# ziwang1121/IEEE

Hardware: AMD Instinct MI355X
Metric: 3-modal images/s (train fwd+bwd) (higher is better)
Workload: dtype bf16

## Files before the change

ieee_amd/_lib.py:

```python
import ctypes
import os

_HERE = os.path.dirname(os.path.abspath(__file__))
LIB_PATH = os.environ.get("IEEE_AMD_LIB", os.path.join(_HERE, "libieee_amd.so"))
_lib = None

c_void_p, c_int, c_int64, c_float, c_double = (ctypes.c_void_p, ctypes.c_int, ctypes.c_int64,
                                               ctypes.c_float, ctypes.c_double)

IEEE_F32, IEEE_BF16 = 0, 1

HEADER_PATH = os.path.join(os.path.dirname(_HERE), "include", "ieee_amd.h")

_CTYPE = {"int": c_int, "int64_t": c_int64, "float": c_float, "double": c_double}


def _parse_header(path=HEADER_PATH):
    import re
    txt = open(path).read()
    txt = re.sub(r"/\*.*?\*/", "", txt, flags=re.S)
    txt = re.sub(r"^\s*#.*$", "", txt, flags=re.M)
    sigs, res = {}, {}
    for m in re.finditer(r"([A-Za-z_][\w\s\*]*?)\b(ieee_[a-z0-9_]+)\s*\(([^)]*)\)\s*;", txt):
        ret, name, args = m.group(1).strip(), m.group(2), m.group(3).strip()
        argt = []
        if args and args != "void":
            for a in args.split(","):
                a = a.strip()
                if "*" in a:
                    argt.append(c_void_p)
                else:
                    base = a.replace("const", "").split()[0]
                    argt.append(_CTYPE[base])
        sigs[name] = argt
        if "char" in ret and "*" in ret:
            res[name] = ctypes.c_char_p
        elif "*" in ret:
            res[name] = c_void_p
        else:
            res[name] = _CTYPE[ret.replace("const", "").split()[0]]
    return sigs, res


_SIGNATURES, _RESTYPE = _parse_header()


class WgradReduceDesc(ctypes.Structure):
    _fields_ = [("slab", c_void_p), ("dw", c_void_p), ("slab_gs", c_int64), ("dw_gs", c_int64),
                ("nsplit", ctypes.c_int32), ("Co", ctypes.c_int32), ("Ci", ctypes.c_int32), ("RS", ctypes.c_int32),
                ("kind", ctypes.c_int32), ("sl_log2", ctypes.c_int32), ("blocks", ctypes.c_int32),
                ("accumulate", ctypes.c_int32), ("block_begin", ctypes.c_int32), ("reserved_", ctypes.c_int32)]


class ConvExtras(ctypes.Structure):
    _fields_ = [("totals", c_void_p), ("group_stride", c_int64), ("replicas", ctypes.c_int32), ("reserved_", ctypes.c_int32),
                ("overflow", c_void_p), ("start", c_void_p), ("stop", c_void_p)]


class SgemmSet(ctypes.Structure):
    _fields_ = [("groups", c_int64), ("A", c_void_p), ("B", c_void_p), ("C", c_void_p), ("bias", c_void_p),
                ("M", c_int64), ("N", c_int64), ("K", c_int64), ("sam", c_int64), ("sak", c_int64), ("sbn", c_int64),
                ("sbk", c_int64), ("ldc", c_int64), ("alpha", c_float), ("relu", ctypes.c_int32), ("accumulate", ctypes.c_int32)]


class IeeeAmdError(RuntimeError):
    pass


def exported_symbols():
    return sorted(_SIGNATURES)


def load():
    global _lib
    if _lib is not None:
        return _lib
    if not os.path.exists(LIB_PATH):
        raise IeeeAmdError(
            "ieee_amd HIP library not built: %s is missing. Run `python -c 'import __graft_entry__ as g; "
            "g.build()'` or `make -C ieee_amd/csrc`. There is no CPU fallback." % LIB_PATH)
    import torch
    lib = ctypes.CDLL(LIB_PATH)
    for name, argtypes in _SIGNATURES.items():
        fn = getattr(lib, name)
        fn.argtypes = argtypes
        fn.restype = _RESTYPE.get(name, c_int)
    _lib = lib
    return lib


def check(status):
    if status != 0:
        msg = load().ieee_last_error()
        raise IeeeAmdError((msg or b"").decode("utf-8", "replace") or "ieee_amd error %d" % status)


def require_gpu():
    import torch
    if not torch.cuda.is_available():
        raise IeeeAmdError("ieee_amd needs an MI355X (gfx950) GPU: torch.cuda.is_available() is False and there "
                           "is no CPU fallback.")
    lib = load()
    if not lib.ieee_device_is_gfx950():
        raise IeeeAmdError("ieee_amd kernels are built for gfx950 only; current device is not gfx950.")
    return lib


def ptr(t):
    return c_void_p(t.data_ptr()) if t is not None else c_void_p(0)


def stream():
    import torch
    return c_void_p(torch.cuda.current_stream().cuda_stream)
```

ieee_amd/csrc/head.hip:

```cpp
#include "gemm_core.h"

namespace ieee {

constexpr int MAXG = IEEE_MAX_GROUPS;

struct PtrTab { void* p[MAXG]; };

struct SgemmArgs {
  PtrTab A, B, C, bias;
  int M, N, K;
  int64_t sam, sak, sbn, sbk, ldc;
  float alpha;
  int relu, accumulate;
  int splitk, kchunk, vec_a, vec_b;
  float* slab;
};

typedef float SgemmStage[64][33];
__device__ __forceinline__ void sgemm_tile(const SgemmArgs& a, int bx, int by, int bz, SgemmStage* As, SgemmStage* Bs) {
  const int g = bz / a.splitk, ks = bz - g * a.splitk;
  const float* A = (const float*)a.A.p[g];
  const float* B = (const float*)a.B.p[g];
  const int m0 = by * 64, n0 = bx * 64;
  const int t = threadIdx.x, lane = t & 63, wave = t >> 6, wm = wave >> 1, wn = wave & 1;
  const int kbeg = ks * a.kchunk, kend = min(a.K, kbeg + a.kchunk);
  const int ktiles = (kend - kbeg + 31) / 32;
  f32x4 acc[2][2];
#pragma unroll
  for (int i = 0; i < 2; ++i)
#pragma unroll
    for (int j = 0; j < 2; ++j) acc[i][j] = f32x4{0.f, 0.f, 0.f, 0.f};
  float ra[8], rb[8];
  auto fetch = [&](const float* P, int vec, int64_t srow, int64_t sk, int row0, int nrows, int kt, float* r) {
    const int k0 = kbeg + kt * 32;
    if (vec == 1) {
#pragma unroll
      for (int h = 0; h < 2; ++h) {
        const int row = row0 + (t >> 3) + 32 * h, k = k0 + (t & 7) * 4;
        float4 v = make_float4(0.f, 0.f, 0.f, 0.f);
        if (row < nrows && k + 3 < kend) v = *(const float4*)(P + row * srow + k);
        else if (row < nrows) {
          if (k < kend) v.x = P[row * srow + k];
          if (k + 1 < kend) v.y = P[row * srow + k + 1];
          if (k + 2 < kend) v.z = P[row * srow + k + 2];
        }
        r[4 * h] = v.x; r[4 * h + 1] = v.y; r[4 * h + 2] = v.z; r[4 * h + 3] = v.w;
      }
    } else if (vec == 2) {
#pragma unroll
      for (int h = 0; h < 2; ++h) {
        const int k = k0 + (t >> 4) + 16 * h, row = row0 + (t & 15) * 4;
        float4 v = make_float4(0.f, 0.f, 0.f, 0.f);
        if (k < kend && row + 3 < nrows) v = *(const float4*)(P + k * sk + row);
        else if (k < kend) {
          if (row < nrows) v.x = P[k * sk + row];
          if (row + 1 < nrows) v.y = P[k * sk + row + 1];
          if (row + 2 < nrows) v.z = P[k * sk + row + 2];
        }
        r[4 * h] = v.x; r[4 * h + 1] = v.y; r[4 * h + 2] = v.z; r[4 * h + 3] = v.w;
      }
    } else {
#pragma unroll
      for (int e = 0; e < 8; ++e) {
        const int row = row0 + (t & 63), k = k0 + (t >> 6) + 4 * e;
        r[e] = (row < nrows && k < kend) ? P[row * srow + k * sk] : 0.f;
      }
    }
  };
  auto stash = [&](float (*S)[33], int vec, const float* r) {
    if (vec == 1) {
#pragma unroll
      for (int e = 0; e < 8; ++e) S[(t >> 3) + 32 * (e >> 2)][(t & 7) * 4 + (e & 3)] = r[e];
    } else if (vec == 2) {
#pragma unroll
      for (int e = 0; e < 8; ++e) S[(t & 15) * 4 + (e & 3)][(t >> 4) + 16 * (e >> 2)] = r[e];
    } else {
#pragma unroll
      for (int e = 0; e < 8; ++e) S[t & 63][(t >> 6) + 4 * e] = r[e];
    }
  };
  if (ktiles > 0) {
    fetch(A, a.vec_a, a.sam, a.sak, m0, a.M, 0, ra);
    fetch(B, a.vec_b, a.sbn, a.sbk, n0, a.N, 0, rb);
    stash(As[0], a.vec_a, ra);
    stash(Bs[0], a.vec_b, rb);
  }
  __syncthreads();
  for (int kt = 0; kt < ktiles; ++kt) {
    const int cur = kt & 1;
    const bool has_next = kt + 1 < ktiles;
    if (has_next) {
      fetch(A, a.vec_a, a.sam, a.sak, m0, a.M, kt + 1, ra);
      fetch(B, a.vec_b, a.sbn, a.sbk, n0, a.N, kt + 1, rb);
    }
#pragma unroll
    for (int kk = 0; kk < 8; ++kk) {
      float fa[2], fb[2];
#pragma unroll
      for (int i = 0; i < 2; ++i) fa[i] = As[cur][wm * 32 + i * 16 + (lane & 15)][kk * 4 + (lane >> 4)];
#pragma unroll
      for (int j = 0; j < 2; ++j) fb[j] = Bs[cur][wn * 32 + j * 16 + (lane & 15)][kk * 4 + (lane >> 4)];
#pragma unroll
      for (int i = 0; i < 2; ++i)
#pragma unroll
        for (int j = 0; j < 2; ++j) acc[i][j] = mfma16(fb[j], fa[i], acc[i][j]);
    }
    if (has_next) {
      stash(As[cur ^ 1], a.vec_a, ra);
      stash(Bs[cur ^ 1], a.vec_b, rb);
    }
    __syncthreads();
  }
  if (a.splitk > 1) {
    float* S = a.slab + (int64_t)bz * a.M * a.N;
#pragma unroll
    for (int i = 0; i < 2; ++i)
#pragma unroll
      for (int j = 0; j < 2; ++j) {
        const int m = m0 + wm * 32 + i * 16 + (lane & 15);
        const int n = n0 + wn * 32 + j * 16 + (lane >> 4) * 4;
        if (m >= a.M) continue;
#pragma unroll
        for (int r = 0; r < 4; ++r)
          if (n + r < a.N) S[(int64_t)m * a.N + n + r] = acc[i][j][r];
      }
    return;
  }
  float* C = (float*)a.C.p[g];
  const float* bias = (const float*)a.bias.p[g];
#pragma unroll
  for (int i = 0; i < 2; ++i)
#pragma unroll
    for (int j = 0; j < 2; ++j) {
      const int m = m0 + wm * 32 + i * 16 + (lane & 15);
      const int n = n0 + wn * 32 + j * 16 + (lane >> 4) * 4;
      if (m >= a.M) continue;
#pragma unroll
      for (int r = 0; r < 4; ++r) {
        if (n + r >= a.N) continue;
        float v = a.alpha * acc[i][j][r];
        if (bias) v += bias[n + r];
        float* c = C + (int64_t)m * a.ldc + n + r;
        if (a.accumulate) v += *c;
        if (a.relu) v = fmaxf(v, 0.f);
        *c = v;
      }
    }
}

__global__ __launch_bounds__(256) void sgemm_grouped_kernel(SgemmArgs a) {
  __shared__ float As[2][64][33];
  __shared__ float Bs[2][64][33];
  sgemm_tile(a, blockIdx.x, blockIdx.y, blockIdx.z, As, Bs);
}

struct PairDims { int gx0, gy0, blocks0, gx1, gy1; };
__global__ __launch_bounds__(256) void sgemm_grouped2_kernel(SgemmArgs a0, SgemmArgs a1, PairDims d) {
  __shared__ float As[2][64][33];
  __shared__ float Bs[2][64][33];
  int b = blockIdx.x;
  if (b < d.blocks0) {
    sgemm_tile(a0, b % d.gx0, (b / d.gx0) % d.gy0, b / (d.gx0 * d.gy0), As, Bs);
  } else {
    b -= d.blocks0;
    sgemm_tile(a1, b % d.gx1, (b / d.gx1) % d.gy1, b / (d.gx1 * d.gy1), As, Bs);
  }
}

__device__ __forceinline__ void sgemm_splitk_reduce_one(const SgemmArgs& a, int g, int64_t i) {
  const int64_t mn = (int64_t)a.M * a.N;
  if (i >= mn) return;
  const float* S = a.slab + (int64_t)g * a.splitk * mn + i;
  float s = 0.f;
  for (int k = 0; k < a.splitk; ++k) s += S[k * mn];
  const int m = (int)(i / a.N), n = (int)(i - (int64_t)m * a.N);
  float v = a.alpha * s;
  const float* bias = (const float*)a.bias.p[g];
  if (bias) v += bias[n];
  float* c = (float*)a.C.p[g] + (int64_t)m * a.ldc + n;
  if (a.accumulate) v += *c;
  if (a.relu) v = fmaxf(v, 0.f);
  *c = v;
}
__global__ __launch_bounds__(256) void sgemm_splitk_reduce_kernel(SgemmArgs a) {
  sgemm_splitk_reduce_one(a, blockIdx.y, (int64_t)blockIdx.x * blockDim.x + threadIdx.x);
}
struct PairReduceDims { int rb0, blocks0, rb1; };
__global__ __launch_bounds__(256) void sgemm_splitk_reduce2_kernel(SgemmArgs a0, SgemmArgs a1, PairReduceDims d) {
  int b = blockIdx.x;
  if (b < d.blocks0) {
    sgemm_splitk_reduce_one(a0, b / d.rb0, (int64_t)(b % d.rb0) * blockDim.x + threadIdx.x);
  } else {
    b -= d.blocks0;
    sgemm_splitk_reduce_one(a1, b / d.rb1, (int64_t)(b % d.rb1) * blockDim.x + threadIdx.x);
  }
}

struct ZeroArgs { PtrTab p; int64_t n[MAXG]; };
__global__ void zero_spans_kernel(ZeroArgs a) {
  float* p = (float*)a.p.p[blockIdx.y];
  const int64_t n = a.n[blockIdx.y];
  for (int64_t i = (int64_t)blockIdx.x * blockDim.x + threadIdx.x; i < n; i += (int64_t)gridDim.x * blockDim.x) p[i] = 0.f;
}

struct ColsumArgs {
  PtrTab X, out;
  int M, N;
  int64_t ldx;
  int accumulate;
};
__global__ void colsum_grouped_kernel(ColsumArgs a) {
  const int g = blockIdx.y;
  const int n = blockIdx.x * blockDim.x + threadIdx.x;
  if (n >= a.N) return;
  const float* X = (const float*)a.X.p[g];
  float s = 0.f;
  for (int m = 0; m < a.M; ++m) s += X[(int64_t)m * a.ldx + n];
  float* o = (float*)a.out.p[g] + n;
  *o = a.accumulate ? *o + s : s;
}

struct RowBnArgs {
  PtrTab x, out, gamma, beta, rmean, rvar, save;
  int R, C;
  int64_t ldx, ldo;
  float momentum, eps;
  int training, relu;
};
constexpr int RB_TX = 16, RB_TY = 16;
__device__ __forceinline__ float rb_sum(float (*red)[RB_TX], int tx) {
  float s = 0.f;
#pragma unroll
  for (int y = 0; y < RB_TY; ++y) s += red[y][tx];
  return s;
}
__global__ __launch_bounds__(256) void rowbn_fwd_kernel(RowBnArgs a) {
  __shared__ float red[RB_TY][RB_TX];
  const int g = blockIdx.y;
  const int tx = threadIdx.x % RB_TX, ty = threadIdx.x / RB_TX;
  const int c = blockIdx.x * RB_TX + tx;
  const bool ok = c < a.C;
  const float* x = (const float*)a.x.p[g];
  float* out = (float*)a.out.p[g];
  float mean, invstd;
  if (a.training) {
    float s = 0.f;
    if (ok) {
#pragma unroll 4
      for (int r = ty; r < a.R; r += RB_TY) s += x[(int64_t)r * a.ldx + c];
    }
    red[ty][tx] = s;
    __syncthreads();
    mean = rb_sum(red, tx) / a.R;
    __syncthreads();
    float v = 0.f;
    if (ok) {
#pragma unroll 4
      for (int r = ty; r < a.R; r += RB_TY) { const float d = x[(int64_t)r * a.ldx + c] - mean; v += d * d; }
    }
    red[ty][tx] = v;
    __syncthreads();
    const float var = rb_sum(red, tx) / a.R;
    invstd = 1.0f / sqrtf(var + a.eps);
    if (ok && ty == 0) {
      float* rm = (float*)a.rmean.p[g];
      float* rv = (float*)a.rvar.p[g];
      if (rm) {
        const float unb = a.R > 1 ? var * ((float)a.R / (float)(a.R - 1)) : var;
        rm[c] = (1.f - a.momentum) * rm[c] + a.momentum * mean;
        rv[c] = (1.f - a.momentum) * rv[c] + a.momentum * unb;
      }
    }
  } else {
    mean = ok ? ((const float*)a.rmean.p[g])[c] : 0.f;
    invstd = ok ? 1.0f / sqrtf(((const float*)a.rvar.p[g])[c] + a.eps) : 0.f;
  }
  if (!ok) return;
  if (ty == 0 && a.save.p[g]) { float* sv = (float*)a.save.p[g]; sv[c] = mean; sv[a.C + c] = invstd; }
  const float ga = ((const float*)a.gamma.p[g])[c], be = ((const float*)a.beta.p[g])[c];
#pragma unroll 4
  for (int r = ty; r < a.R; r += RB_TY) {
    float v = (x[(int64_t)r * a.ldx + c] - mean) * invstd * ga + be;
    if (a.relu) v = fmaxf(v, 0.f);
    out[(int64_t)r * a.ldo + c] = v;
  }
}

struct RowBnBwdArgs {
  PtrTab dout, out, x, gamma, save, dx, dgamma, dbeta;
  int R, C;
  int64_t lddo, ldo, ldx, lddx;
  int relu, accumulate;
};
__global__ __launch_bounds__(256) void rowbn_bwd_kernel(RowBnBwdArgs a) {
  __shared__ float red[2][RB_TY][RB_TX];
  const int g = blockIdx.y;
  const int tx = threadIdx.x % RB_TX, ty = threadIdx.x / RB_TX;
  const int c = blockIdx.x * RB_TX + tx;
  const bool ok = c < a.C;
  const float* dout = (const float*)a.dout.p[g];
  const float* out = (const float*)a.out.p[g];
  const float* x = (const float*)a.x.p[g];
  const float* sv = (const float*)a.save.p[g];
  const float mean = ok ? sv[c] : 0.f, invstd = ok ? sv[a.C + c] : 0.f;
  float s1 = 0.f, s2 = 0.f;
  if (ok) {
#pragma unroll 4
    for (int r = ty; r < a.R; r += RB_TY) {
      float gq = dout[(int64_t)r * a.lddo + c];
      if ((a.relu & 1) && !(out[(int64_t)r * a.ldo + c] > 0.f)) gq = 0.f;
      s1 += gq;
      s2 += gq * (x[(int64_t)r * a.ldx + c] - mean) * invstd;
    }
  }
  red[0][ty][tx] = s1;
  red[1][ty][tx] = s2;
  __syncthreads();
  s1 = rb_sum(red[0], tx);
  s2 = rb_sum(red[1], tx);
  if (!ok) return;
  const float ga = ((const float*)a.gamma.p[g])[c];
  const bool frozen = (a.relu & 2) != 0;
  if (ty == 0 && !frozen) {
    float* dg = (float*)a.dgamma.p[g] + c;
    float* db = (float*)a.dbeta.p[g] + c;
    *dg = a.accumulate ? *dg + s2 : s2;
    *db = a.accumulate ? *db + s1 : s1;
  }
  float* dx = (float*)a.dx.p[g];
  const float c1 = frozen ? 0.f : s1 / a.R, c2 = frozen ? 0.f : s2 / a.R;
#pragma unroll 4
  for (int r = ty; r < a.R; r += RB_TY) {
    float gq = dout[(int64_t)r * a.lddo + c];
    if ((a.relu & 1) && !(out[(int64_t)r * a.ldo + c] > 0.f)) gq = 0.f;
    const float xh = (x[(int64_t)r * a.ldx + c] - mean) * invstd;
    dx[(int64_t)r * a.lddx + c] = ga * invstd * (gq - c1 - xh * c2);
  }
}

__global__ void add_halves_kernel(const float* h, float* hs, int64_t half, int64_t gs_in, int64_t gs_out) {
  const int z = blockIdx.y;
  for (int64_t i = (int64_t)blockIdx.x * blockDim.x + threadIdx.x; i < half; i += (int64_t)gridDim.x * blockDim.x)
    hs[z * gs_out + i] = h[z * gs_in + i] + h[z * gs_in + half + i];
}
__global__ void sigmoid_kernel(float* x, int64_t n) {
  for (int64_t i = (int64_t)blockIdx.x * blockDim.x + threadIdx.x; i < n; i += (int64_t)gridDim.x * blockDim.x)
    x[i] = 1.0f / (1.0f + expf(-x[i]));
}
__global__ void sigmoid_bwd_kernel(const float* datt, const float* att, float* dz, int64_t n) {
  for (int64_t i = (int64_t)blockIdx.x * blockDim.x + threadIdx.x; i < n; i += (int64_t)gridDim.x * blockDim.x)
    dz[i] = datt[i] * att[i] * (1.f - att[i]);
}
__global__ void add_halves_bwd_kernel(const float* dhs, const float* h, float* dh, int64_t half, int64_t gs_half,
                                      int64_t gs_full) {
  const int z = blockIdx.y;
  for (int64_t i = (int64_t)blockIdx.x * blockDim.x + threadIdx.x; i < half; i += (int64_t)gridDim.x * blockDim.x) {
    const float d = dhs[z * gs_half + i];
    dh[z * gs_full + i] = h[z * gs_full + i] > 0.f ? d : 0.f;
    dh[z * gs_full + half + i] = h[z * gs_full + half + i] > 0.f ? d : 0.f;
  }
}

__global__ void rem_fwd_kernel(const float* part, const float* r, const float* param, int64_t param_gs, float* out,
                               int B, int parts, int D) {
  const int z = blockIdx.y;
  const float s = 2.0f * param[z * param_gs];
  const int64_t n = (int64_t)B * parts * D;
  for (int64_t i = (int64_t)blockIdx.x * blockDim.x + threadIdx.x; i < n; i += (int64_t)gridDim.x * blockDim.x) {
    const int k = (int)(i % D);
    const int b = (int)(i / ((int64_t)parts * D));
    out[z * n + i] = part[z * n + i] + s * r[((int64_t)z * B + b) * D + k];
  }
}
__global__ __launch_bounds__(256) void rem_bwd_kernel(const float* dout, const float* r, const float* param,
                                                      int64_t param_gs, float* dr, float* dparam_partial, int B,
                                                      int parts, int D) {
  __shared__ float red[256];
  const int z = blockIdx.y, b = blockIdx.x;
  const float s = 2.0f * param[z * param_gs];
  float accp = 0.f;
  for (int k = threadIdx.x; k < D; k += blockDim.x) {
    float sum = 0.f;
    for (int i = 0; i < parts; ++i) sum += dout[(((int64_t)z * B + b) * parts + i) * D + k];
    dr[((int64_t)z * B + b) * D + k] = s * sum;
    accp += sum * r[((int64_t)z * B + b) * D + k];
  }
  red[threadIdx.x] = accp;
  __syncthreads();
  for (int o = 128; o > 0; o >>= 1) { if (threadIdx.x < o) red[threadIdx.x] += red[threadIdx.x + o]; __syncthreads(); }
  if (threadIdx.x == 0) dparam_partial[(int64_t)z * B + b] = 2.0f * red[0];
}
__global__ void rem_dparam_kernel(const float* partial, float* dparam, int64_t grad_gs, int B, int accumulate) {
  const int z = threadIdx.x;
  if (z >= 3) return;
  float s = 0.f;
  for (int b = 0; b < B; ++b) s += partial[(int64_t)z * B + b];
  float* o = dparam + z * grad_gs;
  *o = accumulate ? *o + s : s;
}

__global__ void l2norm_fwd_kernel(const float* x, float* y, float* norms, int64_t rows, int D) {
  const int64_t row = (int64_t)blockIdx.x * 4 + (threadIdx.x >> 6);
  if (row >= rows) return;
  const int lane = threadIdx.x & 63;
  float s = 0.f;
  for (int k = lane; k < D; k += 64) { const float v = x[row * D + k]; s += v * v; }
  s = wave_sum(s);
  const float nrm = fmaxf(sqrtf(s), 1e-12f);
  for (int k = lane; k < D; k += 64) y[row * D + k] = x[row * D + k] / nrm;
  if (lane == 0) norms[row] = nrm;
}
__global__ void l2norm_bwd_kernel(const float* dy, const float* y, const float* norms, float* dx, int64_t rows, int D,
                                  int accumulate) {
  const int64_t row = (int64_t)blockIdx.x * 4 + (threadIdx.x >> 6);
  if (row >= rows) return;
  const int lane = threadIdx.x & 63;
  float s = 0.f;
  for (int k = lane; k < D; k += 64) s += dy[row * D + k] * y[row * D + k];
  s = wave_sum(s);
  const float nrm = norms[row];
  const float dot = nrm > 1e-12f ? s : 0.f;
  for (int k = lane; k < D; k += 64) {
    const float v = (dy[row * D + k] - y[row * D + k] * dot) / nrm;
    dx[row * D + k] = accumulate ? dx[row * D + k] + v : v;
  }
}

__global__ void ce_rows_kernel(const float* logits, const int64_t* target, float* rowloss, int* correct,
                               float* dlogits, int heads, int B, int C, float eps, float gscale) {
  const int64_t row = (int64_t)blockIdx.x * 4 + (threadIdx.x >> 6);
  if (row >= (int64_t)heads * B) return;
  const int lane = threadIdx.x & 63;
  const int b = (int)(row % B);
  const float* x = logits + row * C;
  const int y = (int)target[b];
  float mx = -INFINITY;
  int am = 0;
  for (int c = lane; c < C; c += 64) { const float v = x[c]; if (v > mx) { mx = v; am = c; } }
  for (int o = 32; o > 0; o >>= 1) {
    const float ov = __shfl_xor(mx, o);
    const int oi = __shfl_xor(am, o);
    if (ov > mx || (ov == mx && oi < am)) { mx = ov; am = oi; }
  }
  float se = 0.f, sx = 0.f;
  for (int c = lane; c < C; c += 64) { se += expf(x[c] - mx); sx += x[c]; }
  se = wave_sum(se);
  sx = wave_sum(sx);
  const float lse = mx + logf(se);
  const float logpy = x[y] - lse;
  if (lane == 0) {
    rowloss[row] = -(1.f - eps) * logpy - (eps / C) * (sx - C * lse);
    correct[row] = am == y ? 1 : 0;
  }
  if (dlogits) {
    const float sc = gscale / B;
    for (int c = lane; c < C; c += 64) {
      const float p = expf(x[c] - lse);
      const float tt = (c == y ? (1.f - eps) : 0.f) + eps / C;
      dlogits[row * C + c] = (p - tt) * sc;
    }
  }
}
__global__ void ce_heads_kernel(const float* rowloss, const int* correct, float* head_loss, float* head_acc,
                                int heads, int B) {
  const int h = blockIdx.x * blockDim.x + threadIdx.x;
  if (h >= heads) return;
  float s = 0.f;
  int k = 0;
  for (int b = 0; b < B; ++b) { s += rowloss[(int64_t)h * B + b]; k += correct[(int64_t)h * B + b]; }
  head_loss[h] = s / B;
  head_acc[h] = 100.0f * k / B;
}

__global__ __launch_bounds__(256) void margin3m_kernel(const float* feats, const int64_t* pids, float* dfeats,
                                                       float* terms, int B, int D, float margin, float gscale) {
  __shared__ float red[3][256];
  __shared__ int s_cnt[256];
  __shared__ int s_sel;
  __shared__ float s_sign;
  const int t = threadIdx.x;
  int cnt = 0;
  for (int i = t; i < B; i += 256) {
    bool seen = false;
    for (int j = 0; j < i; ++j) if (pids[j] == pids[i]) { seen = true; break; }
    cnt += seen ? 0 : 1;
  }
  s_cnt[t] = cnt;
  __syncthreads();
  for (int o = 128; o > 0; o >>= 1) { if (t < o) s_cnt[t] += s_cnt[t + o]; __syncthreads(); }
  const int n = s_cnt[0];
  const int csize = (B + n - 1) / n;
  const int nchunks = (B + csize - 1) / csize;
  const int nuse = nchunks < n ? nchunks : n;
  const int ch = blockIdx.x;
  const int64_t BD = (int64_t)B * D;
  if (ch == 0 && t == 0) { terms[B] = (float)n; terms[B + 1] = (float)nchunks; terms[B + 2] = (float)nuse; }
  const int r0 = ch * csize, r1 = min(B, r0 + csize), rows = r1 - r0;
  if (rows <= 0) { if (t == 0) terms[ch] = 0.f; return; }
  if (ch >= nuse) {
    if (t == 0) terms[ch] = 0.f;
    if (dfeats)
      for (int m = 0; m < 3; ++m)
        for (int64_t i = t; i < (int64_t)rows * D; i += 256) dfeats[m * BD + (int64_t)r0 * D + i] = 0.f;
    return;
  }
  float d12 = 0.f, d23 = 0.f, d13 = 0.f;
  for (int k = t; k < D; k += 256) {
    float c1 = 0.f, c2 = 0.f, c3 = 0.f;
    for (int r = r0; r < r1; ++r) { c1 += feats[r * D + k]; c2 += feats[BD + r * D + k]; c3 += feats[2 * BD + r * D + k]; }
    c1 /= rows; c2 /= rows; c3 /= rows;
    d12 += (c1 - c2) * (c1 - c2);
    d23 += (c2 - c3) * (c2 - c3);
    d13 += (c1 - c3) * (c1 - c3);
  }
  red[0][t] = d12; red[1][t] = d23; red[2][t] = d13;
  __syncthreads();
  for (int o = 128; o > 0; o >>= 1) {
    if (t < o) { red[0][t] += red[0][t + o]; red[1][t] += red[1][t + o]; red[2][t] += red[2][t + o]; }
    __syncthreads();
  }
  if (t == 0) {
    const float a1 = fabsf(margin - red[0][0]), a2 = fabsf(margin - red[1][0]), a3 = fabsf(margin - red[2][0]);
    int sel = 0; float best = a1;
    if (a2 > best) { best = a2; sel = 1; }
    if (a3 > best) { best = a3; sel = 2; }
    const float dsel = sel == 0 ? red[0][0] : (sel == 1 ? red[1][0] : red[2][0]);
    const float x = margin - dsel;
    s_sel = sel;
    s_sign = x > 0.f ? -1.f : (x < 0.f ? 1.f : 0.f);
    terms[ch] = best;
  }
  __syncthreads();
  if (dfeats) {
    const int sel = s_sel;
    const int ia = sel == 1 ? 1 : 0;
    const int ib = sel == 0 ? 1 : 2;
    const int ic = 3 - ia - ib;
    const float coef = s_sign * 2.0f / rows * gscale;
    for (int k = t; k < D; k += 256) {
      float ca = 0.f, cb = 0.f;
      for (int r = r0; r < r1; ++r) { ca += feats[ia * BD + r * D + k]; cb += feats[ib * BD + r * D + k]; }
      const float diff = (ca - cb) / rows;
      for (int r = r0; r < r1; ++r) {
        dfeats[ia * BD + r * D + k] = coef * diff;
        dfeats[ib * BD + r * D + k] = -coef * diff;
        dfeats[ic * BD + r * D + k] = 0.f;
      }
    }
  }
}
__global__ void margin3m_sum_kernel(const float* terms, float* out, int B) {
  if (threadIdx.x != 0) return;
  const int nuse = (int)terms[B + 2];
  float loss = 0.f;
  for (int c = 0; c < nuse; ++c) loss += terms[c];
  out[0] = loss; out[1] = terms[B]; out[2] = terms[B + 1];
}

__device__ __forceinline__ void sgd_one(float& w, float g, float& buf, float lr, float momentum, float wd, int nesterov) {
  float d = g + wd * w;
  if (momentum != 0.f) {
    const float b = momentum * buf + d;
    buf = b;
    d = nesterov ? d + momentum * b : b;
  }
  w = w - lr * d;
}
__global__ void sgd_nesterov_kernel(float* __restrict__ p, const float* __restrict__ g, float* __restrict__ buf,
                                    int64_t n, float lr, float momentum, float wd, int nesterov, int vec, bf16* __restrict__ shadow,
                                    const int* __restrict__ skip) {
  if (skip != nullptr && (skip[0] | skip[1]) != 0) return;
  const int64_t tid = (int64_t)blockIdx.x * blockDim.x + threadIdx.x, nth = (int64_t)gridDim.x * blockDim.x;
  int64_t done = 0;
  if (vec) {
    const int64_t n4 = n >> 2;
    for (int64_t i = tid; i < n4; i += nth) {
      float4 w = ((float4*)p)[i];
      const float4 gg = ((const float4*)g)[i];
      float4 b = momentum != 0.f ? ((float4*)buf)[i] : make_float4(0.f, 0.f, 0.f, 0.f);
      sgd_one(w.x, gg.x, b.x, lr, momentum, wd, nesterov);
      sgd_one(w.y, gg.y, b.y, lr, momentum, wd, nesterov);
      sgd_one(w.z, gg.z, b.z, lr, momentum, wd, nesterov);
      sgd_one(w.w, gg.w, b.w, lr, momentum, wd, nesterov);
      if (momentum != 0.f) ((float4*)buf)[i] = b;
      ((float4*)p)[i] = w;
      if (shadow != nullptr) ((uint2*)shadow)[i] = make_uint2(Vec16<bf16>::pk(w.x, w.y), Vec16<bf16>::pk(w.z, w.w));
    }
    done = n4 << 2;
  }
  for (int64_t i = done + tid; i < n; i += nth) {
    float w = p[i], b = momentum != 0.f ? buf[i] : 0.f;
    sgd_one(w, g[i], b, lr, momentum, wd, nesterov);
    if (momentum != 0.f) buf[i] = b;
    p[i] = w;
    if (shadow != nullptr) shadow[i] = (bf16)w;
  }
}

static int ewb(int64_t n) {
  static const int64_t cap = getenv("IEEE_HEAD_EW_BLOCKS") ? atoll(getenv("IEEE_HEAD_EW_BLOCKS")) : 2048;
  int64_t b = (n + 255) / 256;
  return (int)(b > cap ? cap : (b < 1 ? 1 : b));
}

}

using namespace ieee;

static int fill_tab(PtrTab* t, const void* const* src, int groups) {
  for (int i = 0; i < MAXG; ++i) t->p[i] = i < groups && src ? (void*)src[i] : nullptr;
  return 0;
}

static bool aligned16(const void* const* tab, int groups) {
  for (int i = 0; i < groups; ++i)
    if (((uintptr_t)tab[i] & 15) != 0) return false;
  return true;
}

static int sgemm_fill(SgemmArgs& a, int64_t groups, const void* const* A, const void* const* B, void* const* C,
                      const void* const* bias, int64_t M, int64_t N, int64_t K, int64_t sam, int64_t sak, int64_t sbn,
                      int64_t sbk, int64_t ldc, float alpha, int relu, int accumulate, void* work, int64_t work_bytes);

extern "C" int ieee_sgemm_grouped_ws(int64_t groups, const void* const* A, const void* const* B, void* const* C,
                                     const void* const* bias, int64_t M, int64_t N, int64_t K, int64_t sam, int64_t sak,
                                     int64_t sbn, int64_t sbk, int64_t ldc, float alpha, int relu, int accumulate,
                                     void* work, int64_t work_bytes, void* stream) {
  SgemmArgs a;
  IEEE_TRY(sgemm_fill(a, groups, A, B, C, bias, M, N, K, sam, sak, sbn, sbk, ldc, alpha, relu, accumulate, work, work_bytes));
  dim3 grid(cdiv(N, 64), cdiv(M, 64), (unsigned)(groups * a.splitk));
  sgemm_grouped_kernel<<<grid, 256, 0, (hipStream_t)stream>>>(a);
  IEEE_TRY(launch_status("sgemm_grouped_kernel"));
  if (a.splitk > 1) {
    sgemm_splitk_reduce_kernel<<<dim3(cdiv(M * N, 256), (unsigned)groups), 256, 0, (hipStream_t)stream>>>(a);
    return launch_status("sgemm_splitk_reduce_kernel");
  }
  return IEEE_OK;
}

extern "C" int ieee_sgemm_grouped_pair_ws(const ieee_sgemm_set* s0, const ieee_sgemm_set* s1, void* work, int64_t work_bytes,
                                          void* stream) {
  IEEE_REQUIRE(s0 && s1, "sgemm_grouped_pair: null problem set");
  const int64_t half = work ? (work_bytes / 2) & ~(int64_t)255 : 0;
  SgemmArgs a0, a1;
  IEEE_TRY(sgemm_fill(a0, s0->groups, s0->A, s0->B, s0->C, s0->bias, s0->M, s0->N, s0->K, s0->sam, s0->sak, s0->sbn, s0->sbk, s0->ldc,
                      s0->alpha, s0->relu, s0->accumulate, work, half));
  IEEE_TRY(sgemm_fill(a1, s1->groups, s1->A, s1->B, s1->C, s1->bias, s1->M, s1->N, s1->K, s1->sam, s1->sak, s1->sbn, s1->sbk, s1->ldc,
                      s1->alpha, s1->relu, s1->accumulate, work ? (char*)work + half : nullptr, half));
  PairDims d;
  d.gx0 = cdiv(s0->N, 64); d.gy0 = cdiv(s0->M, 64); d.blocks0 = d.gx0 * d.gy0 * (int)(s0->groups * a0.splitk);
  d.gx1 = cdiv(s1->N, 64); d.gy1 = cdiv(s1->M, 64);
  const int blocks1 = d.gx1 * d.gy1 * (int)(s1->groups * a1.splitk);
  sgemm_grouped2_kernel<<<dim3((unsigned)(d.blocks0 + blocks1)), 256, 0, (hipStream_t)stream>>>(a0, a1, d);
  IEEE_TRY(launch_status("sgemm_grouped2_kernel"));
  if (a0.splitk > 1 || a1.splitk > 1) {
    PairReduceDims r;
    r.rb0 = a0.splitk > 1 ? cdiv(s0->M * s0->N, 256) : 1;
    r.blocks0 = a0.splitk > 1 ? r.rb0 * (int)s0->groups : 0;
    r.rb1 = a1.splitk > 1 ? cdiv(s1->M * s1->N, 256) : 1;
    const int rblocks1 = a1.splitk > 1 ? r.rb1 * (int)s1->groups : 0;
    sgemm_splitk_reduce2_kernel<<<dim3((unsigned)(r.blocks0 + rblocks1)), 256, 0, (hipStream_t)stream>>>(a0, a1, r);
    return launch_status("sgemm_splitk_reduce2_kernel");
  }
  return IEEE_OK;
}

static int sgemm_fill(SgemmArgs& a, int64_t groups, const void* const* A, const void* const* B, void* const* C,
                      const void* const* bias, int64_t M, int64_t N, int64_t K, int64_t sam, int64_t sak, int64_t sbn,
                      int64_t sbk, int64_t ldc, float alpha, int relu, int accumulate, void* work, int64_t work_bytes) {
  IEEE_REQUIRE(groups >= 1 && groups <= MAXG, "sgemm_grouped: groups %ld out of range [1,%d]", (long)groups, MAXG);
  IEEE_REQUIRE(A && B && C, "sgemm_grouped: null pointer table");
  IEEE_REQUIRE(M > 0 && N > 0 && K > 0, "sgemm_grouped: empty problem");
  fill_tab(&a.A, A, (int)groups);
  fill_tab(&a.B, B, (int)groups);
  fill_tab(&a.C, (const void* const*)C, (int)groups);
  fill_tab(&a.bias, bias, (int)groups);
  a.M = (int)M; a.N = (int)N; a.K = (int)K;
  a.sam = sam; a.sak = sak; a.sbn = sbn; a.sbk = sbk; a.ldc = ldc;
  a.alpha = alpha; a.relu = relu; a.accumulate = accumulate;
  a.vec_a = (sak == 1 && sam % 4 == 0 && aligned16(A, (int)groups)) ? 1
            : (sam == 1 && sak % 4 == 0 && aligned16(A, (int)groups)) ? 2 : 0;
  a.vec_b = (sbk == 1 && sbn % 4 == 0 && aligned16(B, (int)groups)) ? 1
            : (sbn == 1 && sbk % 4 == 0 && aligned16(B, (int)groups)) ? 2 : 0;
  const int64_t tiles = cdiv(N, 64) * cdiv(M, 64) * groups;
  int64_t splitk = 1;
  if (work && tiles < 1024 && K >= 256) {
    splitk = cdiv(1024, tiles);
    if (splitk > K / 128) splitk = K / 128;
    if (splitk > 32) splitk = 32;
    while (splitk > 1 && splitk * groups * M * N * 4 > work_bytes) --splitk;
    if (splitk < 1) splitk = 1;
  }
  a.kchunk = (int)(cdiv(cdiv(K, splitk), 32) * 32);
  a.splitk = (int)cdiv(K, a.kchunk);
  a.slab = (float*)work;
  return IEEE_OK;
}

extern "C" int ieee_sgemm_grouped(int64_t groups, const void* const* A, const void* const* B, void* const* C,
                                  const void* const* bias, int64_t M, int64_t N, int64_t K, int64_t sam, int64_t sak,
                                  int64_t sbn, int64_t sbk, int64_t ldc, float alpha, int relu, int accumulate,
                                  void* stream) {
  return ieee_sgemm_grouped_ws(groups, A, B, C, bias, M, N, K, sam, sak, sbn, sbk, ldc, alpha, relu, accumulate, nullptr,
                               0, stream);
}

extern "C" int ieee_zero_spans(int64_t count, void* const* ptrs, const int64_t* floats, void* stream) {
  IEEE_REQUIRE(count >= 1 && count <= MAXG && ptrs && floats, "zero_spans: bad arguments");
  ZeroArgs a;
  fill_tab(&a.p, (const void* const*)ptrs, (int)count);
  int64_t most = 1;
  for (int i = 0; i < MAXG; ++i) { a.n[i] = i < count ? floats[i] : 0; most = a.n[i] > most ? a.n[i] : most; }
  zero_spans_kernel<<<dim3(ewb(most), (unsigned)count), 256, 0, (hipStream_t)stream>>>(a);
  return launch_status("zero_spans_kernel");
}

extern "C" int ieee_colsum_grouped(int64_t groups, const void* const* X, void* const* out, int64_t M, int64_t N,
                                   int64_t ldx, int accumulate, void* stream) {
  IEEE_REQUIRE(groups >= 1 && groups <= MAXG && X && out, "colsum_grouped: bad arguments");
  ColsumArgs a;
  fill_tab(&a.X, X, (int)groups);
  fill_tab(&a.out, (const void* const*)out, (int)groups);
  a.M = (int)M; a.N = (int)N; a.ldx = ldx; a.accumulate = accumulate;
  colsum_grouped_kernel<<<dim3(cdiv(N, 128), (unsigned)groups), 128, 0, (hipStream_t)stream>>>(a);
  return launch_status("colsum_grouped_kernel");
}

extern "C" int ieee_rowbn_fwd(int64_t groups, const void* const* x, void* const* out, const void* const* gamma,
                              const void* const* beta, void* const* running_mean, void* const* running_var,
                              void* const* save, int64_t R, int64_t C, int64_t ldx, int64_t ldo, float momentum,
                              float eps, int training, int relu, void* stream) {
  IEEE_REQUIRE(groups >= 1 && groups <= MAXG && x && out && gamma && beta, "rowbn_fwd: bad arguments");
  IEEE_REQUIRE(training || (running_mean && running_var), "rowbn_fwd: eval mode needs running stats");
  RowBnArgs a;
  fill_tab(&a.x, x, (int)groups);
  fill_tab(&a.out, (const void* const*)out, (int)groups);
  fill_tab(&a.gamma, gamma, (int)groups);
  fill_tab(&a.beta, beta, (int)groups);
  fill_tab(&a.rmean, (const void* const*)running_mean, (int)groups);
  fill_tab(&a.rvar, (const void* const*)running_var, (int)groups);
  fill_tab(&a.save, (const void* const*)save, (int)groups);
  a.R = (int)R; a.C = (int)C; a.ldx = ldx; a.ldo = ldo; a.momentum = momentum; a.eps = eps;
  a.training = training; a.relu = relu;
  rowbn_fwd_kernel<<<dim3(cdiv(C, RB_TX), (unsigned)groups), 256, 0, (hipStream_t)stream>>>(a);
  return launch_status("rowbn_fwd_kernel");
}

extern "C" int ieee_rowbn_bwd(int64_t groups, const void* const* dout, const void* const* out, const void* const* x,
                              const void* const* gamma, const void* const* save, void* const* dx,
                              void* const* dgamma, void* const* dbeta, int64_t R, int64_t C, int64_t lddo,
                              int64_t ldo, int64_t ldx, int64_t lddx, int relu, int accumulate, void* stream) {
  IEEE_REQUIRE(groups >= 1 && groups <= MAXG && dout && out && x && gamma && save && dx && dgamma && dbeta,
               "rowbn_bwd: bad arguments");
  RowBnBwdArgs a;
  fill_tab(&a.dout, dout, (int)groups);
  fill_tab(&a.out, out, (int)groups);
  fill_tab(&a.x, x, (int)groups);
  fill_tab(&a.gamma, gamma, (int)groups);
  fill_tab(&a.save, save, (int)groups);
  fill_tab(&a.dx, (const void* const*)dx, (int)groups);
  fill_tab(&a.dgamma, (const void* const*)dgamma, (int)groups);
  fill_tab(&a.dbeta, (const void* const*)dbeta, (int)groups);
  a.R = (int)R; a.C = (int)C; a.lddo = lddo; a.ldo = ldo; a.ldx = ldx; a.lddx = lddx;
  a.relu = relu; a.accumulate = accumulate;
  rowbn_bwd_kernel<<<dim3(cdiv(C, RB_TX), (unsigned)groups), 256, 0, (hipStream_t)stream>>>(a);
  return launch_status("rowbn_bwd_kernel");
}

extern "C" int ieee_ca_mix_fwd(const float* h, float* hs, int64_t B, int64_t hidden, void* stream) {
  IEEE_REQUIRE(h && hs, "ca_mix_fwd: null pointer");
  add_halves_kernel<<<dim3(ewb(B * hidden), 3), 256, 0, (hipStream_t)stream>>>(h, hs, B * hidden, 2 * B * hidden,
                                                                                B * hidden);
  return launch_status("add_halves_kernel");
}
extern "C" int ieee_ca_mix_bwd(const float* dhs, const float* h, float* dh, int64_t B, int64_t hidden, void* stream) {
  IEEE_REQUIRE(dhs && h && dh, "ca_mix_bwd: null pointer");
  add_halves_bwd_kernel<<<dim3(ewb(B * hidden), 3), 256, 0, (hipStream_t)stream>>>(dhs, h, dh, B * hidden, B * hidden,
                                                                                    2 * B * hidden);
  return launch_status("add_halves_bwd_kernel");
}
extern "C" int ieee_sigmoid_fwd(float* x, int64_t n, void* stream) {
  IEEE_REQUIRE(x, "sigmoid_fwd: null pointer");
  sigmoid_kernel<<<ewb(n), 256, 0, (hipStream_t)stream>>>(x, n);
  return launch_status("sigmoid_kernel");
}
extern "C" int ieee_sigmoid_bwd(const float* datt, const float* att, float* dz, int64_t n, void* stream) {
  IEEE_REQUIRE(datt && att && dz, "sigmoid_bwd: null pointer");
  sigmoid_bwd_kernel<<<ewb(n), 256, 0, (hipStream_t)stream>>>(datt, att, dz, n);
  return launch_status("sigmoid_bwd_kernel");
}

extern "C" int ieee_rem_fwd(const float* part, const float* r, const float* param, int64_t param_gs, float* out,
                            int64_t B, int64_t parts, int64_t D, void* stream) {
  IEEE_REQUIRE(part && r && param && out, "rem_fwd: null pointer");
  rem_fwd_kernel<<<dim3(ewb(B * parts * D), 3), 256, 0, (hipStream_t)stream>>>(part, r, param, param_gs, out, (int)B,
                                                                                (int)parts, (int)D);
  return launch_status("rem_fwd_kernel");
}
extern "C" int ieee_rem_bwd(const float* dout, const float* r, const float* param, int64_t param_gs, float* dr,
                            float* dparam, int64_t grad_gs, float* work, int64_t B, int64_t parts, int64_t D,
                            int accumulate, void* stream) {
  IEEE_REQUIRE(dout && r && param && dr && dparam && work, "rem_bwd: null pointer");
  hipStream_t st = (hipStream_t)stream;
  rem_bwd_kernel<<<dim3((unsigned)B, 3), 256, 0, st>>>(dout, r, param, param_gs, dr, work, (int)B, (int)parts, (int)D);
  IEEE_TRY(launch_status("rem_bwd_kernel"));
  rem_dparam_kernel<<<1, 64, 0, st>>>(work, dparam, grad_gs, (int)B, accumulate);
  return launch_status("rem_dparam_kernel");
}

extern "C" int ieee_l2norm_fwd(const float* x, float* y, float* norms, int64_t rows, int64_t D, void* stream) {
  IEEE_REQUIRE(x && y && norms, "l2norm_fwd: null pointer");
  l2norm_fwd_kernel<<<cdiv(rows, 4), 256, 0, (hipStream_t)stream>>>(x, y, norms, rows, (int)D);
  return launch_status("l2norm_fwd_kernel");
}
extern "C" int ieee_l2norm_bwd(const float* dy, const float* y, const float* norms, float* dx, int64_t rows,
                               int64_t D, int accumulate, void* stream) {
  IEEE_REQUIRE(dy && y && norms && dx, "l2norm_bwd: null pointer");
  l2norm_bwd_kernel<<<cdiv(rows, 4), 256, 0, (hipStream_t)stream>>>(dy, y, norms, dx, rows, (int)D, accumulate);
  return launch_status("l2norm_bwd_kernel");
}

extern "C" int ieee_ce_ls_fwd_bwd(const float* logits, const int64_t* targets, float* dlogits, float* head_loss,
                                  float* head_acc, float* work, int64_t heads, int64_t B, int64_t C, float eps,
                                  float grad_scale, void* stream) {
  IEEE_REQUIRE(logits && targets && head_loss && head_acc && work, "ce_ls_fwd_bwd: null pointer");
  IEEE_REQUIRE(heads >= 1 && B >= 1 && C >= 1, "ce_ls_fwd_bwd: empty input");
  hipStream_t st = (hipStream_t)stream;
  float* rowloss = work;
  int* correct = (int*)(work + heads * B);
  ce_rows_kernel<<<cdiv(heads * B, 4), 256, 0, st>>>(logits, targets, rowloss, correct, dlogits, (int)heads, (int)B,
                                                     (int)C, eps, grad_scale);
  IEEE_TRY(launch_status("ce_rows_kernel"));
  ce_heads_kernel<<<cdiv(heads, 64), 64, 0, st>>>(rowloss, correct, head_loss, head_acc, (int)heads, (int)B);
  return launch_status("ce_heads_kernel");
}

extern "C" int ieee_margin3m_fwd_bwd(const float* feats, const int64_t* pids, float* dfeats, float* out3, float* work,
                                     int64_t B, int64_t D, float margin, float grad_scale, void* stream) {
  IEEE_REQUIRE(feats && pids && out3 && work, "margin3m_fwd_bwd: null pointer");
  IEEE_REQUIRE(B >= 1 && D >= 1 && B <= 65535, "margin3m_fwd_bwd: batch out of range");
  hipStream_t st = (hipStream_t)stream;
  margin3m_kernel<<<(unsigned)B, 256, 0, st>>>(feats, pids, dfeats, work, (int)B, (int)D, margin, grad_scale);
  IEEE_TRY(launch_status("margin3m_kernel"));
  margin3m_sum_kernel<<<1, 64, 0, st>>>(work, out3, (int)B);
  return launch_status("margin3m_sum_kernel");
}

__global__ void adam_kernel(float* __restrict__ p, const float* __restrict__ g, float* __restrict__ m,
                            float* __restrict__ v, float* __restrict__ vmax, int64_t n, float lr, float b1, float b2,
                            float eps, float wd, float bc1, float bc2_sqrt) {
  const float step_size = lr / bc1;
  for (int64_t i = (int64_t)blockIdx.x * blockDim.x + threadIdx.x; i < n; i += (int64_t)gridDim.x * blockDim.x) {
    const float w = p[i];
    const float d = g[i] + wd * w;
    const float mi = m[i] + (d - m[i]) * (1.f - b1);
    const float vi = b2 * v[i] + (1.f - b2) * d * d;
    m[i] = mi;
    v[i] = vi;
    float vv = vi;
    if (vmax != nullptr) {
      vv = fmaxf(vmax[i], vi);
      vmax[i] = vv;
    }
    const float denom = sqrtf(vv) / bc2_sqrt + eps;
    p[i] = w - step_size * (mi / denom);
  }
}

extern "C" int ieee_adam_step(float* params, const float* grads, float* exp_avg, float* exp_avg_sq,
                              float* max_exp_avg_sq, int64_t n, float lr, float beta1, float beta2, float eps,
                              float weight_decay, int64_t step, void* stream) {
  IEEE_REQUIRE(params && grads && exp_avg && exp_avg_sq, "adam_step: null pointer");
  IEEE_REQUIRE(step >= 1, "adam_step: step counts from 1");
  if (n <= 0) return IEEE_OK;
  const double bc1 = 1.0 - pow((double)beta1, (double)step), bc2 = 1.0 - pow((double)beta2, (double)step);
  adam_kernel<<<ewb(n), 256, 0, (hipStream_t)stream>>>(params, grads, exp_avg, exp_avg_sq, max_exp_avg_sq, n, lr, beta1,
                                                       beta2, eps, weight_decay, (float)bc1, (float)sqrt(bc2));
  return launch_status("adam_kernel");
}

__global__ void guard_buffers_kernel(const int* __restrict__ flags, float* __restrict__ buffers, float* __restrict__ backup, int64_t n) {
  const bool restore = flags[0] != 0;
  for (int64_t i = (int64_t)blockIdx.x * blockDim.x + threadIdx.x; i < n; i += (int64_t)gridDim.x * blockDim.x) {
    if (restore) buffers[i] = backup[i]; else backup[i] = buffers[i];
  }
}
extern "C" int ieee_guard_buffers(const int* flags, float* buffers, float* backup, int64_t n, void* stream) {
  IEEE_REQUIRE(flags && buffers && backup && n >= 0, "guard_buffers: bad arguments");
  if (n == 0) return IEEE_OK;
  guard_buffers_kernel<<<ewb(n), 256, 0, (hipStream_t)stream>>>(flags, buffers, backup, n);
  return launch_status("guard_buffers_kernel");
}

extern "C" int ieee_sgd_nesterov_step_ex(float* params, const float* grads, float* momentum_buf, int64_t n, float lr,
                                         float momentum, float weight_decay, int nesterov, void* shadow_bf16,
                                         const int* skip_flags, void* stream) {
  IEEE_REQUIRE(params && grads && (momentum == 0.f || momentum_buf), "sgd_nesterov_step: null pointer");
  if (n <= 0) return IEEE_OK;
  const int vec = ((((uintptr_t)params | (uintptr_t)grads | (uintptr_t)momentum_buf) & 15) == 0 && ((uintptr_t)shadow_bf16 & 7) == 0) ? 1 : 0;
  sgd_nesterov_kernel<<<ewb(vec ? (n + 3) / 4 : n), 256, 0, (hipStream_t)stream>>>(params, grads, momentum_buf, n, lr,
                                                                                   momentum, weight_decay, nesterov, vec,
                                                                                   (bf16*)shadow_bf16, skip_flags);
  return launch_status("sgd_nesterov_kernel");
}

extern "C" int ieee_sgd_nesterov_step(float* params, const float* grads, float* momentum_buf, int64_t n, float lr,
                                      float momentum, float weight_decay, int nesterov, void* stream) {
  return ieee_sgd_nesterov_step_ex(params, grads, momentum_buf, n, lr, momentum, weight_decay, nesterov, nullptr, nullptr, stream);
}

__global__ void grad_pack_bf16_kernel(const float* __restrict__ g, bf16* __restrict__ out, int64_t n, int64_t peel) {
  const int64_t tid = (int64_t)blockIdx.x * blockDim.x + threadIdx.x, nth = (int64_t)gridDim.x * blockDim.x;
  const int64_t n8 = (n - peel) >> 3;
  const float4* g4 = (const float4*)(g + peel);
  uint4* o4 = (uint4*)(out + peel);
  for (int64_t i = tid; i < n8; i += nth) {
    const float4 a = g4[2 * i], b = g4[2 * i + 1];
    const float f[8] = {a.x, a.y, a.z, a.w, b.x, b.y, b.z, b.w};
    o4[i] = Vec16<bf16>::pack(f);
  }
  for (int64_t i = tid; i < peel; i += nth) out[i] = (bf16)g[i];
  for (int64_t i = peel + (n8 << 3) + tid; i < n; i += nth) out[i] = (bf16)g[i];
}
__global__ void grad_unpack_bf16_kernel(const bf16* __restrict__ in, float* __restrict__ g, int64_t n, int64_t peel) {
  const int64_t tid = (int64_t)blockIdx.x * blockDim.x + threadIdx.x, nth = (int64_t)gridDim.x * blockDim.x;
  const int64_t n8 = (n - peel) >> 3;
  const uint4* i4 = (const uint4*)(in + peel);
  float4* g4 = (float4*)(g + peel);
  for (int64_t i = tid; i < n8; i += nth) {
    float f[8];
    Vec16<bf16>::unpack(i4[i], f);
    g4[2 * i] = make_float4(f[0], f[1], f[2], f[3]);
    g4[2 * i + 1] = make_float4(f[4], f[5], f[6], f[7]);
  }
  for (int64_t i = tid; i < peel; i += nth) g[i] = (float)in[i];
  for (int64_t i = peel + (n8 << 3) + tid; i < n; i += nth) g[i] = (float)in[i];
}

static int64_t grad_peel(const void* f32p, const void* bf16p, int64_t n) {
  const int64_t peel = (int64_t)(((32 - ((uintptr_t)f32p & 31)) & 31) >> 2);
  if ((((uintptr_t)f32p & 3) != 0) || ((((uintptr_t)bf16p + 2 * peel) & 15) != 0) || peel > n) return n;
  return peel;
}

extern "C" int ieee_grad_pack_bf16(const float* grads, void* out_bf16, int64_t n, void* stream) {
  if (n <= 0) return IEEE_OK;
  IEEE_REQUIRE(grads && out_bf16, "grad_pack_bf16: null pointer");
  const int64_t peel = grad_peel(grads, out_bf16, n);
  grad_pack_bf16_kernel<<<ewb((n + 7) / 8 + 8), 256, 0, (hipStream_t)stream>>>(grads, (bf16*)out_bf16, n, peel);
  return launch_status("grad_pack_bf16_kernel");
}
extern "C" int ieee_grad_unpack_bf16(const void* in_bf16, float* grads, int64_t n, void* stream) {
  if (n <= 0) return IEEE_OK;
  IEEE_REQUIRE(grads && in_bf16, "grad_unpack_bf16: null pointer");
  const int64_t peel = grad_peel(grads, in_bf16, n);
  grad_unpack_bf16_kernel<<<ewb((n + 7) / 8 + 8), 256, 0, (hipStream_t)stream>>>((const bf16*)in_bf16, grads, n, peel);
  return launch_status("grad_unpack_bf16_kernel");
}
```

ieee_amd/csrc/net.hip:

```cpp
#include <stdio.h>
#include <stdlib.h>
#include <string.h>

#include <map>
#include <string>
#include <vector>

#include "common.h"

namespace {

using namespace ieee;

struct Tensor {
  size_t off = 0;
  int64_t numel = 0;
  int dtype = IEEE_F32;
};

static constexpr int TOT_REP_MAX = 8;
static int totals_tiles() {
  static const int t = getenv("IEEE_BN_TOTALS_TILES") ? atoi(getenv("IEEE_BN_TOTALS_TILES")) : 1024;
  return t;
}
// ... 649 lines not shown
    return wgrad_on(u, dy, x);
  }
  int wgrad_on(const ConvUnit& u, const void* dy, const void* x) {
    prof_begin(1, u);
    struct G { Run* r; ~G() { r->prof_end(); } } guard{this};
    if (u.Ci != u.Ci_src || u.S != u.S_src || u.R != u.R_src) {
      const int64_t npad = (int64_t)u.Co * u.Ci * u.R * u.S;
      IEEE_TRY(wgrad_pending_now());
      IEEE_TRY(ieee_conv2d_wgrad(dy, x, F(u.dwpad), P(n.slab), n.dtype, 3, B, u.Hi, u.Wi, u.Ci, u.Co, u.R, u.S, u.stride,
                                 u.pad, u.M(B) * u.Co, (int64_t)B * u.Hi * u.Wi * u.Ci, npad, 0, st));
      return ieee_unpad_weight_grad(F(u.dwpad), grd(u.s_w), 3, u.Co, u.Ci, u.R, u.S, u.Ci_src, u.R_src, u.S_src, npad, gs(u.s_w), 0,
                                    st);
    }
    if (wgrad_batch_mode() == 0 && wgrad_chain()) {
      ieee_wgrad_reduce_desc d;
      const int rc = ieee_conv2d_wgrad_chained(dy, x, grd(u.s_w), P(n.wflip ? n.slab2 : n.slab), n.dtype, 3, B, u.Hi, u.Wi, u.Ci, u.Co,
                                               u.R, u.S, u.stride, u.pad, u.M(B) * u.Co, (int64_t)B * u.Hi * u.Wi * u.Ci, gs(u.s_w), 0,
                                               n.wpend.kind != 0 ? &n.wpend : nullptr, &d, st);
      if (rc != IEEE_OK) return rc;
      n.wpend = d;
      if (d.kind != 0) n.wflip ^= 1;
      return IEEE_OK;
    }
    if (wgrad_batch_mode() == 0 && wgrad_fold() && n.dtype == IEEE_BF16)
      return ieee_conv2d_wgrad_fold(dy, x, grd(u.s_w), P(n.slab), (int32_t*)P(n.wtickets), n.dtype, 3, B, u.Hi, u.Wi, u.Ci, u.Co,
                                    u.R, u.S, u.stride, u.pad, u.M(B) * u.Co, (int64_t)B * u.Hi * u.Wi * u.Ci, gs(u.s_w), 0, st);
    if (wgrad_batch_mode() == 0)
      return ieee_conv2d_wgrad(dy, x, grd(u.s_w), P(n.slab), n.dtype, 3, B, u.Hi, u.Wi, u.Ci, u.Co, u.R, u.S, u.stride,
                               u.pad, u.M(B) * u.Co, (int64_t)B * u.Hi * u.Wi * u.Ci, gs(u.s_w), 0, st);
    ieee_wgrad_reduce_desc d;
    IEEE_TRY(ieee_conv2d_wgrad_deferred(dy, x, grd(u.s_w), P(u.slab), n.dtype, 3, B, u.Hi, u.Wi, u.Ci, u.Co, u.R, u.S, u.stride,
                                        u.pad, u.M(B) * u.Co, (int64_t)B * u.Hi * u.Wi * u.Ci, gs(u.s_w), 0, &d, st));
    if (d.kind != 0) n.rpend.push_back(d);
    return IEEE_OK;
  }
  int wgrad_pending_now() {
    if (n.wpend.kind == 0) return IEEE_OK;
    const ieee_wgrad_reduce_desc d = n.wpend;
    n.wpend.kind = 0;
    return ieee_wgrad_reduce_pending(&d, 3, st);
  }
  int wgrad_flush(int slot) {
    if (n.wpend.kind != 0) {
      void* main_st = st;
      const bool on_side = side_enabled();
      if (on_side) st = (void*)n.side;
      prof_begin(1, n.reduce_unit, "wgrad_reduce");
      const int rc = wgrad_pending_now();
      prof_end();
      st = main_st;
      if (on_side) n.side_dirty = true;
      IEEE_TRY(rc);
    }
    if (n.rpend.empty()) return IEEE_OK;
    std::vector<ieee_wgrad_reduce_desc> tab;
    tab.swap(n.rpend);
    IEEE_REQUIRE(slot >= 0 && slot < Net::RT_SLOTS && (int)tab.size() <= Net::RT_MAX, "net: reduce table overflow (%d entries, slot %d)",
                 (int)tab.size(), slot);
    int blocks = 0;
    for (auto& d : tab) { d.block_begin = blocks; blocks += d.blocks; }
    void* main_st = st;
    const bool on_side = side_enabled();
    if (on_side) st = (void*)n.side;
    struct G { Run* r; void* m; ~G() { r->st = m; } } restore{this, main_st};
    ieee_wgrad_reduce_desc* dev = (ieee_wgrad_reduce_desc*)(ws + n.rtab.off) + (size_t)slot * Net::RT_MAX;
    std::vector<ieee_wgrad_reduce_desc>& host = n.rtab_host[slot];
    const size_t bytes = tab.size() * sizeof(ieee_wgrad_reduce_desc);
    if (n.rtab_ws[slot] != (const void*)ws || host.size() != tab.size() || memcmp(host.data(), tab.data(), bytes) != 0) {
      host = tab;
      IEEE_HIP(hipStreamSynchronize((hipStream_t)st));
      IEEE_HIP(hipMemcpy(dev, host.data(), bytes, hipMemcpyHostToDevice));
      n.rtab_ws[slot] = (const void*)ws;
    }
    prof_begin(1, n.reduce_unit, "wgrad_reduce");
    struct H { Run* r; ~H() { r->prof_end(); } } guard{this};
    const int rc = ieee_wgrad_reduce_batch(dev, (int64_t)tab.size(), blocks, 3, st);
    if (on_side) n.side_dirty = true;
    return rc;
  }
  const ConvUnit* ds_sums_of = nullptr;
  int dgrad(const ConvUnit& u, const void* dy, void* dx, const void* addend, const ConvUnit* prev = nullptr,
            bool prev_mask_tensor = false, int addend_stride = 1, const ConvUnit* prev_ds = nullptr) {
    const int64_t ldd = ieee_conv_packed_ld(n.dtype, u.Co, u.R, u.S);
    const bool fuse = prev != nullptr && n.dtype == IEEE_BF16;
    static const bool ds_sums = getenv("IEEE_DS_SUMS") && atoi(getenv("IEEE_DS_SUMS")) != 0;
    const bool fuse2 = fuse && prev_ds != nullptr && ds_sums && !branch_enabled(2);
    fused_bwd = fuse;
    n.bwd_totals_state = fuse && !fuse2 && use_totals(*prev) && !frz(*prev);
    if (fuse2) ds_sums_of = prev_ds;
    will_write(dx);
    prof_begin(0, u, "dgrad", true);
    struct G { Run* r; ~G() { r->prof_end(); } } guard{this};
    const ieee_conv_extras* ex = n.bwd_totals_state ? take_extras(P(prev->tot_b), (int64_t)2 * prev->Co, totals_rep(*prev))
                                                    : take_extras(nullptr, 0, 1);
    return ieee_conv2d_dgrad_ex(dy, P(u.wd), dx, addend, n.dtype, 3, B, u.Hi, u.Wi, u.Ci, u.Co, u.R, u.S, u.stride, u.pad,
                              u.M(B) * u.Co, u.Ci * ldd, (int64_t)B * u.Hi * u.Wi * u.Ci, fuse ? bnpart_cur : nullptr,
                              fuse ? P(prev->y) : nullptr,
                              (fuse && prev_mask_tensor) ? (prev->abits.numel ? P(prev->abits) : P(prev->a)) : nullptr,
                              (fuse && !prev_mask_tensor) ? F(prev->stats) : nullptr,
                              (fuse && prev_mask_tensor && prev->abits.numel) ? 1 : 0, addend_stride,
                              fuse2 ? P(prev_ds->y) : nullptr, fuse2 ? (float*)(ws + n.bnpart2.off) : nullptr, ex, st);
  }
  bool compact_ds(const ConvUnit& d, const ConvUnit* prev) const {
    static const bool on = !(getenv("IEEE_DS_COMPACT") && atoi(getenv("IEEE_DS_COMPACT")) == 0);
    return on && n.dtype == IEEE_BF16 && prev != nullptr && d.R == 1 && d.S == 1 && d.stride == 2 && d.pad == 0 && d.Hi == 2 * d.Ho &&
           d.Wi == 2 * d.Wo && !(d.Hi & (d.Hi - 1)) && !(d.Wi & (d.Wi - 1));
  }
  int dgrad_compact(const ConvUnit& d, const void* dy, void* dx) {
    const int64_t ldd = ieee_conv_packed_ld(n.dtype, d.Co, 1, 1);
    fused_bwd = false;
    n.bwd_totals_state = false;
    will_write(dx);
    prof_begin(0, d, "dgrad", true);
    struct G { Run* r; ~G() { r->prof_end(); } } guard{this};
    return ieee_conv2d_dgrad_ex(dy, P(d.wd), dx, nullptr, n.dtype, 3, B, d.Ho, d.Wo, d.Ci, d.Co, 1, 1, 1, 0, d.M(B) * d.Co,
                                d.Ci * ldd, d.M(B) * d.Ci, nullptr, nullptr, nullptr, nullptr, 0, 1, nullptr, nullptr,
                                take_extras(nullptr, 0, 1), st);
  }
  int gemm3(const float* A, int64_t a_gs, const float* Bm, int64_t b_gs, float* C, int64_t c_gs, const float* bias,
            int64_t bias_gs, int64_t M, int64_t N, int64_t K, int64_t sam, int64_t sak, int64_t sbn, int64_t sbk,
            int64_t ldc, int relu, int acc) {
    const void* a[3]; const void* b[3]; void* c[3]; const void* bi[3];
    for (int m = 0; m < 3; ++m) { a[m] = A + m * a_gs; b[m] = Bm + m * b_gs; c[m] = C + m * c_gs; bi[m] = bias ? bias + m * bias_gs : nullptr; }
    return ieee_sgemm_grouped_ws(3, a, b, c, bias ? bi : nullptr, M, N, K, sam, sak, sbn, sbk, ldc, 1.0f, relu, acc,
                                 P(n.gemm_work), (int64_t)n.gemm_work.numel * 2, st);
  }
  static bool head_pairs() {
    static const bool on = !(getenv("IEEE_HEAD_PAIRS") && atoi(getenv("IEEE_HEAD_PAIRS")) == 0);
    return on;
  }
  struct Set3 {
    const void* a[3]; const void* b[3]; void* c[3]; const void* bi[3];
    ieee_sgemm_set s;
  };
  static void set3(Set3& o, const float* A, int64_t a_gs, const float* Bm, int64_t b_gs, float* C, int64_t c_gs, const float* bias,
                   int64_t bias_gs, int64_t M, int64_t N, int64_t K, int64_t sam, int64_t sak, int64_t sbn, int64_t sbk,
                   int64_t ldc, int relu, int acc) {
    for (int m = 0; m < 3; ++m) { o.a[m] = A + m * a_gs; o.b[m] = Bm + m * b_gs; o.c[m] = C + m * c_gs; o.bi[m] = bias ? bias + m * bias_gs : nullptr; }
    o.s = ieee_sgemm_set{3, o.a, o.b, o.c, bias ? o.bi : nullptr, M, N, K, sam, sak, sbn, sbk, ldc, 1.0f, relu, acc};
  }
  static ieee_sgemm_set setg(int64_t groups, const void* const* A, const void* const* B, void* const* C, int64_t M, int64_t N,
                             int64_t K, int64_t sam, int64_t sak, int64_t sbn, int64_t sbk, int64_t ldc, int acc) {
    return ieee_sgemm_set{groups, A, B, C, nullptr, M, N, K, sam, sak, sbn, sbk, ldc, 1.0f, 0, acc};
  }
  int gemm_pair(const ieee_sgemm_set& s0, const ieee_sgemm_set& s1) {
    const int64_t bytes = (int64_t)n.gemm_work.numel * 4;
    if (head_pairs()) return ieee_sgemm_grouped_pair_ws(&s0, &s1, P(n.gemm_work), bytes, st);
    const int64_t half = (bytes / 2) & ~(int64_t)255;
    for (const ieee_sgemm_set* s : {&s0, &s1})
      IEEE_TRY(ieee_sgemm_grouped_ws(s->groups, s->A, s->B, s->C, s->bias, s->M, s->N, s->K, s->sam, s->sak, s->sbn, s->sbk, s->ldc,
                                     s->alpha, s->relu, s->accumulate, P(n.gemm_work), half, st));
    return IEEE_OK;
  }
  bool late_pack_pending = false;
  bool use_shadow = false;
  int forward(const float* xr, const float* xn, const float* xt, int training, float* logits_out, float* feats_out) {
    const int rc = forward_impl(xr, xn, xt, training, logits_out, feats_out);
    if (rc != IEEE_OK && training)
      (void)hipMemsetAsync(P(n.tickets), 0, 512 * 4, (hipStream_t)st);
    if (late_pack_pending) {
      (void)hipStreamWaitEvent((hipStream_t)st, n.pack_ev[1], 0);
      late_pack_pending = false;
    }
    return rc;
  }
  int forward_impl(const float* xr, const float* xn, const float* xt, int training, float* logits_out, float* feats_out);
  int backward(const float* dlogits, const float* dfeats, int part = -1, bool join = true) {
    const int rc = backward_impl(dlogits, dfeats, part);
    if (join || rc != IEEE_OK) side_join();
    return rc;
  }
  void side_wait_on(void* other) {
    if (!n.side_dirty || n.side == nullptr) return;
    (void)hipEventRecord(n.side_done, n.side);
    (void)hipStreamWaitEvent((hipStream_t)other, n.side_done, 0);
  }
  int backward_impl(const float* dlogits, const float* dfeats, int part);
  int backward_head(const float* dlogits, const float* dfeats);
};

int Run::forward_impl(const float* xr, const float* xn, const float* xt, int training, float* logits_out, float* feats_out) {
  Net& N = n;
  const int dt = N.dtype;
  {
    char* tab_dev = ws + N.packtab.off;
    const size_t bytes_eval = N.pack_eval.size() * sizeof(PackDescHost);
    const size_t bytes_train = N.pack_train.size() * sizeof(PackDescHost);
    const size_t bytes_late = N.pack_late.size() * sizeof(PackDescHost);
    const size_t bytes_train_s = N.pack_train_s.size() * sizeof(PackDescHost);
    if (N.pack_uploaded_ws != (const void*)ws) {
      IEEE_HIP(hipMemcpyAsync(tab_dev, N.pack_eval.data(), bytes_eval, hipMemcpyHostToDevice, (hipStream_t)st));
      IEEE_HIP(hipMemcpyAsync(tab_dev + bytes_eval, N.pack_train.data(), bytes_train, hipMemcpyHostToDevice, (hipStream_t)st));
      IEEE_HIP(hipMemcpyAsync(tab_dev + bytes_eval + bytes_train, N.pack_late.data(), bytes_late, hipMemcpyHostToDevice, (hipStream_t)st));
      if (bytes_train_s)
        IEEE_HIP(hipMemcpyAsync(tab_dev + bytes_eval + bytes_train + bytes_late, N.pack_train_s.data(), bytes_train_s,
                                hipMemcpyHostToDevice, (hipStream_t)st));
      if (!N.pack_late_s.empty())
        IEEE_HIP(hipMemcpyAsync(tab_dev + bytes_eval + bytes_train + bytes_late + bytes_train_s, N.pack_late_s.data(),
                                N.pack_late_s.size() * sizeof(PackDescHost), hipMemcpyHostToDevice, (hipStream_t)st));
      N.pack_uploaded_ws = ws;
    }
    use_shadow = training && dt == IEEE_BF16 && N.shadow != nullptr;
    const char* t_train = use_shadow ? tab_dev + bytes_eval + bytes_train + bytes_late : tab_dev + bytes_eval;
    const char* t_late = use_shadow ? tab_dev + bytes_eval + bytes_train + bytes_late + bytes_train_s : tab_dev + bytes_eval + bytes_train;
    const int64_t n_train = use_shadow ? (int64_t)N.pack_train_s.size() : (int64_t)N.pack_train.size();
    const int64_t n_late = use_shadow ? (int64_t)N.pack_late_s.size() : (int64_t)N.pack_late.size();
    const int64_t n_early = use_shadow ? N.pack_late_first_s : N.pack_late_first;
    const int b_train = use_shadow ? N.pack_blocks_train_s : N.pack_blocks_train, b_late = use_shadow ? N.pack_blocks_late_s : N.pack_blocks_late,
              b_early = use_shadow ? N.pack_blocks_early_s : N.pack_blocks_early;
    static const bool pack_async = !(getenv("IEEE_PACK_ASYNC") && atoi(getenv("IEEE_PACK_ASYNC")) == 0);
    if (training && pack_async && side_enabled() && n_late > 0) {
      IEEE_HIP(hipEventRecord(N.pack_ev[0], (hipStream_t)st));
      IEEE_HIP(hipStreamWaitEvent(N.side, N.pack_ev[0], 0));
      IEEE_TRY(ieee_pack_all_weights(N.params, ws, t_late, n_late, b_late, dt, (void*)N.side));
      IEEE_HIP(hipEventRecord(N.pack_ev[1], N.side));
      late_pack_pending = true;
      if (n_early > 0) IEEE_TRY(ieee_pack_all_weights(N.params, ws, t_train, n_early, b_early, dt, st));
    } else if (training)
      IEEE_TRY(ieee_pack_all_weights(N.params, ws, t_train, n_train, b_train, dt, st));
    else if (!(eval_cached = (N.eval_cache_valid && N.eval_cache_ws == (const void*)ws && !N.profiling)))
      IEEE_TRY(ieee_pack_all_weights(N.params, ws, tab_dev, (int64_t)N.pack_eval.size(), N.pack_blocks_eval, dt, st));
    if (training) N.eval_cache_valid = false;
  }
  {
    static const bool f_fin = getenv("IEEE_BN_FIN_FUSE") && atoi(getenv("IEEE_BN_FIN_FUSE")) != 0;
    if (training && f_fin) IEEE_HIP(hipMemsetAsync(P(N.tickets), 0, 512 * 4, (hipStream_t)st));
  }
  if (training && dt == IEEE_BF16 && (totals_tiles() > 0 || wgrad_fold())) {
    IEEE_HIP(hipMemsetAsync(ws + N.tot_begin, 0, N.tot_end - N.tot_begin, (hipStream_t)st));
    N.bwd_totals_fresh = true;
  }
  IEEE_TRY(ieee_nchw_to_nhwc3(xr, xn, xt, P(N.x0), dt, B, 3, N.H, N.W, 4, 3, st));
  const ConvUnit& s = N.units[N.u_stem];
  static const bool fuse_eval = !(getenv("IEEE_EVAL_FUSE") && atoi(getenv("IEEE_EVAL_FUSE")) == 0);
  const bool fe = !training && fuse_eval;
  bool stem_pool_fused = false;
  if (fe) {
    IEEE_TRY(conv_bn_eval(s, P(N.x0), nullptr, P(s.a), 1));
  } else {
    IEEE_TRY(conv(s, P(N.x0), training != 0));
    static const bool fuse_pool = !(getenv("IEEE_STEM_POOL_FUSE") && atoi(getenv("IEEE_STEM_POOL_FUSE")) == 0);
    stem_pool_fused = training && fuse_pool;
    IEEE_TRY(bn(s, nullptr, stem_pool_fused ? nullptr : P(s.a), 1, training));
  }
  N.stem_a_valid = !stem_pool_fused;
  if (stem_pool_fused)
    IEEE_TRY(ieee_bn_relu_maxpool3x3s2_fwd(P(s.y), F(s.stats), P(N.pool), (uint8_t*)P(N.pool_arg), dt, 3, B, s.Ho, s.Wo, s.Co, st));
  else
    IEEE_TRY(ieee_maxpool3x3s2_fwd(P(s.a), P(N.pool), (uint8_t*)P(N.pool_arg), dt, 3, B, s.Ho, s.Wo, s.Co, st));
  const void* x = P(N.pool);
  int ds_slot = 0;
  for (const Block& b : N.blocks) {
    const ConvUnit &c1 = N.units[b.c1], &c2 = N.units[b.c2], &c3 = N.units[b.c3];
    if (late_pack_pending && b.c1 >= N.pack_late_unit) {
      IEEE_HIP(hipStreamWaitEvent((hipStream_t)st, N.pack_ev[1], 0));
      late_pack_pending = false;
    }
    const bool ws_ = training != 0;
    const bool par_ds = b.ds >= 0 && training && branch_enabled(1);
    if (par_ds) {
      const ConvUnit& d = N.units[b.ds];
      BranchScope scope(*this, ds_slot);
      IEEE_TRY(conv(d, x, ws_));
      IEEE_TRY(bn(d, nullptr, P(d.a), 0, training));
    }
    if (fe) {
      IEEE_TRY(conv_bn_eval(c1, x, nullptr, P(c1.a), 1));
      IEEE_TRY(conv_bn_eval(c2, P(c1.a), nullptr, P(c2.a), 1));
      const void* idn = x;
      if (b.ds >= 0) {
        const ConvUnit& d = N.units[b.ds];
        IEEE_TRY(conv_bn_eval(d, x, nullptr, P(d.a), 0));
        idn = P(d.a);
      }
      IEEE_TRY(conv_bn_eval(c3, P(c2.a), idn, P(c3.a), 1));
      x = P(c3.a);
      continue;
    }
    IEEE_TRY(conv(c1, x, ws_));
    IEEE_TRY(bn(c1, nullptr, P(c1.a), 1, training));
    IEEE_TRY(conv(c2, P(c1.a), ws_));
    IEEE_TRY(bn(c2, nullptr, P(c2.a), 1, training));
    const void* identity = x;
    if (b.ds >= 0) {
      const ConvUnit& d = N.units[b.ds];
      if (par_ds) {
        branch_join(ds_slot);
      } else {
        IEEE_TRY(conv(d, x, ws_));
        IEEE_TRY(bn(d, nullptr, P(d.a), 0, training));
      }
      identity = P(d.a);
      ++ds_slot;
    }
    IEEE_TRY(conv(c3, P(c2.a), ws_));
    IEEE_TRY(bn(c3, identity, P(c3.a), 1, training, (training && c3.abits.numel) ? P(c3.abits) : nullptr));
    x = P(c3.a);
  }
  const void* Fm = x;
  const ConvUnit &uo = N.units[N.u_one], &ur = N.units[N.u_rest];
  const int Hh_ = uo.Hi, Ww = uo.Wi, C = N.fdim;
  const int64_t BC = (int64_t)B * C;
  IEEE_TRY(ieee_gpool_sum_others(Fm, N.interaction ? P(N.S) : nullptr, F(N.Gp), dt, B, Hh_, Ww, C, st));
  const int mode = !N.interaction ? 2 : (N.attention ? 0 : 1);
  if (N.interaction) {
    IEEE_TRY(conv(uo, Fm, training != 0));
    if (!eval_cached) IEEE_TRY(bn(uo, nullptr, nullptr, 1, training));
    IEEE_TRY(conv(ur, P(N.S), training != 0));
    if (!eval_cached) IEEE_TRY(bn(ur, nullptr, nullptr, 1, training));
    if (N.attention) {
      IEEE_TRY(ieee_ca_pool(P(ur.y), F(ur.stats), F(N.avgmax), F(N.avgmax) + BC, 2 * BC, (int32_t*)P(N.amax), dt, B, Hh_,
                            Ww, C, st));
      IEEE_TRY(gemm3(F(N.avgmax), 2 * BC, par(N.s_ca1), gs(N.s_ca1), F(N.Hh), 2 * B * N.hid, nullptr, 0, 2 * B, N.hid, C,
                     C, 1, C, 1, N.hid, 1, 0));
      IEEE_TRY(ieee_ca_mix_fwd(F(N.Hh), F(N.Hs), B, N.hid, st));
      IEEE_TRY(gemm3(F(N.Hs), (int64_t)B * N.hid, par(N.s_ca2), gs(N.s_ca2), F(N.att), BC, nullptr, 0, B, C, N.hid,
                     N.hid, 1, N.hid, 1, C, 0, 0));
      IEEE_TRY(ieee_sigmoid_fwd(F(N.att), 3 * BC, st));
    }
    IEEE_TRY(ieee_cim_tail_fwd(P(uo.y), P(ur.y), F(uo.stats), F(ur.stats), F(N.att), F(N.Pp), dt, B, Hh_, Ww, C, N.parts,
                               mode, st));
  } else {
    IEEE_TRY(ieee_cim_tail_fwd(Fm, nullptr, nullptr, nullptr, nullptr, F(N.Pp), dt, B, Hh_, Ww, C, N.parts, 2, st));
  }
  const int R = N.rdim, PB = N.parts * B;
  {
    Set3 g, p;
    set3(g, F(N.Gp), BC, par(N.s_rw), gs(N.s_rw), F(N.Zg), (int64_t)B * R, nullptr, 0, B, R, C, C, 1, C, 1, R, 0, 0);
    set3(p, F(N.Pp), (int64_t)PB * C, par(N.s_rw), gs(N.s_rw), F(N.Zp), (int64_t)PB * R, nullptr, 0, PB, R, C, C, 1, C, 1, R, 0, 0);
    IEEE_TRY(gemm_pair(g.s, p.s));
  }
  {
    const void *x1[3], *x2[3], *ga[3], *be[3];
    void *o1[3], *o2[3], *rm[3], *rv[3], *s1[3], *s2[3];
    for (int m = 0; m < 3; ++m) {
      x1[m] = F(N.Zg) + (int64_t)m * B * R; o1[m] = F(N.glob) + (int64_t)m * B * R;
      x2[m] = F(N.Zp) + (int64_t)m * PB * R; o2[m] = F(N.part) + (int64_t)m * PB * R;
      ga[m] = par(N.s_rg + m); be[m] = par(N.s_rb + m); rm[m] = buf(N.s_rrm + m); rv[m] = buf(N.s_rrv + m);
      s1[m] = F(N.sv_g) + m * 2 * R; s2[m] = F(N.sv_p) + m * 2 * R;
    }
    const int tr_red = (training && !(N.frozen & IEEE_FROZEN_REDUCE)) ? 1 : 0;
    IEEE_TRY(ieee_rowbn_fwd(3, x1, o1, ga, be, rm, rv, s1, B, R, R, R, N.bn_mom, N.bn_eps, tr_red, 1, st));
    IEEE_TRY(ieee_rowbn_fwd(3, x2, o2, ga, be, rm, rv, s2, PB, R, R, R, N.bn_mom, N.bn_eps, tr_red, 1, st));
  }
  const float* p2 = F(N.part);
  if (N.using_rem) {
    IEEE_TRY(gemm3(F(N.glob), (int64_t)B * R, par(N.s_rem_pw), gs(N.s_rem_pw), F(N.rr), (int64_t)B * R, par(N.s_rem_pb),
                   gs(N.s_rem_pb), B, R, R, R, 1, R, 1, R, 0, 0));
    IEEE_TRY(ieee_rem_fwd(F(N.part), F(N.rr), par(N.s_rem_param), gs(N.s_rem_param), F(N.part2), B, N.parts, R, st));
    p2 = F(N.part2);
  }
  const int D = N.cdim;
  {
    const void *a[18], *w[18], *bi[18], *ga[18], *be[18], *xs[18];
    void *c[18], *o[18], *rm[18], *rv[18], *sv[18];
    const int eval_off[3] = {R, 2 * R, 0};
    for (int m = 0; m < 3; ++m)
      for (int i = 0; i < 6; ++i) {
        const int g = m * 6 + i;
        a[g] = p2 + (int64_t)m * PB * R + i * R;
        w[g] = par(N.s_fcw[g]); bi[g] = par(N.s_fcb[g]);
        c[g] = F(N.fcraw) + (int64_t)g * B * D; xs[g] = c[g];
        ga[g] = par(N.s_fcg[g]); be[g] = par(N.s_fcbe[g]); rm[g] = buf(N.s_fcrm[g]); rv[g] = buf(N.s_fcrv[g]);
        sv[g] = F(N.sv_fc) + g * 2 * D;
        o[g] = training ? (void*)(F(N.featcat) + (int64_t)m * B * R + i * D) : (void*)(F(N.fcall) + eval_off[m] + i * D);
      }
    IEEE_TRY(ieee_sgemm_grouped_ws(18, a, w, c, bi, B, D, R, (int64_t)N.parts * R, 1, R, 1, D, 1.0f, 0, 0, P(N.gemm_work),
                                   (int64_t)N.gemm_work.numel * 2, st));
    const int fz = (N.frozen / IEEE_FROZEN_FC_R) & 7;
    if (!training || fz == 0 || fz == 7) {
      IEEE_TRY(ieee_rowbn_fwd(18, xs, o, ga, be, rm, rv, sv, B, D, D, training ? R : 3 * R, N.bn_mom, N.bn_eps,
                              (training && fz == 0) ? 1 : 0, 1, st));
    } else {
      for (int m = 0; m < 3; ++m)
        IEEE_TRY(ieee_rowbn_fwd(6, xs + 6 * m, o + 6 * m, ga + 6 * m, be + 6 * m, rm + 6 * m, rv + 6 * m, sv + 6 * m, B, D, D, R,
                                N.bn_mom, N.bn_eps, (fz >> m) & 1 ? 0 : 1, 1, st));
    }
  }
  if (!training) {
    IEEE_HIP(hipMemcpyAsync(feats_out, F(N.fcall), sizeof(float) * (size_t)B * 3 * R, hipMemcpyDeviceToDevice, (hipStream_t)st));
    if (fe) { N.eval_cache_valid = true; N.eval_cache_ws = ws; }
    return IEEE_OK;
  }
  {
    const void *a[18], *w[18], *bi[18];
    void* c[18];
    const int NC = N.num_classes;
    for (int m = 0; m < 3; ++m)
      for (int i = 0; i < 6; ++i) {
        const int g = m * 6 + i;
        a[g] = F(N.featcat) + (int64_t)m * B * R + i * D;
        w[g] = par(N.s_clw[g]); bi[g] = par(N.s_clb[g]);
        c[g] = logits_out + (int64_t)g * B * NC;
      }
    IEEE_TRY(ieee_sgemm_grouped_ws(18, a, w, c, bi, B, NC, D, R, 1, D, 1, NC, 1.0f, 0, 0, P(N.gemm_work),
                                   (int64_t)N.gemm_work.numel * 2, st));
  }
  IEEE_TRY(ieee_l2norm_fwd(F(N.featcat), F(N.featn), F(N.norms), 3 * (int64_t)B, R, st));
  IEEE_HIP(hipMemcpyAsync(feats_out, F(N.featn), sizeof(float) * (size_t)3 * B * R, hipMemcpyDeviceToDevice, (hipStream_t)st));
  return IEEE_OK;
}

int Run::backward_impl(const float* dlogits, const float* dfeats, int part) {
  Net& N = n;
  const int dt = N.dtype;
  if (!N.rpend.empty()) {
    N.rpend.clear();
    for (int i = 0; i < Net::RT_SLOTS; ++i) N.rtab_ws[i] = nullptr;
    IEEE_REQUIRE(false, "net_backward: the previous backward ended with unflushed weight-gradient reductions (a failed call?); "
                        "its gradients are incomplete -- run the step again");
  }
  if (part <= 0) {
    N.wpend.kind = 0;
    if (dt == IEEE_BF16 && (totals_tiles() > 0 || wgrad_fold())) {
      if (!N.bwd_totals_fresh) {
        const size_t skip = (size_t)N.oflags.numel * 4;
        IEEE_HIP(hipMemsetAsync(ws + N.tot_begin + skip, 0, N.tot_end - N.tot_begin - skip, (hipStream_t)st));
      }
      N.bwd_totals_fresh = false;
    }
    IEEE_TRY(backward_head(dlogits, dfeats));
  }
  if (part == 0) return IEEE_OK;
  static const int first_block[5] = {0, 3, 7, 13, 16};
  int hi = (int)N.blocks.size() - 1, lo = 0;
  if (part > 0) { hi = first_block[5 - part] - 1; lo = first_block[4 - part]; }
  static const int nsets = gbuf_sets();
  auto set_of = [](int bi) { return nsets == 2 ? ((bi & 1) ? 0 : 5) : ((bi + 3) % 3) * 5; };
  void *X = nullptr, *Q = nullptr, *Rb = nullptr, *U = nullptr, *V = nullptr, *Xout = nullptr;
  for (int bi = hi; bi >= lo; --bi) {
    const Block& b = N.blocks[bi];
    const int sb = set_of(bi);
    X = P(N.gbuf[sb]); Q = P(N.gbuf[sb + 1]); Rb = P(N.gbuf[sb + 2]); U = P(N.gbuf[sb + 3]); V = P(N.gbuf[sb + 4]);
    Xout = P(N.gbuf[set_of(bi - 1)]);
    const ConvUnit &c1 = N.units[b.c1], &c2 = N.units[b.c2], &c3 = N.units[b.c3];
    const void* xin = bi == 0 ? P(N.pool) : P(N.units[N.blocks[bi - 1].c3].a);
    if (N.tap_base && bi + 1 == (int)N.blocks.size()) IEEE_TRY(tap(c3.name + ".dout", X, out_numel(c3)));
    if (dt == IEEE_BF16 && bi + 1 < (int)N.blocks.size()) {
      static const bool ds_totals = !(getenv("IEEE_DS_TOTALS") && atoi(getenv("IEEE_DS_TOTALS")) == 0);
      if (ds_totals && b.ds >= 0 && !branch_enabled(2)) ds_pending = &N.units[b.ds];
      IEEE_TRY(bn_bwd(c3, X, nullptr, Q, nullptr));
      std::swap(X, Q);
    } else {
      IEEE_TRY(bn_bwd(c3, X, P(c3.a), X, Q));
    }
    if (N.tap_base) {
      IEEE_TRY(tap(c3.name + ".g", Q, out_numel(c3)));
      IEEE_TRY(tap(c3.name + ".dy", X, out_numel(c3)));
    }
    const int bslot = 4 + (bi == 0 ? 0 : (bi == 3 ? 1 : (bi == 7 ? 2 : 3)));
    const bool par_ds = b.ds >= 0 && branch_enabled(2);
    if (par_ds) {
      const ConvUnit& d = N.units[b.ds];
      BranchScope scope(*this, bslot);
      IEEE_TRY(bn_bwd(d, Q, nullptr, Q, nullptr));
      IEEE_TRY(tap(d.name + ".dy", Q, out_numel(d)));
      IEEE_TRY(wgrad(d, Q, xin));
      IEEE_TRY(dgrad(d, Q, V, nullptr));
      IEEE_TRY(tap(d.name + ".dx", V, in_numel(d)));
    }
    IEEE_TRY(wgrad(c3, X, P(c2.a)));
    IEEE_TRY(dgrad(c3, X, Rb, nullptr, &c2));
    IEEE_TRY(tap(c3.name + ".dx", Rb, in_numel(c3)));
    IEEE_TRY(bn_bwd(c2, Rb, nullptr, Rb, nullptr, 1));
    IEEE_TRY(tap(c2.name + ".dy", Rb, out_numel(c2)));
    IEEE_TRY(wgrad(c2, Rb, P(c1.a)));
    IEEE_TRY(dgrad(c2, Rb, U, nullptr, &c1));
    IEEE_TRY(tap(c2.name + ".dx", U, in_numel(c2)));
    IEEE_TRY(bn_bwd(c1, U, nullptr, U, nullptr, 1));
    IEEE_TRY(tap(c1.name + ".dy", U, out_numel(c1)));
    IEEE_TRY(wgrad(c1, U, xin));
    const void* addend = Q;
    const ConvUnit* pc3 = bi > 0 ? &N.units[N.blocks[bi - 1].c3] : nullptr;
    int addend_stride = 1;
    if (b.ds >= 0) {
      const ConvUnit& d = N.units[b.ds];
      const bool compact = !par_ds && compact_ds(d, pc3);
      if (par_ds) {
        branch_join(bslot);
      } else {
        if (ds_sums_of == &d)
          IEEE_TRY(bn_bwd(d, Q, nullptr, Q, nullptr, 0, (float*)(ws + N.bnpart2.off), (d.M(B) + 127) / 128));
        else
          IEEE_TRY(bn_bwd(d, Q, nullptr, Q, nullptr));
        ds_sums_of = nullptr;
        IEEE_TRY(tap(d.name + ".dy", Q, out_numel(d)));
        IEEE_TRY(wgrad(d, Q, xin));
        if (compact) IEEE_TRY(dgrad_compact(d, Q, V));
        else IEEE_TRY(dgrad(d, Q, V, nullptr));
        IEEE_TRY(tap(d.name + (compact ? ".dx_compact" : ".dx"), V, compact ? (int64_t)3 * d.M(B) * d.Ci : in_numel(d)));
      }
      addend = V;
      if (compact) addend_stride = 2;
    }
    const ConvUnit* pds = (bi > 0 && N.blocks[bi - 1].ds >= 0) ? &N.units[N.blocks[bi - 1].ds] : nullptr;
    IEEE_TRY(dgrad(c1, U, Xout, addend, pc3, true, addend_stride, pds));
    IEEE_TRY(tap(c1.name + ".dx", Xout, in_numel(c1)));
    if (wgrad_batch_mode() == 2 && bi > 0) IEEE_TRY(wgrad_flush(5 + bi));
    if (bi > 0)
      for (int l = 1; l < 4; ++l) if (bi == first_block[l]) IEEE_TRY(wgrad_flush(4 - l));
  }
  if (lo > 0) return IEEE_OK;
  X = P(N.gbuf[set_of(-1)]);
  Q = P(N.gbuf[set_of(-1) + 1]);
  const ConvUnit& s = N.units[N.u_stem];
  will_write(Q);
  static const bool fuse_stem = !(getenv("IEEE_STEM_BWD_FUSE") && atoi(getenv("IEEE_STEM_BWD_FUSE")) == 0);
  if (fuse_stem && !frz(s)) {
    fused_bwd = false;
    IEEE_TRY(ieee_bn2d_bwd_pooled(X, (const uint8_t*)P(N.pool_arg), P(s.y), Q, dt, 3, B, s.Ho, s.Wo, s.Co, par(s.s_g),
                                  gs(s.s_g), F(s.stats), grd(s.s_g), grd(s.s_b), gs(s.s_g), bnpart_cur, bncoef_cur, 0, st));
  } else {
    IEEE_TRY(ieee_maxpool3x3s2_bwd(X, (const uint8_t*)P(N.pool_arg), Q, dt, 3, B, s.Ho, s.Wo, s.Co, st));
    IEEE_TRY(bn_bwd(s, Q, nullptr, Q, nullptr, 1));
  }
  IEEE_TRY(tap(s.name + ".dy", Q, out_numel(s)));
  IEEE_TRY(wgrad(s, Q, P(N.x0)));
  IEEE_TRY(wgrad_flush(4));
  return IEEE_OK;
}

int Run::backward_head(const float* dlogits, const float* dfeats) {
  Net& N = n;
  fused_bwd = false;
  const int dt = N.dtype;
  const int R = N.rdim, D = N.cdim, C = N.fdim, PB = N.parts * B, NC = N.num_classes;
  const int64_t BC = (int64_t)B * C;
  const ConvUnit &uo = N.units[N.u_one], &ur = N.units[N.u_rest];
  const int Hh_ = uo.Hi, Ww = uo.Wi;
  const float* p2 = N.using_rem ? F(N.part2) : F(N.part);
  IEEE_TRY(ieee_l2norm_bwd(dfeats, F(N.featn), F(N.norms), F(N.dfeatcat), 3 * (int64_t)B, R, 0, st));
  {
    const void *dl[18], *fe[18], *w[18], *xs[18], *ga[18], *sv[18], *dfr[18], *pp[18];
    void *dw[18], *db[18], *dfc[18], *dx[18], *dg[18], *dbe[18], *dwf[18], *dbf[18], *dp2[18];
    for (int m = 0; m < 3; ++m)
      for (int i = 0; i < 6; ++i) {
        const int g = m * 6 + i;
        dl[g] = dlogits + (int64_t)g * B * NC;
        fe[g] = F(N.featcat) + (int64_t)m * B * R + i * D;
        w[g] = par(N.s_clw[g]);
        dw[g] = grd(N.s_clw[g]); db[g] = grd(N.s_clb[g]);
        dfc[g] = F(N.dfeatcat) + (int64_t)m * B * R + i * D;
        xs[g] = F(N.fcraw) + (int64_t)g * B * D;
        ga[g] = par(N.s_fcg[g]); sv[g] = F(N.sv_fc) + g * 2 * D;
        dx[g] = F(N.dfcraw) + (int64_t)g * B * D; dfr[g] = dx[g];
        dg[g] = grd(N.s_fcg[g]); dbe[g] = grd(N.s_fcbe[g]);
        dwf[g] = grd(N.s_fcw[g]); dbf[g] = grd(N.s_fcb[g]);
        pp[g] = p2 + (int64_t)m * PB * R + i * R;
        dp2[g] = F(N.dpart2) + (int64_t)m * PB * R + i * R;
      }
    IEEE_TRY(gemm_pair(setg(18, dl, fe, dw, NC, D, B, 1, NC, 1, R, D, 0), setg(18, dl, w, dfc, B, D, NC, NC, 1, 1, D, R, 1)));
    IEEE_TRY(ieee_colsum_grouped(18, dl, db, B, NC, NC, 0, st));
    const int fz = (N.frozen / IEEE_FROZEN_FC_R) & 7;
    if (fz == 0 || fz == 7) {
      IEEE_TRY(ieee_rowbn_bwd(18, (const void* const*)dfc, fe, xs, ga, sv, dx, dg, dbe, B, D, R, R, D, D, fz ? 3 : 1, 0, st));
    } else {
      for (int m = 0; m < 3; ++m)
        IEEE_TRY(ieee_rowbn_bwd(6, (const void* const*)dfc + 6 * m, fe + 6 * m, xs + 6 * m, ga + 6 * m, sv + 6 * m, dx + 6 * m,
                                dg + 6 * m, dbe + 6 * m, B, D, R, R, D, D, (fz >> m) & 1 ? 3 : 1, 0, st));
    }
    const void* wf[18];
    for (int g = 0; g < 18; ++g) wf[g] = par(N.s_fcw[g]);
    IEEE_TRY(gemm_pair(setg(18, dfr, pp, dwf, D, R, B, 1, D, 1, (int64_t)N.parts * R, R, 0),
                       setg(18, dfr, wf, dp2, B, R, D, D, 1, 1, R, (int64_t)N.parts * R, 0)));
    IEEE_TRY(ieee_colsum_grouped(18, dfr, dbf, B, D, D, 0, st));
  }
  bool have_dglob = false;
  if (N.using_rem) {
    IEEE_TRY(ieee_rem_bwd(F(N.dpart2), F(N.rr), par(N.s_rem_param), gs(N.s_rem_param), F(N.dr), grd(N.s_rem_param),
                          gs(N.s_rem_param), F(N.remwork), B, N.parts, R, 0, st));
    {
      Set3 dw_, dx_;
      set3(dw_, F(N.dr), (int64_t)B * R, F(N.glob), (int64_t)B * R, grd(N.s_rem_pw), gs(N.s_rem_pw), nullptr, 0, R, R, B, 1, R, 1, R, R, 0, 0);
      set3(dx_, F(N.dr), (int64_t)B * R, par(N.s_rem_pw), gs(N.s_rem_pw), F(N.dglob), (int64_t)B * R, nullptr, 0, B, R, R, R, 1, 1, R, R, 0, 0);
      IEEE_TRY(gemm_pair(dw_.s, dx_.s));
    }
    {
      const void* x[3]; void* o[3];
      for (int m = 0; m < 3; ++m) { x[m] = F(N.dr) + (int64_t)m * B * R; o[m] = grd(N.s_rem_pb + m); }
      IEEE_TRY(ieee_colsum_grouped(3, x, o, B, R, R, 0, st));
    }
    have_dglob = true;
    void* zp[6];
    int64_t zn[6];
    for (int m = 0; m < 3; ++m) {
      zp[2 * m] = grd(N.s_rem_qw + m); zn[2 * m] = (int64_t)R * R;
      zp[2 * m + 1] = grd(N.s_rem_qb + m); zn[2 * m + 1] = R;
    }
    IEEE_TRY(ieee_zero_spans(6, zp, zn, st));
  }
  {
    const void *d1[3], *o1[3], *x1[3], *ga[3], *s1[3], *d2[3], *o2[3], *x2[3], *s2[3];
    void *dx1[3], *dx2[3], *dg[3], *db[3];
    for (int m = 0; m < 3; ++m) {
      d1[m] = F(N.dpart2) + (int64_t)m * PB * R; o1[m] = F(N.part) + (int64_t)m * PB * R; x1[m] = F(N.Zp) + (int64_t)m * PB * R;
      dx1[m] = F(N.dZp) + (int64_t)m * PB * R; s1[m] = F(N.sv_p) + m * 2 * R;
      d2[m] = F(N.dglob) + (int64_t)m * B * R; o2[m] = F(N.glob) + (int64_t)m * B * R; x2[m] = F(N.Zg) + (int64_t)m * B * R;
      dx2[m] = F(N.dZg) + (int64_t)m * B * R; s2[m] = F(N.sv_g) + m * 2 * R;
      ga[m] = par(N.s_rg + m); dg[m] = grd(N.s_rg + m); db[m] = grd(N.s_rb + m);
    }
    const int rl = (N.frozen & IEEE_FROZEN_REDUCE) ? 3 : 1;
    IEEE_TRY(ieee_rowbn_bwd(3, d1, o1, x1, ga, s1, dx1, dg, db, PB, R, R, R, R, R, rl, 0, st));
    if (have_dglob) IEEE_TRY(ieee_rowbn_bwd(3, d2, o2, x2, ga, s2, dx2, dg, db, B, R, R, R, R, R, rl, 1, st));
  }
  {
    Set3 dw_, dx_;
    set3(dw_, F(N.dZp), (int64_t)PB * R, F(N.Pp), (int64_t)PB * C, grd(N.s_rw), gs(N.s_rw), nullptr, 0, R, C, PB, 1, R, 1, C, C, 0, 0);
    set3(dx_, F(N.dZp), (int64_t)PB * R, par(N.s_rw), gs(N.s_rw), F(N.dPp), (int64_t)PB * C, nullptr, 0, PB, C, R, R, 1, 1, C, C, 0, 0);
    IEEE_TRY(gemm_pair(dw_.s, dx_.s));
  }
  if (have_dglob) {
    Set3 dw_, dx_;
    set3(dw_, F(N.dZg), (int64_t)B * R, F(N.Gp), BC, grd(N.s_rw), gs(N.s_rw), nullptr, 0, R, C, B, 1, R, 1, C, C, 0, 1);
    set3(dx_, F(N.dZg), (int64_t)B * R, par(N.s_rw), gs(N.s_rw), F(N.dGp), BC, nullptr, 0, B, C, R, R, 1, 1, C, C, 0, 0);
    IEEE_TRY(gemm_pair(dw_.s, dx_.s));
  } else {
    IEEE_HIP(hipMemsetAsync(P(N.dGp), 0, sizeof(float) * (size_t)3 * BC, (hipStream_t)st));
  }
  void* dF = P(N.gbuf[0]);
  const void* Fm = P(N.units[N.blocks.back().c3].a);
  const int mode = !N.interaction ? 2 : (N.attention ? 0 : 1);
  if (N.interaction) {
    if (N.attention) {
      IEEE_TRY(ieee_cim_tail_bwd_datt(F(N.dPp), P(ur.y), F(ur.stats), F(N.datt), dt, B, Hh_, Ww, C, N.parts, st));
      IEEE_TRY(ieee_sigmoid_bwd(F(N.datt), F(N.att), F(N.datt), 3 * BC, st));
      {
        Set3 dw_, dx_;
        set3(dw_, F(N.datt), BC, F(N.Hs), (int64_t)B * N.hid, grd(N.s_ca2), gs(N.s_ca2), nullptr, 0, C, N.hid, B, 1, C, 1, N.hid, N.hid, 0, 0);
        set3(dx_, F(N.datt), BC, par(N.s_ca2), gs(N.s_ca2), F(N.dHs), (int64_t)B * N.hid, nullptr, 0, B, N.hid, C, C, 1, 1, N.hid, N.hid, 0, 0);
        IEEE_TRY(gemm_pair(dw_.s, dx_.s));
      }
      IEEE_TRY(ieee_ca_mix_bwd(F(N.dHs), F(N.Hh), F(N.dH), B, N.hid, st));
      {
        Set3 dw_, dx_;
        set3(dw_, F(N.dH), 2 * (int64_t)B * N.hid, F(N.avgmax), 2 * BC, grd(N.s_ca1), gs(N.s_ca1), nullptr, 0, N.hid, C, 2 * B, 1, N.hid, 1, C, C, 0, 0);
        set3(dx_, F(N.dH), 2 * (int64_t)B * N.hid, par(N.s_ca1), gs(N.s_ca1), F(N.davgmax), 2 * BC, nullptr, 0, 2 * B, C, N.hid, N.hid, 1, 1, C, C, 0, 0);
        IEEE_TRY(gemm_pair(dw_.s, dx_.s));
      }
    }
    const int hb = gbuf_sets() == 3 ? 5 : 0;
    void *g1 = P(N.gbuf[hb + 1]), *g2 = P(N.gbuf[hb + 2]);
    IEEE_TRY(ieee_cim_tail_bwd_g(F(N.dPp), P(uo.y), P(ur.y), F(uo.stats), F(ur.stats), F(N.att), F(N.davgmax),
                                 F(N.davgmax) + BC, 2 * BC, (const int32_t*)P(N.amax), g1, g2, dt, B, Hh_, Ww, C, N.parts,
                                 mode, F(N.bnpart), F(N.bnpart) + 6 * BC, st));
    if (N.tap_base) { IEEE_TRY(tap(uo.name + ".g", g1, out_numel(uo))); IEEE_TRY(tap(ur.name + ".g", g2, out_numel(ur))); }
    IEEE_TRY(bn_bwd(uo, g1, nullptr, g1, nullptr, 0, F(N.bnpart), B));
    IEEE_TRY(bn_bwd(ur, g2, nullptr, g2, nullptr, 0, F(N.bnpart) + 6 * BC, B));
    if (N.tap_base) { IEEE_TRY(tap(uo.name + ".dy", g1, out_numel(uo))); IEEE_TRY(tap(ur.name + ".dy", g2, out_numel(ur))); }
    IEEE_TRY(wgrad(uo, g1, Fm));
    IEEE_TRY(wgrad(ur, g2, P(N.S)));
    IEEE_TRY(wgrad_flush(0));
    IEEE_TRY(dgrad(uo, g1, P(N.gbuf[hb + 3]), nullptr));
    IEEE_TRY(dgrad(ur, g2, P(N.gbuf[hb + 4]), nullptr));
    if (N.tap_base) { IEEE_TRY(tap(uo.name + ".dx", P(N.gbuf[hb + 3]), in_numel(uo))); IEEE_TRY(tap(ur.name + ".dx", P(N.gbuf[hb + 4]), in_numel(ur))); }
    IEEE_TRY(ieee_cim_bwd_combine(P(N.gbuf[hb + 3]), P(N.gbuf[hb + 4]), F(N.dGp), dF, dt, B, Hh_, Ww, C, mode, st));
  } else {
    IEEE_TRY(ieee_cim_tail_bwd_g(F(N.dPp), nullptr, nullptr, nullptr, nullptr, nullptr, nullptr, nullptr, 0, nullptr,
                                 P(N.gbuf[1]), nullptr, dt, B, Hh_, Ww, C, N.parts, 2, nullptr, nullptr, st));
    IEEE_TRY(ieee_cim_bwd_combine(P(N.gbuf[1]), nullptr, F(N.dGp), dF, dt, B, Hh_, Ww, C, 2, st));
  }
  return IEEE_OK;
}

Net* as_net(void* h) { return (Net*)h; }

}

extern "C" int ieee_net_create(int64_t batch, int64_t height, int64_t width, int64_t num_classes, int dtype,
                               int interaction, int attention, int using_rem, void** handle) {
  IEEE_REQUIRE(handle, "net_create: null handle");
  IEEE_REQUIRE(batch >= 1 && batch <= 4096, "net_create: batch %ld out of range", (long)batch);
  IEEE_REQUIRE(height >= 32 && width >= 32 && height % 16 == 0 && width % 16 == 0,
               "net_create: image size %ldx%ld must be a multiple of 16", (long)height, (long)width);
  IEEE_REQUIRE(num_classes >= 1, "net_create: num_classes");
  IEEE_REQUIRE(dtype == IEEE_F32 || dtype == IEEE_BF16, "net_create: dtype");
  Net* n = new Net();
  n->B = (int)batch; n->H = (int)height; n->W = (int)width; n->num_classes = (int)num_classes; n->dtype = dtype;
  n->interaction = interaction; n->attention = attention; n->using_rem = using_rem;
  n->build();
  n->plan();
  *handle = n;
  return IEEE_OK;
}

extern "C" int ieee_net_destroy(void* handle) {
  delete as_net(handle);
  return IEEE_OK;
}

extern "C" int64_t ieee_net_num_slots(void* handle) { return handle ? (int64_t)as_net(handle)->slot_names.size() : -1; }

extern "C" const char* ieee_net_slot_name(void* handle, int64_t i) {
  Net* n = as_net(handle);
  if (!n || i < 0 || i >= (int64_t)n->slot_names.size()) return nullptr;
  return n->slot_names[i].c_str();
}

extern "C" int64_t ieee_net_workspace_bytes(void* handle) { return handle ? (int64_t)as_net(handle)->ws_bytes : -1; }

extern "C" int ieee_net_bind(void* handle, float* params, float* grads, float* buffers, const int64_t* offsets,
                             int64_t num_offsets) {
  Net* n = as_net(handle);
  IEEE_REQUIRE(n && params && buffers && offsets, "net_bind: null pointer");
  IEEE_REQUIRE(num_offsets == (int64_t)n->slot_names.size(), "net_bind: expected %zu offsets, got %ld",
               n->slot_names.size(), (long)num_offsets);
  for (int64_t i = 0; i < num_offsets; ++i) {
    IEEE_REQUIRE(offsets[i] >= 0, "net_bind: slot %s is unbound", n->slot_names[i].c_str());
    n->slot_off[i] = offsets[i];
  }
  for (int t : n->triples)
    IEEE_REQUIRE(offsets[t + 2] - offsets[t + 1] == offsets[t + 1] - offsets[t],
                 "net_bind: modality stride of %s is not uniform", n->slot_names[t].c_str());
  n->params = params;
  n->grads = grads;
  n->buffers = buffers;
  n->bound = true;
  const int es = n->esz();
  for (int training = 0; training < 2; ++training) {
    std::vector<PackDescHost>& tab = training ? n->pack_train : n->pack_eval;
    tab.clear();
    int blocks = 0;
    for (size_t ui = 0; ui < n->units.size(); ++ui) {
      const ConvUnit& u = n->units[ui];
      const bool used = n->interaction || ((int)ui != n->u_one && (int)ui != n->u_rest);
      if (!used) continue;
      for (int mode = 0; mode < 2; ++mode) {
        if (mode == 1 && (!training || !u.need_dgrad)) continue;
        PackDescHost d;
        const int64_t ld = ieee_conv_packed_ld(n->dtype, mode == 0 ? u.Ci : u.Co, u.R, u.S);
        const int rows = mode == 0 ? u.Co : u.Ci;
        d.src_off = n->slot_off[u.s_w];
        d.src_gs = n->slot_off[u.s_w + 1] - n->slot_off[u.s_w];
        d.dst_off = (int64_t)((mode == 0 ? u.wf.off : u.wd.off) / es);
        d.dst_gs = rows * ld;
        d.Co = u.Co; d.Ci = u.Ci; d.R = u.R; d.S = u.S; d.ld = (int)ld; d.mode = mode;
        d.Ci_src = u.Ci_src; d.S_src = u.S_src; d.R_src = u.R_src; d.reserved_ = 0;
        d.block_begin = blocks;
        const bool tiled = mode == 1 && u.R == 1 && u.S == 1 && u.Co % 64 == 0 && u.Ci % 64 == 0 && ld == u.Co &&
                           u.Ci == u.Ci_src;
        const bool k3 = u.R == 3 && u.S == 3 && u.Ci == u.Ci_src && u.S == u.S_src && u.Co % 32 == 0 && u.Ci % 64 == 0 &&
                        ld == 9 * (mode == 0 ? u.Ci : u.Co);
        const int vec = 16 / es;
        const bool conv1 = mode == 0 && u.R == 1 && u.S == 1 && ld == u.Ci && u.Ci == u.Ci_src && (u.Co * ld) % vec == 0 &&
                           d.src_off % 4 == 0 && d.src_gs % 4 == 0;
        d.pad_ = tiled ? 1 : (k3 ? (mode == 0 ? 2 : 3) : (conv1 ? 4 : 0));
        if (training && mode == 0)
          n->units[ui].shadow_ok = conv1 && es == 2 && d.src_off % 8 == 0 && d.src_gs % 8 == 0;
        blocks += tiled ? (u.Co / 64) * (u.Ci / 64)
                        : (k3 ? (mode == 0 ? cdiv(u.Co * (u.Ci / 64), 4) : (u.Co / 32) * (u.Ci / 32))
                              : (conv1 ? cdiv(rows * ld, 256 * vec) : cdiv(rows * ld, 256)));
        tab.push_back(d);
      }
    }
    (training ? n->pack_blocks_train : n->pack_blocks_eval) = blocks;
  }
  {
// ... 241 lines not shown
```

ieee_amd/engine.py:

```python
from __future__ import absolute_import, division, print_function

import datetime
import os
import os.path as osp
import time
from collections import OrderedDict, namedtuple

import numpy as np
import torch
from torch.nn import functional as F

from . import _lib, dist as ddp
from .checkpoint import save_checkpoint
from .losses import (CrossEntropyLoss, DeepSupervision, chunks_short_of_identities, multiModalMarginLossNew,
                     target_out_of_range)
from .meters import AverageMeter, DeferredSummary, MetricMeter
from .metrics import accuracy, compute_distance_matrix, evaluate_rank
from .optim import FusedAdam, FusedSGD

_Entry = namedtuple("_Entry", "model optim sched")
_SUMMARY_3M = ('loss', 'LossX', 'LossM', 'accR', 'lossR', 'accN', 'lossN', 'accT', 'lossT')


def _hms(seconds):
# ... 241 lines not shown
                say('Applying person re-ranking ... (gnn)')
                from .rerank import gnn_distmat
                distmat = gnn_distmat(F.normalize(qf, p=2, dim=1), F.normalize(gf, p=2, dim=1), rerank_k1, rerank_k2)
            elif rerank:
                say('Applying person re-ranking ...')
                from .rerank import re_ranking
                distmat = re_ranking(distmat, compute_distance_matrix(qf, qf, dist_metric),
                                     compute_distance_matrix(gf, gf, dist_metric))
            say('Computing CMC and mAP for {}'.format(dataset_name))
            cmc, mAP = evaluate_rank(distmat, q_pids, g_pids, q_camids, g_camids, use_metric_cuhk03=use_metric_cuhk03)
        say('** Results **')
        say('mAP: {:.2%}'.format(mAP))
        say('CMC curve')
        for r in ranks:
            say('Rank-{:<3}: {:.2%}'.format(r, cmc[r - 1]))
        say('\n')
        if visrank:
            self._visrank(distmat, dataset_name, query_loader, gallery_loader, visrank_topk, save_dir)
        return cmc[0], mAP

    def _test_records(self, name, query_loader, gallery_loader):
        fetch = getattr(self.datamanager, 'fetch_test_loaders', None)
        if callable(fetch):
            return fetch(name)
        recs = [getattr(getattr(ld, 'dataset', None), 'data', None) for ld in (query_loader, gallery_loader)]
        if recs[0] is None or recs[1] is None:
            raise ValueError('visrank needs the query / gallery records of {!r}: give the data manager a '
                             'fetch_test_loaders(name) or use loaders with a .dataset.data list '
                             '(ieee_amd.data.build_loaders)'.format(name))
        return recs[0], recs[1]

    def _visrank(self, distmat, name, query_loader, gallery_loader, topk, save_dir):
        from .reidtools import visualize_ranked_results
        dm = self.datamanager
        visualize_ranked_results(distmat, self._test_records(name, query_loader, gallery_loader),
                                 getattr(dm, 'data_type', 'image'), width=getattr(dm, 'width', 128),
                                 height=getattr(dm, 'height', 256), save_dir=osp.join(save_dir, 'visrank_' + name),
                                 topk=topk)

    def compute_loss(self, criterion, outputs, targets):
        if isinstance(outputs, (tuple, list)):
            return DeepSupervision(criterion, outputs, targets)
        return criterion(outputs, targets)

    def extract_features(self, input, timeids):
        return self.model(input, timeids)

    def parse_data_for_train(self, data):
        return data['img'], data['pid'], data['timeid']

    def parse_data_for_eval(self, data):
        return data['img'], data['pid'], data['camid'], data['timeid']

    def two_stepped_transfer_learning(self, epoch, fixbase_epoch, open_layers, model=None):
        model = self.model if model is None else model
        if model is None:
            return
        freezing = (epoch + 1) <= fixbase_epoch and open_layers is not None
        keep = []
        if freezing:
            keep = [open_layers] if isinstance(open_layers, str) else list(open_layers)
            for layer in keep:
                assert hasattr(model, layer), \
                    '"{}" is not an attribute of the model, please provide the correct name'.format(layer)
            print('* Only train {} (epoch: {}/{})'.format(keep, epoch + 1, fixbase_epoch))
        frozen = []
        for child_name, child in model.named_children():
            flag = (child_name in keep) if freezing else True
            if not flag:
                frozen.append(child_name)
            if not _is_native(model):
                child.train(flag)
            for p in child.parameters():
                p.requires_grad = flag
        if _is_native(model):
            model.set_frozen_children(frozen)

    def _local_batch(self, data):
        world = ddp.world_size()
        rows = int(data['pid'].shape[0])
        if world == 1:
            return data, rows
        stamped = data.get('global_rows') if isinstance(data, dict) else None
        if stamped is not None:
            return data, int(stamped)
        if self.dp_presharded:
            return data, int(self.dp_total_rows) if self.dp_total_rows is not None else ddp.global_rows(rows)
        k = int(getattr(self.datamanager, 'num_instances', 4))
        return ddp.shard_batch(data, k), rows

    def _sync_replicas_once(self):
        if ddp.world_size() > 1 and not self._replicas_synced and self.model is not None:
            ddp.sync_replicas(self.model, self.optimizer)
        self._replicas_synced = True


def _is_native(model):
    return hasattr(model, "native_net")


def batch_error(pids, weight_m, num_classes):
    pids = pids.detach().cpu()
    if weight_m > 0 and chunks_short_of_identities(pids):
        return IndexError('tuple index out of range')
    return target_out_of_range(pids, num_classes)


class _FusedStepMixin(object):

    def _fused_ok(self):
        return _is_native(self.model) and isinstance(self.optimizer, (FusedSGD, FusedAdam)) and self.use_gpu

    def _guard_batch(self, pids, weight_m):
        if self.resident_batch and getattr(self, "_guard_for", None) is pids:
            err = self._guard_err
        else:
            classes = getattr(self.model, "num_classes", None) or self.datamanager.num_train_pids
            err = batch_error(pids, weight_m, classes)
            self._guard_for, self._guard_err = (pids if self.resident_batch else None), err
        if err is not None:
            raise err

    def _fused_step(self, imgs, pids, weight_x, weight_m, margin, eps, total_rows=None):
        lib = _lib.require_gpu()
        m = self.model
        B, _, H, W = imgs[0].shape
        dev = m._flat_params.device
        net = self._step_net = m.native_net(B, H, W)
        pids = pids.to(device=dev, dtype=torch.int64).contiguous()
        m._bump_counters()
        staged = ddp.world_size() > 1 or (os.environ.get("IEEE_FORCE_DP_PATH") == "1" and torch.distributed.is_initialized())
        guard = (not staged) and isinstance(self.optimizer, FusedSGD) and net.dtype == torch.bfloat16
        self._step_guarded = guard
        flags = net.flags_view() if net.dtype == torch.bfloat16 else None
        self._step_flags = flags
        if isinstance(self.optimizer, FusedSGD):
            self.optimizer.skip_flags = flags if guard else None
        if guard:
            bk = getattr(self, "_buf_backup", None)
            if bk is None or bk.shape != m._flat_buffers.shape or bk.device != m._flat_buffers.device or \
                    self._buf_backup_key != (m._flat_buffers._version, id(m)):
                bk = self._buf_backup = m._flat_buffers.detach().clone()
                self._buf_backup_key = (m._flat_buffers._version, id(m))
        logits, feats = net.forward(imgs, training=True)
        C = logits.shape[2]
        if not hasattr(self, "_scratch") or self._scratch[0].shape != logits.shape:
            self._scratch = (torch.empty_like(logits), torch.empty_like(feats),
                             torch.empty(18 * 2 + 3, dtype=torch.float32, device=dev),
                             torch.empty(18 * B * 2, dtype=torch.float32, device=dev),
                             torch.empty(B + 3, dtype=torch.float32, device=dev))
        dl, df, small, work, mwork = self._scratch
        head_loss, head_acc, out3 = small[:18], small[18:36], small[36:39]
        ce_scale = float(weight_x) * ddp.ce_grad_scale(B, total_rows)
        _lib.check(lib.ieee_ce_ls_fwd_bwd(_lib.ptr(logits), _lib.ptr(pids), _lib.ptr(dl), _lib.ptr(head_loss),
                                          _lib.ptr(head_acc), _lib.ptr(work), 18, B, C, float(eps), ce_scale,
                                          _lib.stream()))
        if weight_m > 0:
            _lib.check(lib.ieee_margin3m_fwd_bwd(_lib.ptr(feats), _lib.ptr(pids), _lib.ptr(df), _lib.ptr(out3),
                                                 _lib.ptr(mwork), B, feats.shape[2], float(margin), float(weight_m),
                                                 _lib.stream()))
        else:
            df.zero_()
            out3.zero_()
        def guard_buffers():
            if guard:
                _lib.check(lib.ieee_guard_buffers(_lib.ptr(flags), _lib.ptr(m._flat_buffers), _lib.ptr(self._buf_backup),
                                                  m._flat_buffers.numel(), _lib.stream()))
        if not staged and isinstance(self.optimizer, FusedSGD) and os.environ.get("IEEE_OPT_OVERLAP", "1") != "0":
            main = torch.cuda.current_stream()
            if not hasattr(self, "_opt_stream"):
                self._opt_stream = torch.cuda.Stream(priority=int(os.environ.get("IEEE_OPT_PRIO", "0")))
            helper = self._opt_stream
            for part in range(4):
                net.backward_part_async(dl, df, part)
            helper.wait_stream(main)
            net.side_wait(helper)
            net.backward_part_async(dl, df, 4)
            with torch.cuda.stream(helper):
                guard_buffers()
                for part in range(4):
                    self.optimizer.step_part(part)
            net.side_wait()
            self.optimizer.step_part(4)
            main.wait_stream(helper)
            return small, out3
        overlap = getattr(self, "dp_overlap", None)
        if overlap is None:
            overlap = os.environ.get("IEEE_DP_OVERLAP", "1") != "0"
        if staged and not overlap:
            net.backward(dl, df)
            self._allreduce_ranges(m, [r for ranges in m.grad_part_ranges() for r in ranges])
        elif not staged:
            net.backward(dl, df)
        else:
            main = torch.cuda.current_stream()
            if not hasattr(self, "_comm_stream"):
                prio = os.environ.get("IEEE_COMM_PRIO")
                from . import HW_QUEUES
                prio = int(prio) if prio is not None else (-1 if ddp.world_size() > 1 and HW_QUEUES == 1 else 0)
                self._comm_stream = torch.cuda.Stream(priority=prio)
            comm = self._comm_stream
            by_part = isinstance(self.optimizer, FusedSGD) and os.environ.get("IEEE_OPT_OVERLAP", "1") != "0"
            for part, ranges in enumerate(m.grad_part_ranges()):
                net.backward_part_async(dl, df, part)
                comm.wait_stream(main)
                net.side_wait(comm)
                with torch.cuda.stream(comm):
                    timing = getattr(self, "time_collectives", None)
                    if timing is not None:
                        e0, e1 = torch.cuda.Event(enable_timing=True), torch.cuda.Event(enable_timing=True)
                        e0.record(comm)
                    self._allreduce_ranges(m, ranges)
                    if timing is not None:
                        e1.record(comm)
                        timing.append((part, e0, e1, (4 if self._grad_dtype() == 'fp32' else 2) * sum(b - a for a, b in ranges)))
                    if by_part:
                        self.optimizer.step_part(part)
            net.side_wait()
            main.wait_stream(comm)
            if by_part:
                return small, out3
        guard_buffers()
        self.optimizer.step()
        return small, out3

    def _grad_dtype(self):
        v = getattr(self, "dp_grad_dtype", None) or os.environ.get("IEEE_DP_GRAD_DTYPE", "fp32")
        v = {"float32": "fp32", "bfloat16": "bf16"}.get(v, v)
        if v not in ("fp32", "bf16"):
            raise ValueError("IEEE_DP_GRAD_DTYPE / dp_grad_dtype must be fp32 or bf16, not %r" % (v,))
        return v

    def _allreduce_ranges(self, m, ranges):
        ar = torch.distributed.all_reduce
        if self._grad_dtype() == "fp32":
            handles = [ar(m._flat_grads[a:b], op=torch.distributed.ReduceOp.SUM, async_op=True) for a, b in ranges]
            for h in handles:
                h.wait()
            return
        lib = _lib.load()
        stage = getattr(m, "_flat_grads_bf16", None)
        if stage is None or stage.numel() != m._flat_grads.numel() or stage.device != m._flat_grads.device:
            stage = m._flat_grads_bf16 = torch.empty(m._flat_grads.numel(), dtype=torch.bfloat16, device=m._flat_grads.device)
        for a, b in ranges:
            _lib.check(lib.ieee_grad_pack_bf16(_lib.ptr(m._flat_grads[a:b]), _lib.ptr(stage[a:b]), b - a, _lib.stream()))
        handles = [ar(stage[a:b], op=torch.distributed.ReduceOp.SUM, async_op=True) for a, b in ranges]
        for h in handles:
            h.wait()
        for a, b in ranges:
            _lib.check(lib.ieee_grad_unpack_bf16(_lib.ptr(stage[a:b]), _lib.ptr(m._flat_grads[a:b]), b - a, _lib.stream()))

    _RING = 4

    def _summary_from(self, small, finish, keys):
        ring = getattr(self, "_small_ring", None)
        if ring is None or ring[0][0].numel() != small.numel():
            ring = self._small_ring = [[torch.empty(small.numel(), dtype=small.dtype, pin_memory=True), None]
                                       for _ in range(self._RING)]
            self._ring_at = 0
        slot = ring[self._ring_at]
        self._ring_at = (self._ring_at + 1) % self._RING
        if slot[1] is not None:
            slot[1].resolve()
        host = slot[0]
        host.copy_(small, non_blocking=True)
        flags, hostf = getattr(self, "_step_flags", None), None
        if flags is not None:
            if len(slot) < 3:
                slot.append(torch.zeros(4, dtype=torch.int32, pin_memory=True))
            hostf = slot[2]
            hostf.copy_(flags, non_blocking=True)
        done = torch.cuda.Event()
        done.record(torch.cuda.current_stream(small.device))

        net = getattr(self, "_step_net", None)
        step_idx = self._steps_done = getattr(self, "_steps_done", 0) + 1
        guarded = getattr(self, "_step_guarded", False)

        def read():
            done.synchronize()
            slot[1] = None
            if hostf is not None:
                self._check_bn_range(net, step_idx, tuple(int(v) for v in hostf.tolist()), guarded)
            v = host.numpy().copy()
            hl, ha = v[:18], v[18:36]
            lR, lN, lT = float(hl[0:6].sum()), float(hl[6:12].sum()), float(hl[12:18].sum())
            aR, aN, aT = float(ha[0:6].mean()), float(ha[6:12].mean()), float(ha[12:18].mean())
            return dict(zip(keys, finish(lR, lN, lT, aR, aN, aT, float(v[36]))))

        if not getattr(self, "defer_summary", False):
            return read()
        slot[1] = DeferredSummary(keys, read)
        return slot[1]

    def _check_bn_range(self, net, step, flags, guarded):
        if net is None:
            return
        f_clamp, b_clamp, f_half, b_half = flags
        if f_clamp or b_clamp:
            which = " and ".join(w for w, on in (("forward (sum y, sum y^2 of a conv output)", f_clamp),
                                                 ("backward (sum g, sum g*y)", b_clamp)) if on)
            msg = ("BatchNorm statistics left the range of the fixed-point totals in the %s pass of step %s (or were NaN): "
                   "the int64 totals hold sum y^2 up to 2.7e11 and backward sums up to 4.2e6 per channel; beyond that a tile sum is "
                   "clamped, so the statistics -- and everything computed from them -- are not what fp32 BatchNorm gives. "
                   "Activations / gradients of that size usually mean the run is diverging." % (which, "?" if step is None else step))
            import os
            if os.environ.get("IEEE_BN_STRICT", "0") == "1" or not guarded:
                raise _lib.IeeeAmdError(msg + ("  (IEEE_BN_STRICT=1: raising.)" if guarded else "  The update of that step HAS BEEN APPLIED (no "
                                               "device-side skip in this configuration): restart from the last checkpoint.") +
                                        "  IEEE_BN_TOTALS_TILES=0 selects the per-tile partial-sum path, which has no range limit, "
# ... 116 lines not shown
```

include/ieee_amd.h:

```cpp
#ifndef IEEE_AMD_H
#define IEEE_AMD_H

#include <stdint.h>

#ifdef __cplusplus
extern "C" {
#endif

#define IEEE_OK 0
#define IEEE_ERR_BAD_ARG (-1)
#define IEEE_ERR_HIP (-2)
#define IEEE_ERR_UNSUPPORTED (-3)
#define IEEE_ERR_NO_VALID_QUERY (-4)

#define IEEE_F32 0
#define IEEE_BF16 1

#define IEEE_MAX_GROUPS 18

const char* ieee_last_error(void);
int ieee_version(void);
int ieee_device_is_gfx950(void);

int ieee_sqeuclid_distmat(const void* q, const void* g, int64_t m, int64_t n, int64_t d, int dtype,
// ... 50 lines not shown
                            const float* bn_stats, int relu, int dtype, int64_t groups, int64_t N, int64_t Hi,
                            int64_t Wi, int64_t Ci, int64_t Co, int64_t R, int64_t S, int64_t stride, int64_t pad,
                            int64_t x_gs, int64_t w_gs, int64_t out_gs, void* stream);

int ieee_conv2d_dgrad(const void* dy, const void* w_packed_d, void* dx, const void* addend, int dtype,
                      int64_t groups, int64_t N, int64_t Hi, int64_t Wi, int64_t Ci, int64_t Co, int64_t R,
                      int64_t S, int64_t stride, int64_t pad, int64_t dy_gs, int64_t w_gs, int64_t dx_gs,
                      float* bn_partial, const void* bn_y, const void* bn_mask, const float* bn_stats,
                      int bn_mask_bits, int addend_stride, void* stream);
int ieee_conv2d_dgrad2(const void* dy, const void* w_packed_d, void* dx, const void* addend, int dtype,
                      int64_t groups, int64_t N, int64_t Hi, int64_t Wi, int64_t Ci, int64_t Co, int64_t R,
                      int64_t S, int64_t stride, int64_t pad, int64_t dy_gs, int64_t w_gs, int64_t dx_gs,
                      float* bn_partial, const void* bn_y, const void* bn_mask, const float* bn_stats,
                      int bn_mask_bits, int addend_stride, const void* bn_y2,
                      float* bn_partial2, void* stream);

int64_t ieee_conv2d_wgrad_workspace_bytes(int dtype, int64_t groups, int64_t N, int64_t Ho, int64_t Wo,
                                          int64_t Ci, int64_t Co, int64_t R, int64_t S);
int ieee_conv2d_wgrad(const void* dy, const void* x, float* dw_oihw, void* work, int dtype, int64_t groups,
                      int64_t N, int64_t Hi, int64_t Wi, int64_t Ci, int64_t Co, int64_t R, int64_t S,
                      int64_t stride, int64_t pad, int64_t dy_gs, int64_t x_gs, int64_t dw_gs, int accumulate,
                      void* stream);
int64_t ieee_conv2d_wgrad_fold_ticket_words(void);
int ieee_conv2d_wgrad_fold(const void* dy, const void* x, float* dw_oihw, void* work, int32_t* tickets, int dtype,
                           int64_t groups, int64_t N, int64_t Hi, int64_t Wi, int64_t Ci, int64_t Co, int64_t R, int64_t S,
                           int64_t stride, int64_t pad, int64_t dy_gs, int64_t x_gs, int64_t dw_gs, int accumulate,
                           void* stream);
typedef struct ieee_wgrad_reduce_desc {
  const float* slab;
  float* dw;
  int64_t slab_gs, dw_gs;
  int32_t nsplit, Co, Ci, RS;
  int32_t kind;
  int32_t sl_log2, blocks;
  int32_t accumulate;
  int32_t block_begin;
  int32_t reserved_;
} ieee_wgrad_reduce_desc;
int ieee_conv2d_wgrad_deferred(const void* dy, const void* x, float* dw_oihw, void* work, int dtype, int64_t groups,
                      int64_t N, int64_t Hi, int64_t Wi, int64_t Ci, int64_t Co, int64_t R, int64_t S,
                      int64_t stride, int64_t pad, int64_t dy_gs, int64_t x_gs, int64_t dw_gs, int accumulate,
                      ieee_wgrad_reduce_desc* reduce, void* stream);
int ieee_wgrad_reduce_batch(const ieee_wgrad_reduce_desc* device_descs, int64_t n, int64_t total_blocks, int64_t groups,
                            void* stream);
int ieee_conv2d_wgrad_chained(const void* dy, const void* x, float* dw_oihw, void* work, int dtype, int64_t groups,
                      int64_t N, int64_t Hi, int64_t Wi, int64_t Ci, int64_t Co, int64_t R, int64_t S,
                      int64_t stride, int64_t pad, int64_t dy_gs, int64_t x_gs, int64_t dw_gs, int accumulate,
                      const ieee_wgrad_reduce_desc* prev, ieee_wgrad_reduce_desc* reduce, void* stream);
int ieee_wgrad_reduce_pending(const ieee_wgrad_reduce_desc* pending, int64_t groups, void* stream);


int64_t ieee_bn_partial_floats(int dtype, int64_t M, int64_t C);
int ieee_bn2d_fwd(const void* y, const void* residual, void* out, int dtype, int64_t groups, int64_t M,
                  int64_t C, int64_t act_gs, const float* gamma, const float* beta, int64_t param_gs,
                  float* running_mean, float* running_var, int64_t buf_gs, float* stats, float* partial,
                  float momentum, float eps, int training, int relu, int64_t stats_rblocks, void* relu_bits,
                  void* stream);
int ieee_bn2d_bwd(const void* dout, const void* out_mask, const void* y, void* dy, void* g_out, int dtype,
                  int64_t groups, int64_t M, int64_t C, int64_t act_gs, const float* gamma, int64_t param_gs,
                  const float* stats, float* dgamma, float* dbeta, int64_t grad_gs, float* partial,
                  float* coef, int accumulate, int mask_from_y, int64_t stats_rblocks, void* stream);
int ieee_bn2d_bwd_ev(const void* dout, const void* out_mask, const void* y, void* dy, void* g_out, int dtype,
                  int64_t groups, int64_t M, int64_t C, int64_t act_gs, const float* gamma, int64_t param_gs,
                  const float* stats, float* dgamma, float* dbeta, int64_t grad_gs, float* partial,
                  float* coef, int accumulate, int mask_from_y, int64_t stats_rblocks, void* done_event, void* stream);
int ieee_conv_next_bn_totals(void* totals, int64_t group_stride, int replicas, int* overflow);
typedef struct ieee_conv_extras {
  void* totals;
  int64_t group_stride;
  int32_t replicas;
  int32_t reserved_;
  int* overflow;
  void* start;
  void* stop;
} ieee_conv_extras;
int ieee_conv2d_fwd_ex(const void* x, const void* w_packed, void* y, int dtype, int64_t groups, int64_t N, int64_t Hi,
                       int64_t Wi, int64_t Ci, int64_t Co, int64_t R, int64_t S, int64_t stride, int64_t pad, int64_t x_gs,
                       int64_t w_gs, int64_t y_gs, float* bn_partial, const ieee_conv_extras* extras, void* stream);
int ieee_conv2d_dgrad_ex(const void* dy, const void* w_packed_d, void* dx, const void* addend, int dtype,
                         int64_t groups, int64_t N, int64_t Hi, int64_t Wi, int64_t Ci, int64_t Co, int64_t R,
                         int64_t S, int64_t stride, int64_t pad, int64_t dy_gs, int64_t w_gs, int64_t dx_gs,
                         float* bn_partial, const void* bn_y, const void* bn_mask, const float* bn_stats,
                         int bn_mask_bits, int addend_stride, const void* bn_y2, float* bn_partial2,
                         const ieee_conv_extras* extras, void* stream);
int ieee_bn2d_fwd_totals(const void* y, const void* residual, void* out, int dtype, int64_t groups, int64_t M,
                         int64_t C, int64_t act_gs, const float* gamma, const float* beta, int64_t param_gs,
                         float* running_mean, float* running_var, int64_t buf_gs, float* stats, const void* totals,
                         int replicas, float momentum, float eps, int relu, void* relu_bits, int* overflow, void* stream);
int ieee_bn2d_bwd_totals(const void* dout, const void* out_mask, const void* y, void* dy, void* g_out, int dtype,
                         int64_t groups, int64_t M, int64_t C, int64_t act_gs, const float* gamma, int64_t param_gs,
                         const float* stats, float* dgamma, float* dbeta, int64_t grad_gs, const void* totals,
                         int replicas, int mask_from_y, int* overflow, void* done_event, void* stream);
int ieee_bn2d_bwd_totals_ds(const void* dout, const void* y, const void* y_ds, void* dy, int dtype, int64_t groups, int64_t M,
                            int64_t C, int64_t act_gs, const float* gamma, int64_t param_gs, const float* stats,
                            float* dgamma, float* dbeta, int64_t grad_gs, const void* totals, int replicas, void* totals_ds,
                            int replicas_ds, int* overflow, void* done_event, void* stream);
int ieee_bn2d_bwd_frozen(const void* dout, const void* out_mask, const void* y, void* dy, void* g_out, int dtype,
                         int64_t groups, int64_t M, int64_t C, int64_t act_gs, const float* stats, float* coef,
                         int mask_from_y, void* done_event, void* stream);
int ieee_event_ride_selfcheck(void* stream_a, void* stream_b);

int ieee_nchw_to_nhwc3(const float* x_rgb, const float* x_ni, const float* x_ti, void* out, int dtype,
                       int64_t B, int64_t C, int64_t H, int64_t W, int64_t Cpad, int64_t pad, void* stream);
int ieee_maxpool3x3s2_fwd(const void* x, void* out, uint8_t* argmax, int dtype, int64_t groups, int64_t B,
                          int64_t Hi, int64_t Wi, int64_t C, void* stream);
int ieee_bn_relu_maxpool3x3s2_fwd(const void* y, const float* stats, void* out, uint8_t* argmax, int dtype, int64_t groups,
                                  int64_t B, int64_t Hi, int64_t Wi, int64_t C, void* stream);

int ieee_maxpool3x3s2_bwd(const void* dout, const uint8_t* argmax, void* dx, int dtype, int64_t groups,
                          int64_t B, int64_t Hi, int64_t Wi, int64_t C, void* stream);

int ieee_bn2d_bwd_pooled(const void* dpool, const uint8_t* argmax, const void* y, void* dy, int dtype,
                         int64_t groups, int64_t B, int64_t Hi, int64_t Wi, int64_t C, const float* gamma,
                         int64_t param_gs, const float* stats, float* dgamma, float* dbeta, int64_t grad_gs,
                         float* partial, float* coef, int accumulate, void* stream);

int ieee_gpool_sum_others(const void* F, void* S, float* Gp, int dtype, int64_t B, int64_t H, int64_t W,
                          int64_t C, void* stream);
int ieee_ca_pool(const void* y2, const float* stats2, float* avg, float* mx, int64_t pool_gs, int32_t* argmax,
                 int dtype, int64_t B, int64_t H, int64_t W, int64_t C, void* stream);
int ieee_cim_tail_fwd(const void* y1, const void* y2, const float* stats1, const float* stats2,
                      const float* att, float* parts_out, int dtype, int64_t B, int64_t H, int64_t W,
                      int64_t C, int64_t parts, int mode, void* stream);
int ieee_cim_tail_bwd_datt(const float* dparts, const void* y2, const float* stats2, float* datt, int dtype,
                           int64_t B, int64_t H, int64_t W, int64_t C, int64_t parts, void* stream);
int ieee_cim_tail_bwd_g(const float* dparts, const void* y1, const void* y2, const float* stats1,
                        const float* stats2, const float* att, const float* davg, const float* dmax,
                        int64_t pool_gs, const int32_t* argmax, void* g1, void* g2, int dtype, int64_t B,
                        int64_t H, int64_t W, int64_t C, int64_t parts, int mode, float* bn_partial1,
                        float* bn_partial2, void* stream);
int ieee_cim_bwd_combine(const void* D1, const void* DS, const float* dG, void* dF, int dtype, int64_t B,
                         int64_t H, int64_t W, int64_t C, int mode, void* stream);

int ieee_sgemm_grouped(int64_t groups, const void* const* A, const void* const* B, void* const* C,
                       const void* const* bias, int64_t M, int64_t N, int64_t K, int64_t sam, int64_t sak,
                       int64_t sbn, int64_t sbk, int64_t ldc, float alpha, int relu, int accumulate,
                       void* stream);
int ieee_sgemm_grouped_ws(int64_t groups, const void* const* A, const void* const* B, void* const* C,
                          const void* const* bias, int64_t M, int64_t N, int64_t K, int64_t sam, int64_t sak,
                          int64_t sbn, int64_t sbk, int64_t ldc, float alpha, int relu, int accumulate, void* work,
                          int64_t work_bytes, void* stream);
typedef struct ieee_sgemm_set {
  int64_t groups;
  const void* const* A;
  const void* const* B;
  void* const* C;
  const void* const* bias;
  int64_t M, N, K, sam, sak, sbn, sbk, ldc;
  float alpha;
  int32_t relu, accumulate;
} ieee_sgemm_set;
int ieee_sgemm_grouped_pair_ws(const ieee_sgemm_set* s0, const ieee_sgemm_set* s1, void* work, int64_t work_bytes,
                               void* stream);
int ieee_zero_spans(int64_t count, void* const* ptrs, const int64_t* floats, void* stream);
int ieee_colsum_grouped(int64_t groups, const void* const* X, void* const* out, int64_t M, int64_t N,
                        int64_t ldx, int accumulate, void* stream);
int ieee_rowbn_fwd(int64_t groups, const void* const* x, void* const* out, const void* const* gamma,
                   const void* const* beta, void* const* running_mean, void* const* running_var,
                   void* const* save, int64_t R, int64_t C, int64_t ldx, int64_t ldo, float momentum,
                   float eps, int training, int relu, void* stream);
int ieee_rowbn_bwd(int64_t groups, const void* const* dout, const void* const* out, const void* const* x,
                   const void* const* gamma, const void* const* save, void* const* dx, void* const* dgamma,
                   void* const* dbeta, int64_t R, int64_t C, int64_t lddo, int64_t ldo, int64_t ldx,
                   int64_t lddx, int relu, int accumulate, void* stream);
int ieee_ca_mix_fwd(const float* h, float* hs, int64_t B, int64_t hidden, void* stream);
int ieee_ca_mix_bwd(const float* dhs, const float* h, float* dh, int64_t B, int64_t hidden, void* stream);
int ieee_sigmoid_fwd(float* x, int64_t n, void* stream);
int ieee_sigmoid_bwd(const float* datt, const float* att, float* dz, int64_t n, void* stream);
int ieee_rem_fwd(const float* part, const float* r, const float* param, int64_t param_gs, float* out,
                 int64_t B, int64_t parts, int64_t D, void* stream);
int ieee_rem_bwd(const float* dout, const float* r, const float* param, int64_t param_gs, float* dr,
                 float* dparam, int64_t grad_gs, float* work, int64_t B, int64_t parts, int64_t D,
                 int accumulate, void* stream);
int ieee_l2norm_fwd(const float* x, float* y, float* norms, int64_t rows, int64_t D, void* stream);
int ieee_l2norm_bwd(const float* dy, const float* y, const float* norms, float* dx, int64_t rows, int64_t D,
                    int accumulate, void* stream);

int ieee_ce_ls_fwd_bwd(const float* logits, const int64_t* targets, float* dlogits, float* head_loss,
                       float* head_acc, float* work, int64_t heads, int64_t B, int64_t C, float eps,
                       float grad_scale, void* stream);
int ieee_margin3m_fwd_bwd(const float* feats, const int64_t* pids, float* dfeats, float* out3, float* work,
                          int64_t B, int64_t D, float margin, float grad_scale, void* stream);
int ieee_sgd_nesterov_step_ex(float* params, const float* grads, float* momentum_buf, int64_t n, float lr, float momentum,
                              float weight_decay, int nesterov, void* shadow_bf16, const int* skip_flags, void* stream);
int ieee_guard_buffers(const int* flags, float* buffers, float* backup, int64_t n, void* stream);
int ieee_sgd_nesterov_step(float* params, const float* grads, float* momentum_buf, int64_t n, float lr,
                           float momentum, float weight_decay, int nesterov, void* stream);
int ieee_grad_pack_bf16(const float* grads, void* out_bf16, int64_t n, void* stream);
int ieee_grad_unpack_bf16(const void* in_bf16, float* grads, int64_t n, void* stream);
int ieee_adam_step(float* params, const float* grads, float* exp_avg, float* exp_avg_sq, float* max_exp_avg_sq,
                   int64_t n, float lr, float beta1, float beta2, float eps, float weight_decay, int64_t step,
                   void* stream);

int64_t ieee_rerank_workspace_bytes(int64_t Q, int64_t G, int64_t k1);
int ieee_rerank(const float* q_g_dist, const float* q_q_dist, const float* g_g_dist, int64_t Q, int64_t G,
                int64_t k1, int64_t k2, double lambda_value, float* out, void* work, int64_t work_bytes,
                void* stream);
int64_t ieee_rerank_sparse_workspace_bytes(int64_t Q, int64_t G, int64_t k1, int64_t k2);
int ieee_rerank_sparse(const float* q_g_dist, const float* q_q_dist, const float* g_g_dist, int64_t Q, int64_t G,
                       int64_t k1, int64_t k2, double lambda_value, float* out, void* work, int64_t work_bytes,
                       void* stream);
int ieee_rerank_sparse_layout(int64_t Q, int64_t G, int64_t k1, int64_t k2, int64_t* fields);
int64_t ieee_gnn_rerank_workspace_bytes(int64_t Q, int64_t G, int64_t d, int64_t k1, int64_t k2, int precision);
int ieee_gnn_rerank(const float* xq, const float* xg, int64_t Q, int64_t G, int64_t d, int64_t k1, int64_t k2,
                    int precision, float* out, void* work, int64_t work_bytes, void* stream);
int ieee_gnn_rerank_layout(int64_t Q, int64_t G, int64_t d, int64_t k1, int64_t k2, int precision, int64_t* fields);

int ieee_resize_flip_normalize(const uint8_t* src, float* dst, uint8_t* tmp, int64_t N, int64_t Hs, int64_t Ws,
                               int64_t Ho, int64_t Wo, const int32_t* bounds_h, const int32_t* kk_h, int64_t ksize_h,
                               const int32_t* bounds_v, const int32_t* kk_v, int64_t ksize_v, int64_t ybox_first,
                               int64_t tmp_rows, const uint8_t* flip, const float* mean3, const float* std3,
                               void* stream);

int ieee_net_create(int64_t batch, int64_t height, int64_t width, int64_t num_classes, int dtype,
                    int interaction, int attention, int using_rem, void** handle);
int ieee_net_destroy(void* handle);
int64_t ieee_net_num_slots(void* handle);
const char* ieee_net_slot_name(void* handle, int64_t i);
int64_t ieee_net_workspace_bytes(void* handle);
int ieee_net_bind(void* handle, float* params, float* grads, float* buffers, const int64_t* offsets,
                  int64_t num_offsets);
int ieee_net_forward(void* handle, void* workspace, const float* x_rgb, const float* x_ni, const float* x_ti,
                     int training, float* logits, float* feats, void* stream);
int ieee_net_backward(void* handle, void* workspace, const float* dlogits, const float* dfeats, void* stream);
int ieee_net_backward_part(void* handle, void* workspace, const float* dlogits, const float* dfeats, int part,
                           void* stream);
int ieee_net_backward_part_async(void* handle, void* workspace, const float* dlogits, const float* dfeats, int part,
                                 void* stream);
int ieee_net_side_wait(void* handle, void* workspace, void* waiting_stream, int is_launch_stream);
int ieee_net_sync_streams(void* handle, void* stream);
#define IEEE_FROZEN_BACKBONE 1
#define IEEE_FROZEN_CONV_ONE 2
#define IEEE_FROZEN_CONV_REST 4
#define IEEE_FROZEN_REDUCE 8
#define IEEE_FROZEN_FC_R 16
#define IEEE_FROZEN_FC_N 32
#define IEEE_FROZEN_FC_T 64
int ieee_net_set_frozen(void* handle, int mask);
int ieee_net_bn_overflow(void* handle, int* out4);
int64_t ieee_net_bn_flags_offset(void* handle);
int ieee_net_set_bn_totals(void* handle, int on);
int ieee_net_set_shadow(void* handle, const void* shadow_bf16);
int ieee_net_eval_cache(void* handle, int keep);
int ieee_net_profile(void* handle, int enable, double* out6);
int ieee_conv_profile_events(void* start, void* stop);
int ieee_net_tensor(void* handle, const char* name, int64_t* byte_offset, int64_t* numel, int* dtype);
int ieee_net_debug_taps(void* handle, void* buffer, int64_t bytes);
int ieee_net_debug_tap(void* handle, const char* name, int64_t* byte_offset, int64_t* numel, int* dtype);

#ifdef __cplusplus
}
#endif
#endif
```

Measured before the change: 4404.

## Fuse head kernels: GEMM epilogues, rider blocks, chained rowbn, combined losses

Folds several small head kernels into fewer launches. Sigmoid, mix and REM epilogues move into the GEMM and split-k reduce. Colsum, zeroing and dparam reduction ride as extra blocks in the paired GEMM kernel. Split-k reduce and bias are folded into a chained two-problem rowbn forward, with a matching chained backward. CE and margin losses share one kernel, and l2norm gains a dual output. This targets launch overhead and extra memory passes in the latency-bound head, at the cost of more complex kernels and possibly uneven block work.

```diff
diff --git a/ieee_amd/_lib.py b/ieee_amd/_lib.py
--- a/ieee_amd/_lib.py
+++ b/ieee_amd/_lib.py
@@ -63,6 +63,30 @@
                 ("sbk", c_int64), ("ldc", c_int64), ("alpha", c_float), ("relu", ctypes.c_int32), ("accumulate", ctypes.c_int32)]
 
 
+class PairRiders(ctypes.Structure):
+    _fields_ = [("cs_groups", c_int64), ("cs_X", c_void_p), ("cs_out", c_void_p), ("cs_M", c_int64), ("cs_N", c_int64),
+                ("cs_ldx", c_int64), ("z_count", c_int64), ("z_ptrs", c_void_p), ("z_floats", c_void_p),
+                ("cs_accumulate", ctypes.c_int32), ("defer", ctypes.c_int32), ("splitk", ctypes.c_int32 * 2),
+                ("slab", c_void_p * 2), ("dp_partial", c_void_p), ("dp_out", c_void_p), ("dp_grad_gs", c_int64), ("dp_B", c_int64),
+                ("dp_accumulate", ctypes.c_int32), ("reserved_", ctypes.c_int32)]
+
+
+class SgemmTail(ctypes.Structure):
+    _fields_ = [("mix_out", c_void_p), ("rem_part", c_void_p), ("rem_out", c_void_p), ("rem_param", c_void_p),
+                ("rem_param_gs", c_int64), ("rem_parts", c_int64)]
+
+
+class RowBnProb(ctypes.Structure):
+    _fields_ = [("x", c_void_p), ("out", c_void_p), ("save", c_void_p), ("R", c_int64), ("ldx", c_int64), ("ldo", c_int64),
+                ("slab", c_void_p), ("splitk", c_int64), ("bias", c_void_p)]
+
+
+class RowBnBwdProb(ctypes.Structure):
+    _fields_ = [("dout", c_void_p), ("out", c_void_p), ("x", c_void_p), ("save", c_void_p), ("dx", c_void_p), ("R", c_int64),
+                ("lddo", c_int64), ("ldo", c_int64), ("ldx", c_int64), ("lddx", c_int64), ("accumulate", ctypes.c_int32),
+                ("reserved_", ctypes.c_int32)]
+
+
 class IeeeAmdError(RuntimeError):
     pass
 
diff --git a/ieee_amd/csrc/head.hip b/ieee_amd/csrc/head.hip
--- a/ieee_amd/csrc/head.hip
+++ b/ieee_amd/csrc/head.hip
@@ -14,6 +14,12 @@
   int relu, accumulate;
   int splitk, kchunk, vec_a, vec_b;
   float* slab;
+  int sigmoid;
+  float* mix_out;
+  int mix_half;
+  const float* rem_part; float* rem_out; const float* rem_param;
+  int64_t rem_param_gs;
+  int rem_parts;
 };
 
 typedef float SgemmStage[64][33];
@@ -143,6 +149,7 @@
         float* c = C + (int64_t)m * a.ldc + n + r;
         if (a.accumulate) v += *c;
         if (a.relu) v = fmaxf(v, 0.f);
+        if (a.sigmoid) v = 1.0f / (1.0f + expf(-v));
         *c = v;
       }
     }
@@ -167,9 +174,8 @@
   }
 }
 
-__device__ __forceinline__ void sgemm_splitk_reduce_one(const SgemmArgs& a, int g, int64_t i) {
+__device__ __forceinline__ float sgemm_splitk_reduce_elem(const SgemmArgs& a, int g, int64_t i) {
   const int64_t mn = (int64_t)a.M * a.N;
-  if (i >= mn) return;
   const float* S = a.slab + (int64_t)g * a.splitk * mn + i;
   float s = 0.f;
   for (int k = 0; k < a.splitk; ++k) s += S[k * mn];
@@ -180,7 +186,27 @@
   float* c = (float*)a.C.p[g] + (int64_t)m * a.ldc + n;
   if (a.accumulate) v += *c;
   if (a.relu) v = fmaxf(v, 0.f);
+  if (a.sigmoid) v = 1.0f / (1.0f + expf(-v));
   *c = v;
+  return v;
+}
+__device__ __forceinline__ void sgemm_splitk_reduce_one(const SgemmArgs& a, int g, int64_t i) {
+  const int64_t mn = (int64_t)a.M * a.N;
+  if (a.mix_out != nullptr) {
+    const int64_t hn = (int64_t)a.mix_half * a.N;
+    if (i >= hn) return;
+    const float v0 = sgemm_splitk_reduce_elem(a, g, i), v1 = sgemm_splitk_reduce_elem(a, g, hn + i);
+    a.mix_out[g * hn + i] = v0 + v1;
+    return;
+  }
+  if (i >= mn) return;
+  const float v = sgemm_splitk_reduce_elem(a, g, i);
+  if (a.rem_out != nullptr) {
+    const float sc = 2.0f * a.rem_param[g * a.rem_param_gs];
+    const int m = (int)(i / a.N), n = (int)(i - (int64_t)m * a.N);
+    const int64_t base = ((int64_t)g * a.M + m) * a.rem_parts * a.N + n;
+    for (int p = 0; p < a.rem_parts; ++p) a.rem_out[base + (int64_t)p * a.N] = a.rem_part[base + (int64_t)p * a.N] + sc * v;
+  }
 }
 __global__ __launch_bounds__(256) void sgemm_splitk_reduce_kernel(SgemmArgs a) {
   sgemm_splitk_reduce_one(a, blockIdx.y, (int64_t)blockIdx.x * blockDim.x + threadIdx.x);
@@ -220,6 +246,54 @@
   *o = a.accumulate ? *o + s : s;
 }
 
+struct PairRiders {
+  ColsumArgs cs;
+  int cs_bx, cs_blocks;
+  ZeroArgs z;
+  int z_bx, z_blocks;
+  const float* dp_partial; float* dparam; int64_t dp_gs; int dp_B, dp_accumulate;
+};
+__global__ __launch_bounds__(256) void sgemm_grouped2r_kernel(SgemmArgs a0, SgemmArgs a1, PairDims d, int blocks1, PairRiders r) {
+  __shared__ float As[2][64][33];
+  __shared__ float Bs[2][64][33];
+  int b = blockIdx.x;
+  if (b < d.blocks0) {
+    sgemm_tile(a0, b % d.gx0, (b / d.gx0) % d.gy0, b / (d.gx0 * d.gy0), As, Bs);
+    return;
+  }
+  b -= d.blocks0;
+  if (b < blocks1) {
+    sgemm_tile(a1, b % d.gx1, (b / d.gx1) % d.gy1, b / (d.gx1 * d.gy1), As, Bs);
+    return;
+  }
+  b -= blocks1;
+  if (b < r.cs_blocks) {
+    const int g = b / r.cs_bx;
+    const int n = (b - g * r.cs_bx) * 256 + threadIdx.x;
+    if (n >= r.cs.N) return;
+    const float* X = (const float*)r.cs.X.p[g];
+    float s = 0.f;
+    for (int m = 0; m < r.cs.M; ++m) s += X[(int64_t)m * r.cs.ldx + n];
+    float* o = (float*)r.cs.out.p[g] + n;
+    *o = r.cs.accumulate ? *o + s : s;
+    return;
+  }
+  b -= r.cs_blocks;
+  if (b >= r.z_blocks) {
+    const int z = threadIdx.x;
+    if (z >= 3) return;
+    float s = 0.f;
+    for (int q = 0; q < r.dp_B; ++q) s += r.dp_partial[(int64_t)z * r.dp_B + q];
+    float* o = r.dparam + z * r.dp_gs;
+    *o = r.dp_accumulate ? *o + s : s;
+    return;
+  }
+  const int span = b / r.z_bx;
+  float* p = (float*)r.z.p.p[span];
+  const int64_t n = r.z.n[span];
+  for (int64_t i = (int64_t)(b - span * r.z_bx) * 256 + threadIdx.x; i < n; i += (int64_t)r.z_bx * 256) p[i] = 0.f;
+}
+
 struct RowBnArgs {
   PtrTab x, out, gamma, beta, rmean, rvar, save;
   int R, C;
@@ -234,14 +308,25 @@
   for (int y = 0; y < RB_TY; ++y) s += red[y][tx];
   return s;
 }
-__global__ __launch_bounds__(256) void rowbn_fwd_kernel(RowBnArgs a) {
-  __shared__ float red[RB_TY][RB_TX];
-  const int g = blockIdx.y;
+__device__ __forceinline__ void rowbn_fwd_body(const RowBnArgs& a, int g, const float* slab, int splitk, const float* bias,
+                                               float (*red)[RB_TX]) {
   const int tx = threadIdx.x % RB_TX, ty = threadIdx.x / RB_TX;
   const int c = blockIdx.x * RB_TX + tx;
   const bool ok = c < a.C;
-  const float* x = (const float*)a.x.p[g];
+  float* x = (float*)a.x.p[g];
   float* out = (float*)a.out.p[g];
+  if (slab != nullptr && ok) {
+    const int64_t mn = (int64_t)a.R * a.C;
+    const float* S = slab + (int64_t)g * splitk * mn + c;
+    const float bv = bias ? bias[c] : 0.f;
+#pragma unroll 2
+    for (int r = ty; r < a.R; r += RB_TY) {
+      float s = 0.f;
+      for (int k = 0; k < splitk; ++k) s += S[k * mn + (int64_t)r * a.C];
+      if (bias) s += bv;
+      x[(int64_t)r * a.ldx + c] = s;
+    }
+  }
   float mean, invstd;
   if (a.training) {
     float s = 0.f;
@@ -285,6 +370,26 @@
     out[(int64_t)r * a.ldo + c] = v;
   }
 }
+__global__ __launch_bounds__(256) void rowbn_fwd_kernel(RowBnArgs a) {
+  __shared__ float red[RB_TY][RB_TX];
+  rowbn_fwd_body(a, blockIdx.y, nullptr, 0, nullptr, red);
+}
+struct RowBnChainArgs {
+  RowBnArgs a[2];
+  PtrTab bias[2];
+  const float* slab[2];
+  int splitk[2];
+  int nprob;
+};
+__global__ __launch_bounds__(256) void rowbn_fwd_chain_kernel(RowBnChainArgs c) {
+  __shared__ float red[RB_TY][RB_TX];
+  const int g = blockIdx.y;
+  rowbn_fwd_body(c.a[0], g, c.slab[0], c.splitk[0], (const float*)c.bias[0].p[g], red);
+  if (c.nprob > 1) {
+    __syncthreads();
+    rowbn_fwd_body(c.a[1], g, c.slab[1], c.splitk[1], (const float*)c.bias[1].p[g], red);
+  }
+}
 
 struct RowBnBwdArgs {
   PtrTab dout, out, x, gamma, save, dx, dgamma, dbeta;
@@ -292,9 +397,7 @@
   int64_t lddo, ldo, ldx, lddx;
   int relu, accumulate;
 };
-__global__ __launch_bounds__(256) void rowbn_bwd_kernel(RowBnBwdArgs a) {
-  __shared__ float red[2][RB_TY][RB_TX];
-  const int g = blockIdx.y;
+__device__ __forceinline__ void rowbn_bwd_body(const RowBnBwdArgs& a, int g, float (*red)[RB_TY][RB_TX]) {
   const int tx = threadIdx.x % RB_TX, ty = threadIdx.x / RB_TX;
   const int c = blockIdx.x * RB_TX + tx;
   const bool ok = c < a.C;
@@ -337,6 +440,17 @@
     dx[(int64_t)r * a.lddx + c] = ga * invstd * (gq - c1 - xh * c2);
   }
 }
+__global__ __launch_bounds__(256) void rowbn_bwd_kernel(RowBnBwdArgs a) {
+  __shared__ float red[2][RB_TY][RB_TX];
+  rowbn_bwd_body(a, blockIdx.y, red);
+}
+struct RowBnBwdChainArgs { RowBnBwdArgs a[2]; };
+__global__ __launch_bounds__(256) void rowbn_bwd_chain_kernel(RowBnBwdChainArgs c) {
+  __shared__ float red[2][RB_TY][RB_TX];
+  rowbn_bwd_body(c.a[0], blockIdx.y, red);
+  __syncthreads();
+  rowbn_bwd_body(c.a[1], blockIdx.y, red);
+}
 
 __global__ void add_halves_kernel(const float* h, float* hs, int64_t half, int64_t gs_in, int64_t gs_out) {
   const int z = blockIdx.y;
@@ -399,7 +513,7 @@
   *o = accumulate ? *o + s : s;
 }
 
-__global__ void l2norm_fwd_kernel(const float* x, float* y, float* norms, int64_t rows, int D) {
+__global__ void l2norm_fwd_kernel(const float* x, float* y, float* y2, float* norms, int64_t rows, int D) {
   const int64_t row = (int64_t)blockIdx.x * 4 + (threadIdx.x >> 6);
   if (row >= rows) return;
   const int lane = threadIdx.x & 63;
@@ -407,7 +521,11 @@
   for (int k = lane; k < D; k += 64) { const float v = x[row * D + k]; s += v * v; }
   s = wave_sum(s);
   const float nrm = fmaxf(sqrtf(s), 1e-12f);
-  for (int k = lane; k < D; k += 64) y[row * D + k] = x[row * D + k] / nrm;
+  for (int k = lane; k < D; k += 64) {
+    const float v = x[row * D + k] / nrm;
+    y[row * D + k] = v;
+    if (y2 != nullptr) y2[row * D + k] = v;
+  }
   if (lane == 0) norms[row] = nrm;
 }
 __global__ void l2norm_bwd_kernel(const float* dy, const float* y, const float* norms, float* dx, int64_t rows, int D,
@@ -426,9 +544,9 @@
   }
 }
 
-__global__ void ce_rows_kernel(const float* logits, const int64_t* target, float* rowloss, int* correct,
-                               float* dlogits, int heads, int B, int C, float eps, float gscale) {
-  const int64_t row = (int64_t)blockIdx.x * 4 + (threadIdx.x >> 6);
+__device__ __forceinline__ void ce_rows_body(int block, const float* logits, const int64_t* target, float* rowloss, int* correct,
+                                             float* dlogits, int heads, int B, int C, float eps, float gscale) {
+  const int64_t row = (int64_t)block * 4 + (threadIdx.x >> 6);
   if (row >= (int64_t)heads * B) return;
   const int lane = threadIdx.x & 63;
   const int b = (int)(row % B);
@@ -461,9 +579,12 @@
     }
   }
 }
-__global__ void ce_heads_kernel(const float* rowloss, const int* correct, float* head_loss, float* head_acc,
-                                int heads, int B) {
-  const int h = blockIdx.x * blockDim.x + threadIdx.x;
+__global__ void ce_rows_kernel(const float* logits, const int64_t* target, float* rowloss, int* correct,
+                               float* dlogits, int heads, int B, int C, float eps, float gscale) {
+  ce_rows_body(blockIdx.x, logits, target, rowloss, correct, dlogits, heads, B, C, eps, gscale);
+}
+__device__ __forceinline__ void ce_heads_body(int h, const float* rowloss, const int* correct, float* head_loss, float* head_acc,
+                                              int heads, int B) {
   if (h >= heads) return;
   float s = 0.f;
   int k = 0;
@@ -471,9 +592,13 @@
   head_loss[h] = s / B;
   head_acc[h] = 100.0f * k / B;
 }
-
-__global__ __launch_bounds__(256) void margin3m_kernel(const float* feats, const int64_t* pids, float* dfeats,
-                                                       float* terms, int B, int D, float margin, float gscale) {
+__global__ void ce_heads_kernel(const float* rowloss, const int* correct, float* head_loss, float* head_acc,
+                                int heads, int B) {
+  ce_heads_body(blockIdx.x * blockDim.x + threadIdx.x, rowloss, correct, head_loss, head_acc, heads, B);
+}
+
+__device__ __forceinline__ void margin3m_body(int ch, const float* feats, const int64_t* pids, float* dfeats,
+                                              float* terms, int B, int D, float margin, float gscale) {
   __shared__ float red[3][256];
   __shared__ int s_cnt[256];
   __shared__ int s_sel;
@@ -492,7 +617,6 @@
   const int csize = (B + n - 1) / n;
   const int nchunks = (B + csize - 1) / csize;
   const int nuse = nchunks < n ? nchunks : n;
-  const int ch = blockIdx.x;
   const int64_t BD = (int64_t)B * D;
   if (ch == 0 && t == 0) { terms[B] = (float)n; terms[B + 1] = (float)nchunks; terms[B + 2] = (float)nuse; }
   const int r0 = ch * csize, r1 = min(B, r0 + csize), rows = r1 - r0;
@@ -549,12 +673,38 @@
     }
   }
 }
-__global__ void margin3m_sum_kernel(const float* terms, float* out, int B) {
-  if (threadIdx.x != 0) return;
+__global__ __launch_bounds__(256) void margin3m_kernel(const float* feats, const int64_t* pids, float* dfeats,
+                                                       float* terms, int B, int D, float margin, float gscale) {
+  margin3m_body(blockIdx.x, feats, pids, dfeats, terms, B, D, margin, gscale);
+}
+__device__ __forceinline__ void margin3m_sum_body(const float* terms, float* out, int B) {
   const int nuse = (int)terms[B + 2];
   float loss = 0.f;
   for (int c = 0; c < nuse; ++c) loss += terms[c];
   out[0] = loss; out[1] = terms[B]; out[2] = terms[B + 1];
+}
+__global__ void margin3m_sum_kernel(const float* terms, float* out, int B) {
+  if (threadIdx.x != 0) return;
+  margin3m_sum_body(terms, out, B);
+}
+struct LossArgs {
+  const float* logits; const int64_t* target; float* rowloss; int* correct; float* dlogits; float* head_loss; float* head_acc;
+  int heads, B, C; float eps, ce_scale;
+  const float* feats; float* dfeats; float* terms; float* out3;
+  int D; float margin, m_scale;
+  int ce_blocks;
+};
+__global__ __launch_bounds__(256) void losses_rows_kernel(LossArgs a) {
+  const int b = blockIdx.x;
+  if (b < a.ce_blocks) ce_rows_body(b, a.logits, a.target, a.rowloss, a.correct, a.dlogits, a.heads, a.B, a.C, a.eps, a.ce_scale);
+  else margin3m_body(b - a.ce_blocks, a.feats, a.target, a.dfeats, a.terms, a.B, a.D, a.margin, a.m_scale);
+}
+__global__ void losses_sums_kernel(LossArgs a) {
+  if (blockIdx.x + 1 < gridDim.x) {
+    ce_heads_body(blockIdx.x * blockDim.x + threadIdx.x, a.rowloss, a.correct, a.head_loss, a.head_acc, a.heads, a.B);
+  } else if (threadIdx.x == 0) {
+    margin3m_sum_body(a.terms, a.out3, a.B);
+  }
 }
 
 __device__ __forceinline__ void sgd_one(float& w, float g, float& buf, float lr, float momentum, float wd, int nesterov) {
@@ -677,7 +827,8 @@
   fill_tab(&a.bias, bias, (int)groups);
   a.M = (int)M; a.N = (int)N; a.K = (int)K;
   a.sam = sam; a.sak = sak; a.sbn = sbn; a.sbk = sbk; a.ldc = ldc;
-  a.alpha = alpha; a.relu = relu; a.accumulate = accumulate;
+  a.alpha = alpha; a.relu = relu; a.accumulate = accumulate; a.sigmoid = 0;
+  a.mix_out = nullptr; a.mix_half = 0; a.rem_part = nullptr; a.rem_out = nullptr; a.rem_param = nullptr; a.rem_param_gs = 0; a.rem_parts = 0;
   a.vec_a = (sak == 1 && sam % 4 == 0 && aligned16(A, (int)groups)) ? 1
             : (sam == 1 && sak % 4 == 0 && aligned16(A, (int)groups)) ? 2 : 0;
   a.vec_b = (sbk == 1 && sbn % 4 == 0 && aligned16(B, (int)groups)) ? 1
@@ -767,6 +918,174 @@
   return launch_status("rowbn_bwd_kernel");
 }
 
+extern "C" int ieee_sgemm_grouped_sigmoid_ws(int64_t groups, const void* const* A, const void* const* B, void* const* C,
+                                             const void* const* bias, int64_t M, int64_t N, int64_t K, int64_t sam, int64_t sak,
+                                             int64_t sbn, int64_t sbk, int64_t ldc, float alpha, void* work, int64_t work_bytes,
+                                             void* stream) {
+  SgemmArgs a;
+  IEEE_TRY(sgemm_fill(a, groups, A, B, C, bias, M, N, K, sam, sak, sbn, sbk, ldc, alpha, 0, 0, work, work_bytes));
+  a.sigmoid = 1;
+  dim3 grid(cdiv(N, 64), cdiv(M, 64), (unsigned)(groups * a.splitk));
+  sgemm_grouped_kernel<<<grid, 256, 0, (hipStream_t)stream>>>(a);
+  IEEE_TRY(launch_status("sgemm_grouped_kernel"));
+  if (a.splitk > 1) {
+    sgemm_splitk_reduce_kernel<<<dim3(cdiv(M * N, 256), (unsigned)groups), 256, 0, (hipStream_t)stream>>>(a);
+    return launch_status("sgemm_splitk_reduce_kernel");
+  }
+  return IEEE_OK;
+}
+
+extern "C" int ieee_sgemm_grouped_tail_ws(int64_t groups, const void* const* A, const void* const* B, void* const* C,
+                                          const void* const* bias, int64_t M, int64_t N, int64_t K, int64_t sam, int64_t sak,
+                                          int64_t sbn, int64_t sbk, int64_t ldc, float alpha, int relu, const ieee_sgemm_tail* tail,
+                                          void* work, int64_t work_bytes, void* stream) {
+  IEEE_REQUIRE(tail && groups == 3, "sgemm_grouped_tail: needs a tail and the 3 modality groups");
+  IEEE_REQUIRE(!tail->mix_out != !tail->rem_out, "sgemm_grouped_tail: exactly one of mix_out / rem_out");
+  IEEE_REQUIRE(ldc == N, "sgemm_grouped_tail: C must be dense");
+  SgemmArgs a;
+  IEEE_TRY(sgemm_fill(a, groups, A, B, C, bias, M, N, K, sam, sak, sbn, sbk, ldc, alpha, relu, 0, work, work_bytes));
+  const float* c0 = (const float*)C[0];
+  for (int g = 1; g < 3; ++g) IEEE_REQUIRE((const float*)C[g] == c0 + (int64_t)g * M * N, "sgemm_grouped_tail: C groups must be contiguous");
+  if (tail->mix_out) {
+    IEEE_REQUIRE(M % 2 == 0, "sgemm_grouped_tail: mix needs an even M");
+  } else {
+    IEEE_REQUIRE(tail->rem_part && tail->rem_param && tail->rem_parts >= 1, "sgemm_grouped_tail: bad REM tail");
+  }
+  const bool fold = a.splitk > 1;
+  if (fold) {
+    if (tail->mix_out) { a.mix_out = tail->mix_out; a.mix_half = (int)(M / 2); }
+    else { a.rem_part = tail->rem_part; a.rem_out = tail->rem_out; a.rem_param = tail->rem_param; a.rem_param_gs = tail->rem_param_gs; a.rem_parts = (int)tail->rem_parts; }
+  }
+  dim3 grid(cdiv(N, 64), cdiv(M, 64), (unsigned)(groups * a.splitk));
+  sgemm_grouped_kernel<<<grid, 256, 0, (hipStream_t)stream>>>(a);
+  IEEE_TRY(launch_status("sgemm_grouped_kernel"));
+  if (fold) {
+    sgemm_splitk_reduce_kernel<<<dim3(cdiv(M * N, 256), (unsigned)groups), 256, 0, (hipStream_t)stream>>>(a);
+    return launch_status("sgemm_splitk_reduce_kernel");
+  }
+  if (tail->mix_out) return ieee_ca_mix_fwd(c0, tail->mix_out, M / 2, N, stream);
+  return ieee_rem_fwd(tail->rem_part, c0, tail->rem_param, tail->rem_param_gs, tail->rem_out, M, tail->rem_parts, N, stream);
+}
+
+extern "C" int ieee_sgemm_grouped_pair_ex(const ieee_sgemm_set* s0, const ieee_sgemm_set* s1, ieee_pair_riders* rd, void* work,
+                                          int64_t work_bytes, void* stream) {
+  IEEE_REQUIRE(s0 && rd, "sgemm_grouped_pair_ex: null problem set or riders");
+  IEEE_REQUIRE(rd->cs_groups >= 0 && rd->cs_groups <= MAXG && rd->z_count >= 0 && rd->z_count <= MAXG,
+               "sgemm_grouped_pair_ex: rider counts out of range");
+  IEEE_REQUIRE(rd->cs_groups == 0 || (rd->cs_X && rd->cs_out && rd->cs_M > 0 && rd->cs_N > 0), "sgemm_grouped_pair_ex: bad column sums");
+  IEEE_REQUIRE(rd->z_count == 0 || (rd->z_ptrs && rd->z_floats), "sgemm_grouped_pair_ex: bad zero spans");
+  const int64_t half = work ? (work_bytes / 2) & ~(int64_t)255 : 0;
+  SgemmArgs a0, a1;
+  IEEE_TRY(sgemm_fill(a0, s0->groups, s0->A, s0->B, s0->C, s0->bias, s0->M, s0->N, s0->K, s0->sam, s0->sak, s0->sbn, s0->sbk, s0->ldc,
+                      s0->alpha, s0->relu, s0->accumulate, work, half));
+  PairDims d;
+  d.gx0 = cdiv(s0->N, 64); d.gy0 = cdiv(s0->M, 64); d.blocks0 = d.gx0 * d.gy0 * (int)(s0->groups * a0.splitk);
+  int blocks1 = 0;
+  if (s1) {
+    IEEE_TRY(sgemm_fill(a1, s1->groups, s1->A, s1->B, s1->C, s1->bias, s1->M, s1->N, s1->K, s1->sam, s1->sak, s1->sbn, s1->sbk, s1->ldc,
+                        s1->alpha, s1->relu, s1->accumulate, work ? (char*)work + half : nullptr, half));
+    d.gx1 = cdiv(s1->N, 64); d.gy1 = cdiv(s1->M, 64);
+    blocks1 = d.gx1 * d.gy1 * (int)(s1->groups * a1.splitk);
+  } else {
+    a1 = a0; a1.splitk = 1;
+    d.gx1 = d.gy1 = 1;
+  }
+  PairRiders r;
+  fill_tab(&r.cs.X, rd->cs_X, (int)rd->cs_groups);
+  fill_tab(&r.cs.out, (const void* const*)rd->cs_out, (int)rd->cs_groups);
+  r.cs.M = (int)rd->cs_M; r.cs.N = (int)rd->cs_N; r.cs.ldx = rd->cs_ldx; r.cs.accumulate = rd->cs_accumulate;
+  r.cs_bx = rd->cs_groups ? (int)cdiv(rd->cs_N, 256) : 1;
+  r.cs_blocks = rd->cs_groups ? r.cs_bx * (int)rd->cs_groups : 0;
+  fill_tab(&r.z.p, (const void* const*)rd->z_ptrs, (int)rd->z_count);
+  int64_t most = 1;
+  for (int i = 0; i < MAXG; ++i) { r.z.n[i] = i < rd->z_count ? rd->z_floats[i] : 0; most = r.z.n[i] > most ? r.z.n[i] : most; }
+  r.z_bx = (int)(cdiv(most, 1024) > 256 ? 256 : cdiv(most, 1024));
+  const int zblocks = rd->z_count ? r.z_bx * (int)rd->z_count : 0;
+  r.z_blocks = zblocks;
+  r.dp_partial = rd->dp_partial; r.dparam = rd->dp_out; r.dp_gs = rd->dp_grad_gs; r.dp_B = (int)rd->dp_B; r.dp_accumulate = rd->dp_accumulate;
+  IEEE_REQUIRE(!rd->dp_partial || (rd->dp_out && rd->dp_B > 0), "sgemm_grouped_pair_ex: bad REM parameter sum");
+  const int dpblocks = rd->dp_partial ? 1 : 0;
+  const SgemmArgs* as[2] = {&a0, &a1};
+  const ieee_sgemm_set* ss[2] = {s0, s1};
+  bool defer[2] = {false, false};
+  for (int i = 0; i < 2; ++i) {
+    rd->splitk[i] = ss[i] ? as[i]->splitk : 1;
+    rd->slab[i] = ss[i] ? (void*)as[i]->slab : nullptr;
+    if (ss[i] && ((rd->defer >> i) & 1) && as[i]->splitk > 1) {
+      IEEE_REQUIRE(ss[i]->alpha == 1.0f && !ss[i]->relu && !ss[i]->accumulate && ss[i]->ldc == ss[i]->N,
+                   "sgemm_grouped_pair_ex: set %d cannot defer its split-K reduction", i);
+      defer[i] = true;
+    } else {
+      rd->splitk[i] = 1;
+    }
+  }
+  sgemm_grouped2r_kernel<<<dim3((unsigned)(d.blocks0 + blocks1 + r.cs_blocks + zblocks + dpblocks)), 256, 0, (hipStream_t)stream>>>(a0, a1, d, blocks1, r);
+  IEEE_TRY(launch_status("sgemm_grouped2r_kernel"));
+  const bool red0 = a0.splitk > 1 && !defer[0], red1 = s1 && a1.splitk > 1 && !defer[1];
+  if (red0 || red1) {
+    PairReduceDims q;
+    q.rb0 = red0 ? cdiv(s0->M * s0->N, 256) : 1;
+    q.blocks0 = red0 ? q.rb0 * (int)s0->groups : 0;
+    q.rb1 = red1 ? cdiv(s1->M * s1->N, 256) : 1;
+    const int rblocks1 = red1 ? q.rb1 * (int)s1->groups : 0;
+    sgemm_splitk_reduce2_kernel<<<dim3((unsigned)(q.blocks0 + rblocks1)), 256, 0, (hipStream_t)stream>>>(a0, a1, q);
+    return launch_status("sgemm_splitk_reduce2_kernel");
+  }
+  return IEEE_OK;
+}
+
+extern "C" int ieee_rowbn_fwd_chain(int64_t nprob, int64_t groups, const ieee_rowbn_prob* probs, const void* const* gamma,
+                                    const void* const* beta, void* const* running_mean, void* const* running_var, int64_t C,
+                                    float momentum, float eps, int training, int relu, void* stream) {
+  IEEE_REQUIRE((nprob == 1 || nprob == 2) && groups >= 1 && groups <= MAXG && probs && gamma && beta, "rowbn_fwd_chain: bad arguments");
+  IEEE_REQUIRE(training || (running_mean && running_var), "rowbn_fwd_chain: eval mode needs running stats");
+  RowBnChainArgs c;
+  c.nprob = (int)nprob;
+  for (int i = 0; i < 2; ++i) {
+    const ieee_rowbn_prob& p = probs[i < nprob ? i : 0];
+    IEEE_REQUIRE(p.x && p.out && p.R > 0, "rowbn_fwd_chain: bad problem");
+    IEEE_REQUIRE(p.splitk <= 1 || (p.slab && p.ldx == C), "rowbn_fwd_chain: slabs need a dense x");
+    RowBnArgs& a = c.a[i];
+    fill_tab(&a.x, p.x, (int)groups);
+    fill_tab(&a.out, (const void* const*)p.out, (int)groups);
+    fill_tab(&a.gamma, gamma, (int)groups);
+    fill_tab(&a.beta, beta, (int)groups);
+    fill_tab(&a.rmean, (const void* const*)running_mean, (int)groups);
+    fill_tab(&a.rvar, (const void* const*)running_var, (int)groups);
+    fill_tab(&a.save, (const void* const*)p.save, (int)groups);
+    fill_tab(&c.bias[i], p.splitk > 1 ? p.bias : nullptr, (int)groups);
+    a.R = (int)p.R; a.C = (int)C; a.ldx = p.ldx; a.ldo = p.ldo; a.momentum = momentum; a.eps = eps;
+    a.training = training; a.relu = relu;
+    c.slab[i] = p.splitk > 1 ? (const float*)p.slab : nullptr;
+    c.splitk[i] = (int)p.splitk;
+  }
+  rowbn_fwd_chain_kernel<<<dim3(cdiv(C, RB_TX), (unsigned)groups), 256, 0, (hipStream_t)stream>>>(c);
+  return launch_status("rowbn_fwd_chain_kernel");
+}
+
+extern "C" int ieee_rowbn_bwd_chain(int64_t groups, const ieee_rowbn_bwd_prob* probs, const void* const* gamma, void* const* dgamma,
+                                    void* const* dbeta, int64_t C, int relu, void* stream) {
+  IEEE_REQUIRE(groups >= 1 && groups <= MAXG && probs && gamma && dgamma && dbeta, "rowbn_bwd_chain: bad arguments");
+  RowBnBwdChainArgs c;
+  for (int i = 0; i < 2; ++i) {
+    const ieee_rowbn_bwd_prob& p = probs[i];
+    IEEE_REQUIRE(p.dout && p.out && p.x && p.save && p.dx && p.R > 0, "rowbn_bwd_chain: bad problem");
+    RowBnBwdArgs& a = c.a[i];
+    fill_tab(&a.dout, p.dout, (int)groups);
+    fill_tab(&a.out, p.out, (int)groups);
+    fill_tab(&a.x, p.x, (int)groups);
+    fill_tab(&a.gamma, gamma, (int)groups);
+    fill_tab(&a.save, p.save, (int)groups);
+    fill_tab(&a.dx, (const void* const*)p.dx, (int)groups);
+    fill_tab(&a.dgamma, (const void* const*)dgamma, (int)groups);
+    fill_tab(&a.dbeta, (const void* const*)dbeta, (int)groups);
+    a.R = (int)p.R; a.C = (int)C; a.lddo = p.lddo; a.ldo = p.ldo; a.ldx = p.ldx; a.lddx = p.lddx;
+    a.relu = relu; a.accumulate = p.accumulate;
+  }
+  rowbn_bwd_chain_kernel<<<dim3(cdiv(C, RB_TX), (unsigned)groups), 256, 0, (hipStream_t)stream>>>(c);
+  return launch_status("rowbn_bwd_chain_kernel");
+}
+
 extern "C" int ieee_ca_mix_fwd(const float* h, float* hs, int64_t B, int64_t hidden, void* stream) {
   IEEE_REQUIRE(h && hs, "ca_mix_fwd: null pointer");
   add_halves_kernel<<<dim3(ewb(B * hidden), 3), 256, 0, (hipStream_t)stream>>>(h, hs, B * hidden, 2 * B * hidden,
@@ -808,9 +1127,21 @@
   return launch_status("rem_dparam_kernel");
 }
 
+extern "C" int ieee_rem_bwd_partial(const float* dout, const float* r, const float* param, int64_t param_gs, float* dr, float* work,
+                                    int64_t B, int64_t parts, int64_t D, void* stream) {
+  IEEE_REQUIRE(dout && r && param && dr && work, "rem_bwd_partial: null pointer");
+  rem_bwd_kernel<<<dim3((unsigned)B, 3), 256, 0, (hipStream_t)stream>>>(dout, r, param, param_gs, dr, work, (int)B, (int)parts, (int)D);
+  return launch_status("rem_bwd_kernel");
+}
+
 extern "C" int ieee_l2norm_fwd(const float* x, float* y, float* norms, int64_t rows, int64_t D, void* stream) {
   IEEE_REQUIRE(x && y && norms, "l2norm_fwd: null pointer");
-  l2norm_fwd_kernel<<<cdiv(rows, 4), 256, 0, (hipStream_t)stream>>>(x, y, norms, rows, (int)D);
+  l2norm_fwd_kernel<<<cdiv(rows, 4), 256, 0, (hipStream_t)stream>>>(x, y, nullptr, norms, rows, (int)D);
+  return launch_status("l2norm_fwd_kernel");
+}
+extern "C" int ieee_l2norm_fwd_dual(const float* x, float* y, float* y2, float* norms, int64_t rows, int64_t D, void* stream) {
+  IEEE_REQUIRE(x && y && y2 && norms, "l2norm_fwd_dual: null pointer");
+  l2norm_fwd_kernel<<<cdiv(rows, 4), 256, 0, (hipStream_t)stream>>>(x, y, y2, norms, rows, (int)D);
   return launch_status("l2norm_fwd_kernel");
 }
 extern "C" int ieee_l2norm_bwd(const float* dy, const float* y, const float* norms, float* dx, int64_t rows,
@@ -844,6 +1175,26 @@
   IEEE_TRY(launch_status("margin3m_kernel"));
   margin3m_sum_kernel<<<1, 64, 0, st>>>(work, out3, (int)B);
   return launch_status("margin3m_sum_kernel");
+}
+
+extern "C" int ieee_losses_fwd_bwd(const float* logits, const int64_t* targets, float* dlogits, float* head_loss, float* head_acc,
+                                   float* ce_work, int64_t heads, int64_t B, int64_t C, float eps, float ce_grad_scale,
+                                   const float* feats, float* dfeats, float* out3, float* m_work, int64_t D, float margin,
+                                   float m_grad_scale, void* stream) {
+  IEEE_REQUIRE(logits && targets && head_loss && head_acc && ce_work, "losses_fwd_bwd: null pointer");
+  IEEE_REQUIRE(feats && out3 && m_work, "losses_fwd_bwd: null pointer");
+  IEEE_REQUIRE(heads >= 1 && B >= 1 && C >= 1 && D >= 1 && B <= 65535, "losses_fwd_bwd: shape out of range");
+  hipStream_t st = (hipStream_t)stream;
+  LossArgs a;
+  a.logits = logits; a.target = targets; a.rowloss = ce_work; a.correct = (int*)(ce_work + heads * B); a.dlogits = dlogits;
+  a.head_loss = head_loss; a.head_acc = head_acc;
+  a.heads = (int)heads; a.B = (int)B; a.C = (int)C; a.eps = eps; a.ce_scale = ce_grad_scale;
+  a.feats = feats; a.dfeats = dfeats; a.terms = m_work; a.out3 = out3; a.D = (int)D; a.margin = margin; a.m_scale = m_grad_scale;
+  a.ce_blocks = (int)cdiv(heads * B, 4);
+  losses_rows_kernel<<<(unsigned)(a.ce_blocks + B), 256, 0, st>>>(a);
+  IEEE_TRY(launch_status("losses_rows_kernel"));
+  losses_sums_kernel<<<(unsigned)(cdiv(heads, 64) + 1), 64, 0, st>>>(a);
+  return launch_status("losses_sums_kernel");
 }
 
 __global__ void adam_kernel(float* __restrict__ p, const float* __restrict__ g, float* __restrict__ m,
diff --git a/ieee_amd/csrc/net.hip b/ieee_amd/csrc/net.hip
--- a/ieee_amd/csrc/net.hip
+++ b/ieee_amd/csrc/net.hip
@@ -825,6 +825,19 @@
                                      s->alpha, s->relu, s->accumulate, P(n.gemm_work), half, st));
     return IEEE_OK;
   }
+  static int head_fused() {
+    const char* e = getenv("IEEE_HEAD_FUSED");
+    const int v = e ? atoi(e) : 1;
+    return (v == 0 || !head_pairs()) ? 0 : (v == 2 ? 2 : 1);
+  }
+  int gemm_pair_ex(const ieee_sgemm_set* s0, const ieee_sgemm_set* s1, ieee_pair_riders& rd) {
+    return ieee_sgemm_grouped_pair_ex(s0, s1, &rd, P(n.gemm_work), (int64_t)n.gemm_work.numel * 4, st);
+  }
+  static ieee_pair_riders riders_colsum(int64_t groups, const void* const* X, void* const* out, int64_t M, int64_t N, int64_t ldx) {
+    ieee_pair_riders rd{};
+    rd.cs_groups = groups; rd.cs_X = X; rd.cs_out = out; rd.cs_M = M; rd.cs_N = N; rd.cs_ldx = ldx;
+    return rd;
+  }
   bool late_pack_pending = false;
   bool use_shadow = false;
   int forward(const float* xr, const float* xn, const float* xt, int training, float* logits_out, float* feats_out) {
@@ -976,6 +989,7 @@
   const int64_t BC = (int64_t)B * C;
   IEEE_TRY(ieee_gpool_sum_others(Fm, N.interaction ? P(N.S) : nullptr, F(N.Gp), dt, B, Hh_, Ww, C, st));
   const int mode = !N.interaction ? 2 : (N.attention ? 0 : 1);
+  const int hf = head_fused();
   if (N.interaction) {
     IEEE_TRY(conv(uo, Fm, training != 0));
     if (!eval_cached) IEEE_TRY(bn(uo, nullptr, nullptr, 1, training));
@@ -984,12 +998,27 @@
     if (N.attention) {
       IEEE_TRY(ieee_ca_pool(P(ur.y), F(ur.stats), F(N.avgmax), F(N.avgmax) + BC, 2 * BC, (int32_t*)P(N.amax), dt, B, Hh_,
                             Ww, C, st));
-      IEEE_TRY(gemm3(F(N.avgmax), 2 * BC, par(N.s_ca1), gs(N.s_ca1), F(N.Hh), 2 * B * N.hid, nullptr, 0, 2 * B, N.hid, C,
-                     C, 1, C, 1, N.hid, 1, 0));
-      IEEE_TRY(ieee_ca_mix_fwd(F(N.Hh), F(N.Hs), B, N.hid, st));
-      IEEE_TRY(gemm3(F(N.Hs), (int64_t)B * N.hid, par(N.s_ca2), gs(N.s_ca2), F(N.att), BC, nullptr, 0, B, C, N.hid,
-                     N.hid, 1, N.hid, 1, C, 0, 0));
-      IEEE_TRY(ieee_sigmoid_fwd(F(N.att), 3 * BC, st));
+      if (hf) {
+        const void *a_[3], *b_[3]; void* c_[3];
+        for (int m = 0; m < 3; ++m) { a_[m] = F(N.avgmax) + m * 2 * BC; b_[m] = par(N.s_ca1) + m * gs(N.s_ca1); c_[m] = F(N.Hh) + (int64_t)m * 2 * B * N.hid; }
+        const ieee_sgemm_tail tail = {F(N.Hs), nullptr, nullptr, nullptr, 0, 0};
+        IEEE_TRY(ieee_sgemm_grouped_tail_ws(3, a_, b_, c_, nullptr, 2 * B, N.hid, C, C, 1, C, 1, N.hid, 1.0f, 1, &tail, P(N.gemm_work),
+                                            (int64_t)N.gemm_work.numel * 2, st));
+      } else {
+        IEEE_TRY(gemm3(F(N.avgmax), 2 * BC, par(N.s_ca1), gs(N.s_ca1), F(N.Hh), 2 * B * N.hid, nullptr, 0, 2 * B, N.hid, C,
+                       C, 1, C, 1, N.hid, 1, 0));
+        IEEE_TRY(ieee_ca_mix_fwd(F(N.Hh), F(N.Hs), B, N.hid, st));
+      }
+      if (hf) {
+        const void *a_[3], *b_[3]; void* c_[3];
+        for (int m = 0; m < 3; ++m) { a_[m] = F(N.Hs) + (int64_t)m * B * N.hid; b_[m] = par(N.s_ca2) + m * gs(N.s_ca2); c_[m] = F(N.att) + m * BC; }
+        IEEE_TRY(ieee_sgemm_grouped_sigmoid_ws(3, a_, b_, c_, nullptr, B, C, N.hid, N.hid, 1, N.hid, 1, C, 1.0f, P(N.gemm_work),
+                                               (int64_t)N.gemm_work.numel * 2, st));
+      } else {
+        IEEE_TRY(gemm3(F(N.Hs), (int64_t)B * N.hid, par(N.s_ca2), gs(N.s_ca2), F(N.att), BC, nullptr, 0, B, C, N.hid,
+                       N.hid, 1, N.hid, 1, C, 0, 0));
+        IEEE_TRY(ieee_sigmoid_fwd(F(N.att), 3 * BC, st));
+      }
     }
     IEEE_TRY(ieee_cim_tail_fwd(P(uo.y), P(ur.y), F(uo.stats), F(ur.stats), F(N.att), F(N.Pp), dt, B, Hh_, Ww, C, N.parts,
                                mode, st));
@@ -1013,14 +1042,30 @@
       s1[m] = F(N.sv_g) + m * 2 * R; s2[m] = F(N.sv_p) + m * 2 * R;
     }
     const int tr_red = (training && !(N.frozen & IEEE_FROZEN_REDUCE)) ? 1 : 0;
-    IEEE_TRY(ieee_rowbn_fwd(3, x1, o1, ga, be, rm, rv, s1, B, R, R, R, N.bn_mom, N.bn_eps, tr_red, 1, st));
-    IEEE_TRY(ieee_rowbn_fwd(3, x2, o2, ga, be, rm, rv, s2, PB, R, R, R, N.bn_mom, N.bn_eps, tr_red, 1, st));
+    if (hf) {
+      const ieee_rowbn_prob pr[2] = {{x1, o1, s1, B, R, R, nullptr, 1, nullptr}, {x2, o2, s2, PB, R, R, nullptr, 1, nullptr}};
+      IEEE_TRY(ieee_rowbn_fwd_chain(2, 3, pr, ga, be, rm, rv, R, N.bn_mom, N.bn_eps, tr_red, 1, st));
+    } else {
+      IEEE_TRY(ieee_rowbn_fwd(3, x1, o1, ga, be, rm, rv, s1, B, R, R, R, N.bn_mom, N.bn_eps, tr_red, 1, st));
+      IEEE_TRY(ieee_rowbn_fwd(3, x2, o2, ga, be, rm, rv, s2, PB, R, R, R, N.bn_mom, N.bn_eps, tr_red, 1, st));
+    }
   }
   const float* p2 = F(N.part);
   if (N.using_rem) {
-    IEEE_TRY(gemm3(F(N.glob), (int64_t)B * R, par(N.s_rem_pw), gs(N.s_rem_pw), F(N.rr), (int64_t)B * R, par(N.s_rem_pb),
-                   gs(N.s_rem_pb), B, R, R, R, 1, R, 1, R, 0, 0));
-    IEEE_TRY(ieee_rem_fwd(F(N.part), F(N.rr), par(N.s_rem_param), gs(N.s_rem_param), F(N.part2), B, N.parts, R, st));
+    if (hf) {
+      const void *a_[3], *b_[3], *bi_[3]; void* c_[3];
+      for (int m = 0; m < 3; ++m) {
+        a_[m] = F(N.glob) + (int64_t)m * B * R; b_[m] = par(N.s_rem_pw) + m * gs(N.s_rem_pw); bi_[m] = par(N.s_rem_pb) + m * gs(N.s_rem_pb);
+        c_[m] = F(N.rr) + (int64_t)m * B * R;
+      }
+      const ieee_sgemm_tail tail = {nullptr, F(N.part), F(N.part2), par(N.s_rem_param), gs(N.s_rem_param), N.parts};
+      IEEE_TRY(ieee_sgemm_grouped_tail_ws(3, a_, b_, c_, bi_, B, R, R, R, 1, R, 1, R, 1.0f, 0, &tail, P(N.gemm_work),
+                                          (int64_t)N.gemm_work.numel * 2, st));
+    } else {
+      IEEE_TRY(gemm3(F(N.glob), (int64_t)B * R, par(N.s_rem_pw), gs(N.s_rem_pw), F(N.rr), (int64_t)B * R, par(N.s_rem_pb),
+                     gs(N.s_rem_pb), B, R, R, R, 1, R, 1, R, 0, 0));
+      IEEE_TRY(ieee_rem_fwd(F(N.part), F(N.rr), par(N.s_rem_param), gs(N.s_rem_param), F(N.part2), B, N.parts, R, st));
+    }
     p2 = F(N.part2);
   }
   const int D = N.cdim;
@@ -1038,9 +1083,9 @@
         sv[g] = F(N.sv_fc) + g * 2 * D;
         o[g] = training ? (void*)(F(N.featcat) + (int64_t)m * B * R + i * D) : (void*)(F(N.fcall) + eval_off[m] + i * D);
       }
+    const int fz = (N.frozen / IEEE_FROZEN_FC_R) & 7;
     IEEE_TRY(ieee_sgemm_grouped_ws(18, a, w, c, bi, B, D, R, (int64_t)N.parts * R, 1, R, 1, D, 1.0f, 0, 0, P(N.gemm_work),
                                    (int64_t)N.gemm_work.numel * 2, st));
-    const int fz = (N.frozen / IEEE_FROZEN_FC_R) & 7;
     if (!training || fz == 0 || fz == 7) {
       IEEE_TRY(ieee_rowbn_fwd(18, xs, o, ga, be, rm, rv, sv, B, D, D, training ? R : 3 * R, N.bn_mom, N.bn_eps,
                               (training && fz == 0) ? 1 : 0, 1, st));
@@ -1069,6 +1114,7 @@
     IEEE_TRY(ieee_sgemm_grouped_ws(18, a, w, c, bi, B, NC, D, R, 1, D, 1, NC, 1.0f, 0, 0, P(N.gemm_work),
                                    (int64_t)N.gemm_work.numel * 2, st));
   }
+  if (hf) return ieee_l2norm_fwd_dual(F(N.featcat), F(N.featn), feats_out, F(N.norms), 3 * (int64_t)B, R, st);
   IEEE_TRY(ieee_l2norm_fwd(F(N.featcat), F(N.featn), F(N.norms), 3 * (int64_t)B, R, st));
   IEEE_HIP(hipMemcpyAsync(feats_out, F(N.featn), sizeof(float) * (size_t)3 * B * R, hipMemcpyDeviceToDevice, (hipStream_t)st));
   return IEEE_OK;
@@ -1202,6 +1248,7 @@
   const ConvUnit &uo = N.units[N.u_one], &ur = N.units[N.u_rest];
   const int Hh_ = uo.Hi, Ww = uo.Wi;
   const float* p2 = N.using_rem ? F(N.part2) : F(N.part);
+  const int hf = head_fused();
   IEEE_TRY(ieee_l2norm_bwd(dfeats, F(N.featn), F(N.norms), F(N.dfeatcat), 3 * (int64_t)B, R, 0, st));
   {
     const void *dl[18], *fe[18], *w[18], *xs[18], *ga[18], *sv[18], *dfr[18], *pp[18];
@@ -1222,8 +1269,16 @@
         pp[g] = p2 + (int64_t)m * PB * R + i * R;
         dp2[g] = F(N.dpart2) + (int64_t)m * PB * R + i * R;
       }
-    IEEE_TRY(gemm_pair(setg(18, dl, fe, dw, NC, D, B, 1, NC, 1, R, D, 0), setg(18, dl, w, dfc, B, D, NC, NC, 1, 1, D, R, 1)));
-    IEEE_TRY(ieee_colsum_grouped(18, dl, db, B, NC, NC, 0, st));
+    {
+      const ieee_sgemm_set s0 = setg(18, dl, fe, dw, NC, D, B, 1, NC, 1, R, D, 0), s1 = setg(18, dl, w, dfc, B, D, NC, NC, 1, 1, D, R, 1);
+      if (hf) {
+        ieee_pair_riders rd = riders_colsum(18, dl, db, B, NC, NC);
+        IEEE_TRY(gemm_pair_ex(&s0, &s1, rd));
+      } else {
+        IEEE_TRY(gemm_pair(s0, s1));
+        IEEE_TRY(ieee_colsum_grouped(18, dl, db, B, NC, NC, 0, st));
+      }
+    }
     const int fz = (N.frozen / IEEE_FROZEN_FC_R) & 7;
     if (fz == 0 || fz == 7) {
       IEEE_TRY(ieee_rowbn_bwd(18, (const void* const*)dfc, fe, xs, ga, sv, dx, dg, dbe, B, D, R, R, D, D, fz ? 3 : 1, 0, st));
@@ -1234,33 +1289,50 @@
     }
     const void* wf[18];
     for (int g = 0; g < 18; ++g) wf[g] = par(N.s_fcw[g]);
-    IEEE_TRY(gemm_pair(setg(18, dfr, pp, dwf, D, R, B, 1, D, 1, (int64_t)N.parts * R, R, 0),
-                       setg(18, dfr, wf, dp2, B, R, D, D, 1, 1, R, (int64_t)N.parts * R, 0)));
-    IEEE_TRY(ieee_colsum_grouped(18, dfr, dbf, B, D, D, 0, st));
+    {
+      const ieee_sgemm_set s0 = setg(18, dfr, pp, dwf, D, R, B, 1, D, 1, (int64_t)N.parts * R, R, 0),
+                           s1 = setg(18, dfr, wf, dp2, B, R, D, D, 1, 1, R, (int64_t)N.parts * R, 0);
+      if (hf) {
+        ieee_pair_riders rd = riders_colsum(18, dfr, dbf, B, D, D);
+        IEEE_TRY(gemm_pair_ex(&s0, &s1, rd));
+      } else {
+        IEEE_TRY(gemm_pair(s0, s1));
+        IEEE_TRY(ieee_colsum_grouped(18, dfr, dbf, B, D, D, 0, st));
+      }
+    }
   }
   bool have_dglob = false;
   if (N.using_rem) {
-    IEEE_TRY(ieee_rem_bwd(F(N.dpart2), F(N.rr), par(N.s_rem_param), gs(N.s_rem_param), F(N.dr), grd(N.s_rem_param),
-                          gs(N.s_rem_param), F(N.remwork), B, N.parts, R, 0, st));
+    if (hf) {
+      IEEE_TRY(ieee_rem_bwd_partial(F(N.dpart2), F(N.rr), par(N.s_rem_param), gs(N.s_rem_param), F(N.dr), F(N.remwork), B, N.parts, R, st));
+    } else {
+      IEEE_TRY(ieee_rem_bwd(F(N.dpart2), F(N.rr), par(N.s_rem_param), gs(N.s_rem_param), F(N.dr), grd(N.s_rem_param),
+                            gs(N.s_rem_param), F(N.remwork), B, N.parts, R, 0, st));
+    }
     {
       Set3 dw_, dx_;
       set3(dw_, F(N.dr), (int64_t)B * R, F(N.glob), (int64_t)B * R, grd(N.s_rem_pw), gs(N.s_rem_pw), nullptr, 0, R, R, B, 1, R, 1, R, R, 0, 0);
       set3(dx_, F(N.dr), (int64_t)B * R, par(N.s_rem_pw), gs(N.s_rem_pw), F(N.dglob), (int64_t)B * R, nullptr, 0, B, R, R, R, 1, 1, R, R, 0, 0);
-      IEEE_TRY(gemm_pair(dw_.s, dx_.s));
-    }
-    {
       const void* x[3]; void* o[3];
       for (int m = 0; m < 3; ++m) { x[m] = F(N.dr) + (int64_t)m * B * R; o[m] = grd(N.s_rem_pb + m); }
-      IEEE_TRY(ieee_colsum_grouped(3, x, o, B, R, R, 0, st));
+      void* zp[6];
+      int64_t zn[6];
+      for (int m = 0; m < 3; ++m) {
+        zp[2 * m] = grd(N.s_rem_qw + m); zn[2 * m] = (int64_t)R * R;
+        zp[2 * m + 1] = grd(N.s_rem_qb + m); zn[2 * m + 1] = R;
+      }
+      if (hf) {
+        ieee_pair_riders rd = riders_colsum(3, x, o, B, R, R);
+        rd.z_count = 6; rd.z_ptrs = zp; rd.z_floats = zn;
+        rd.dp_partial = F(N.remwork); rd.dp_out = grd(N.s_rem_param); rd.dp_grad_gs = gs(N.s_rem_param); rd.dp_B = B;
+        IEEE_TRY(gemm_pair_ex(&dw_.s, &dx_.s, rd));
+      } else {
+        IEEE_TRY(gemm_pair(dw_.s, dx_.s));
+        IEEE_TRY(ieee_colsum_grouped(3, x, o, B, R, R, 0, st));
+        IEEE_TRY(ieee_zero_spans(6, zp, zn, st));
+      }
     }
     have_dglob = true;
-    void* zp[6];
-    int64_t zn[6];
-    for (int m = 0; m < 3; ++m) {
-      zp[2 * m] = grd(N.s_rem_qw + m); zn[2 * m] = (int64_t)R * R;
-      zp[2 * m + 1] = grd(N.s_rem_qb + m); zn[2 * m + 1] = R;
-    }
-    IEEE_TRY(ieee_zero_spans(6, zp, zn, st));
   }
   {
     const void *d1[3], *o1[3], *x1[3], *ga[3], *s1[3], *d2[3], *o2[3], *x2[3], *s2[3];
@@ -1273,8 +1345,13 @@
       ga[m] = par(N.s_rg + m); dg[m] = grd(N.s_rg + m); db[m] = grd(N.s_rb + m);
     }
     const int rl = (N.frozen & IEEE_FROZEN_REDUCE) ? 3 : 1;
-    IEEE_TRY(ieee_rowbn_bwd(3, d1, o1, x1, ga, s1, dx1, dg, db, PB, R, R, R, R, R, rl, 0, st));
-    if (have_dglob) IEEE_TRY(ieee_rowbn_bwd(3, d2, o2, x2, ga, s2, dx2, dg, db, B, R, R, R, R, R, rl, 1, st));
+    if (hf && have_dglob) {
+      const ieee_rowbn_bwd_prob pr[2] = {{d1, o1, x1, s1, dx1, PB, R, R, R, R, 0, 0}, {d2, o2, x2, s2, dx2, B, R, R, R, R, 1, 0}};
+      IEEE_TRY(ieee_rowbn_bwd_chain(3, pr, ga, dg, db, R, rl, st));
+    } else {
+      IEEE_TRY(ieee_rowbn_bwd(3, d1, o1, x1, ga, s1, dx1, dg, db, PB, R, R, R, R, R, rl, 0, st));
+      if (have_dglob) IEEE_TRY(ieee_rowbn_bwd(3, d2, o2, x2, ga, s2, dx2, dg, db, B, R, R, R, R, R, rl, 1, st));
+    }
   }
   {
     Set3 dw_, dx_;
diff --git a/ieee_amd/engine.py b/ieee_amd/engine.py
--- a/ieee_amd/engine.py
+++ b/ieee_amd/engine.py
@@ -417,10 +417,20 @@
         dl, df, small, work, mwork = self._scratch
         head_loss, head_acc, out3 = small[:18], small[18:36], small[36:39]
         ce_scale = float(weight_x) * ddp.ce_grad_scale(B, total_rows)
-        _lib.check(lib.ieee_ce_ls_fwd_bwd(_lib.ptr(logits), _lib.ptr(pids), _lib.ptr(dl), _lib.ptr(head_loss),
-                                          _lib.ptr(head_acc), _lib.ptr(work), 18, B, C, float(eps), ce_scale,
-                                          _lib.stream()))
-        if weight_m > 0:
+        if weight_m > 0 and os.environ.get("IEEE_HEAD_FUSED", "1") != "0":
+            _lib.check(lib.ieee_losses_fwd_bwd(_lib.ptr(logits), _lib.ptr(pids), _lib.ptr(dl), _lib.ptr(head_loss),
+                                               _lib.ptr(head_acc), _lib.ptr(work), 18, B, C, float(eps), ce_scale,
+                                               _lib.ptr(feats), _lib.ptr(df), _lib.ptr(out3), _lib.ptr(mwork),
+                                               feats.shape[2], float(margin), float(weight_m), _lib.stream()))
+            weight_m_done = True
+        else:
+            weight_m_done = False
+            _lib.check(lib.ieee_ce_ls_fwd_bwd(_lib.ptr(logits), _lib.ptr(pids), _lib.ptr(dl), _lib.ptr(head_loss),
+                                              _lib.ptr(head_acc), _lib.ptr(work), 18, B, C, float(eps), ce_scale,
+                                              _lib.stream()))
+        if weight_m_done:
+            pass
+        elif weight_m > 0:
             _lib.check(lib.ieee_margin3m_fwd_bwd(_lib.ptr(feats), _lib.ptr(pids), _lib.ptr(df), _lib.ptr(out3),
                                                  _lib.ptr(mwork), B, feats.shape[2], float(margin), float(weight_m),
                                                  _lib.stream()))
diff --git a/include/ieee_amd.h b/include/ieee_amd.h
--- a/include/ieee_amd.h
+++ b/include/ieee_amd.h
@@ -226,6 +226,69 @@
 } ieee_sgemm_set;
 int ieee_sgemm_grouped_pair_ws(const ieee_sgemm_set* s0, const ieee_sgemm_set* s1, void* work, int64_t work_bytes,
                                void* stream);
+int ieee_sgemm_grouped_sigmoid_ws(int64_t groups, const void* const* A, const void* const* B, void* const* C,
+                                  const void* const* bias, int64_t M, int64_t N, int64_t K, int64_t sam, int64_t sak,
+                                  int64_t sbn, int64_t sbk, int64_t ldc, float alpha, void* work, int64_t work_bytes,
+                                  void* stream);
+typedef struct ieee_pair_riders {
+  int64_t cs_groups;
+  const void* const* cs_X;
+  void* const* cs_out;
+  int64_t cs_M, cs_N, cs_ldx;
+  int64_t z_count;
+  void* const* z_ptrs;
+  const int64_t* z_floats;
+  int32_t cs_accumulate, defer;
+  int32_t splitk[2];
+  void* slab[2];
+  const float* dp_partial;
+  float* dp_out;
+  int64_t dp_grad_gs, dp_B;
+  int32_t dp_accumulate, reserved_;
+} ieee_pair_riders;
+int ieee_rem_bwd_partial(const float* dout, const float* r, const float* param, int64_t param_gs, float* dr, float* work,
+                         int64_t B, int64_t parts, int64_t D, void* stream);
+typedef struct ieee_sgemm_tail {
+  float* mix_out;
+  const float* rem_part;
+  float* rem_out;
+  const float* rem_param;
+  int64_t rem_param_gs, rem_parts;
+} ieee_sgemm_tail;
+int ieee_sgemm_grouped_tail_ws(int64_t groups, const void* const* A, const void* const* B, void* const* C,
+                               const void* const* bias, int64_t M, int64_t N, int64_t K, int64_t sam, int64_t sak,
+                               int64_t sbn, int64_t sbk, int64_t ldc, float alpha, int relu, const ieee_sgemm_tail* tail,
+                               void* work, int64_t work_bytes, void* stream);
+int ieee_sgemm_grouped_pair_ex(const ieee_sgemm_set* s0, const ieee_sgemm_set* s1, ieee_pair_riders* riders, void* work,
+                               int64_t work_bytes, void* stream);
+typedef struct ieee_rowbn_prob {
+  const void* const* x;
+  void* const* out;
+  void* const* save;
+  int64_t R, ldx, ldo;
+  const void* slab;
+  int64_t splitk;
+  const void* const* bias;
+} ieee_rowbn_prob;
+int ieee_rowbn_fwd_chain(int64_t nprob, int64_t groups, const ieee_rowbn_prob* probs, const void* const* gamma,
+                         const void* const* beta, void* const* running_mean, void* const* running_var, int64_t C,
+                         float momentum, float eps, int training, int relu, void* stream);
+typedef struct ieee_rowbn_bwd_prob {
+  const void* const* dout;
+  const void* const* out;
+  const void* const* x;
+  const void* const* save;
+  void* const* dx;
+  int64_t R, lddo, ldo, ldx, lddx;
+  int32_t accumulate, reserved_;
+} ieee_rowbn_bwd_prob;
+int ieee_rowbn_bwd_chain(int64_t groups, const ieee_rowbn_bwd_prob* probs, const void* const* gamma, void* const* dgamma,
+                         void* const* dbeta, int64_t C, int relu, void* stream);
+int ieee_l2norm_fwd_dual(const float* x, float* y, float* y2, float* norms, int64_t rows, int64_t D, void* stream);
+int ieee_losses_fwd_bwd(const float* logits, const int64_t* targets, float* dlogits, float* head_loss, float* head_acc,
+                        float* ce_work, int64_t heads, int64_t B, int64_t C, float eps, float ce_grad_scale,
+                        const float* feats, float* dfeats, float* out3, float* m_work, int64_t D, float margin,
+                        float m_grad_scale, void* stream);
 int ieee_zero_spans(int64_t count, void* const* ptrs, const int64_t* floats, void* stream);
 int ieee_colsum_grouped(int64_t groups, const void* const* X, void* const* out, int64_t M, int64_t N,
                         int64_t ldx, int accumulate, void* stream);
```

After: 4428 (median of 6 runs). About the same (+0.6%).
